# decisiongraph/leann-rs

Hardware: AMD Instinct MI355X
Metric: queries/sec @ recall@10>=0.95 (higher is better)
Workload: dtype f32

## Files before the change

### include/leann_backend.h

```cpp
#ifndef LEANN_BACKEND_H
#define LEANN_BACKEND_H
#include <stddef.h>
#include <stdint.h>

#ifdef __cplusplus
extern "C" {
#endif

typedef struct leann_backend leann_backend;

enum { LEANN_BACKEND_HNSW = 0, LEANN_BACKEND_DISKANN = 1 };

enum {
    LEANN_OK = 0,
    LEANN_ERR_INVALID = 1,
    LEANN_ERR_NOT_FOUND = 2,
    LEANN_ERR_FORMAT = 3,
    LEANN_ERR_DEVICE = 4,
    LEANN_ERR_UNSUPPORTED = 5,
    LEANN_ERR_IO = 6,
    LEANN_ERR_OVERFLOW = 7
};

const char *leann_last_error(void);
const char *leann_version(void);

int leann_backend_open(const char *index_path_stem, int backend, size_t dims,
                       const char *device_spec, leann_backend **out);

int leann_backend_search(const leann_backend *h, const float *query, size_t top_k,
                         size_t complexity, uint64_t *keys, float *dists, size_t *n_out);

int leann_backend_search_batch(const leann_backend *h, const float *queries, size_t nq,
                               size_t top_k, size_t complexity, uint64_t *keys, float *dists,
                               uint32_t *counts);

int leann_backend_search_filtered(const leann_backend *h, const float *query, size_t top_k,
                                  size_t complexity, const uint8_t *allow, uint64_t *keys,
                                  float *dists, size_t *n_out);
int leann_backend_search_filtered_batch(const leann_backend *h, const float *queries, size_t nq,
                                        size_t top_k, size_t complexity, const uint8_t *allow,
                                        size_t allow_stride, uint64_t *keys, float *dists,
                                        uint32_t *counts);

int leann_backend_search_filtered_exact_batch(const leann_backend *h, const float *queries, size_t nq,
                                              size_t top_k, const uint8_t *allow, size_t allow_stride,
                                              uint64_t *keys, float *dists, uint32_t *counts);

typedef struct leann_filter leann_filter;
int leann_backend_filter_create(const leann_backend *h, const uint8_t *allow, leann_filter **out);
size_t leann_backend_filter_count(const leann_filter *f);
void leann_backend_filter_free(leann_filter *f);
int leann_backend_search_filter_batch(const leann_backend *h, const float *queries, size_t nq, size_t top_k,
                                      size_t complexity, const leann_filter *filter, int mode,
                                      uint64_t *keys, float *dists, uint32_t *counts);

int leann_backend_set_coalescing(leann_backend *h, uint32_t wait_us, uint32_t max_batch);
int leann_backend_coalescing_stats(const leann_backend *h, uint64_t *n_launches, uint64_t *n_queries);

size_t leann_backend_len(const leann_backend *h);
size_t leann_backend_dims(const leann_backend *h);
void leann_backend_close(leann_backend *h);

int leann_backend_build(int backend, const float *vectors, size_t n, size_t dims,
                        size_t graph_degree, size_t complexity, const char *index_path_stem);
int leann_backend_add(int backend, const float *vectors, size_t n, size_t dims, size_t start_id,
                      const char *index_path_stem);

int leann_backend_remove(leann_backend *h, const uint64_t *keys, size_t n, size_t *n_removed);
int leann_backend_consolidate(leann_backend *h);
size_t leann_backend_live_len(const leann_backend *h);
int leann_backend_removed_bitmap(const leann_backend *h, uint8_t *out , size_t *n_pending);
int leann_backend_remove_from_index(int backend, const uint64_t *keys, size_t n, size_t dims, const char *index_path_stem);
int leann_tombstones_write(const char *path, const uint8_t *bitmap, uint64_t n, uint64_t n_pending);
int leann_tombstones_read(const char *path, uint64_t n_expected, uint8_t *bitmap_out, uint64_t *n_removed, uint64_t *n_pending);

typedef struct {
    uint64_t n_queries;
    uint64_t n_dist_evals;
    uint64_t n_hops_base;
    uint64_t n_hops_upper;
    uint64_t n_table_overflow;
    uint64_t algorithmic_bytes;
} leann_search_stats;
int leann_backend_stats(const leann_backend *h, leann_search_stats *out, int reset);


int leann_backend_build_device(int backend, const float *d_vectors, size_t n, size_t dims,
                               size_t ld, size_t graph_degree, size_t complexity, int device,
                               uint64_t key_offset, int take_copy, leann_backend **out);
int leann_backend_from_arrays(int backend, const float *vectors, size_t n, size_t dims,
                              uint32_t M, uint32_t M0, uint32_t max_level, uint32_t entry,
                              const uint8_t *levels, const uint32_t *upper_off,
                              const uint32_t *adj0, const uint32_t *adjU, size_t n_upper_lists,
                              int device, uint64_t key_offset, leann_backend **out);
int leann_backend_graph_info(const leann_backend *h, uint64_t *info );
int leann_backend_graph_export(const leann_backend *h, uint8_t *levels, uint32_t *upper_off,
                               uint32_t *adj0, uint32_t *adjU, float *vectors );
int leann_backend_save(const leann_backend *h, const char *index_path_stem);

int leann_backend_search_batch_device(const leann_backend *h, const float *d_queries, size_t nq,
                                      size_t top_k, size_t complexity, uint64_t *d_keys,
                                      float *d_dists, uint32_t *d_counts, uint32_t *d_stats,
                                      void *stream);
int leann_backend_search_filtered_batch_device(const leann_backend *h, const float *d_queries,
                                               size_t nq, size_t top_k, size_t complexity,
                                               const uint8_t *d_allow, size_t allow_stride,
                                               uint64_t *d_keys, float *d_dists, uint32_t *d_counts,
                                               uint32_t *d_stats, void *stream);
int leann_backend_search_filtered_exact_batch_device(const leann_backend *h, const float *d_queries,
                                                     size_t nq, size_t top_k, const uint8_t *d_allow,
                                                     size_t allow_stride, uint64_t *d_keys, float *d_dists,
                                                     uint32_t *d_counts, void *stream);
const float *leann_backend_device_rows(const leann_backend *h);

int leann_synth_rows_device(uint64_t seed, uint32_t dims, uint32_t ld, uint32_t r,
                            uint32_t n_clusters, float sigma, uint32_t stream_id, uint64_t i0,
                            uint64_t n, float *d_out, void *stream);

int leann_scan_topk_device(const float *d_rows, size_t n, size_t dims, size_t ld,
                           const float *d_queries, size_t nq, size_t top_k,
                           const uint8_t *d_allow_mask, uint64_t key_offset, uint64_t *d_keys,
                           float *d_scores, uint32_t *d_counts, void *stream);

typedef struct leann_recompute leann_recompute;
int leann_recompute_create(const uint16_t *d_features, size_t n, size_t h, const uint16_t *d_weights,
                           size_t dims, int device, uint64_t key_offset, leann_recompute **out);
int leann_recompute_create_pooled(const uint16_t *d_features, const uint8_t *d_mask, size_t n,
                                  size_t tokens_per_passage, size_t h, const uint16_t *d_weights,
                                  size_t dims, int device, uint64_t key_offset, leann_recompute **out);
int leann_recompute_search_batch_device(const leann_recompute *r, const float *d_queries, size_t nq,
                                        size_t top_k, const uint8_t *d_allow_mask, uint64_t *d_keys,
                                        float *d_scores, uint32_t *d_counts, void *stream);
int leann_recompute_create_host(const uint16_t *features, size_t n, size_t h, const uint16_t *weights,
                                size_t dims, int device, uint64_t key_offset, leann_recompute **out);
int leann_recompute_search_batch(const leann_recompute *r, const float *queries, size_t nq, size_t top_k,
                                 const uint8_t *allow_mask, uint64_t *keys, float *scores, uint32_t *counts);
int leann_recompute_create_sharded(const leann_recompute *const *parts, size_t n_parts, leann_recompute **out);
int leann_recompute_encode_device(const leann_recompute *r, uint64_t row0, uint64_t rows, float *d_out,
                                  void *stream);
size_t leann_recompute_len(const leann_recompute *r);
int leann_recompute_last_timing(const leann_recompute *r, float *ms3);
void leann_recompute_close(leann_recompute *r);
int leann_recompute_build_index(const leann_recompute *r, int backend, size_t graph_degree, size_t complexity,
                                leann_backend **out);
int leann_backend_feature_rows_export(const leann_backend *h, uint32_t *feat_h, uint32_t *row_bytes, void *out);
int leann_synth_features_device(uint64_t seed, uint32_t h, uint32_t r_int, uint32_t n_clusters, float sigma,
                                uint32_t stream_id, uint64_t i0, uint64_t n, uint16_t *d_out, void *stream);
int leann_synth_weights_device(uint64_t seed, uint32_t h, uint32_t dims, uint16_t *d_out, void *stream);

int leann_merge_topk_device(const uint64_t *d_keys, const float *d_dists, const uint32_t *d_counts,
                            size_t n_shards, size_t nq, size_t k_in, size_t k_out, int descending,
                            uint64_t *d_out_keys, float *d_out_dists, uint32_t *d_out_counts,
                            void *stream);

int leann_hybrid_rerank_device(const uint64_t *d_keys, const float *d_dists, const uint32_t *d_counts, size_t nq, size_t fetch_k,
                               const uint32_t *d_bm25_pos, const float *d_bm25_score, const uint32_t *d_bm25_count,
                               size_t bm25_stride, size_t n_docs, float alpha, int compat_polarity, size_t top_k,
                               uint64_t *d_out_keys, float *d_out_scores, uint32_t *d_out_counts, void *stream);

typedef struct leann_bm25 leann_bm25;
int leann_bm25_create(size_t n_docs, size_t n_terms, const uint64_t *post_off, const uint32_t *post_doc, const uint32_t *post_tf,
                      const uint32_t *doc_len, float avg_doc_len, int device, leann_bm25 **out);
size_t leann_bm25_len(const leann_bm25 *b);
size_t leann_bm25_slots(const leann_bm25 *b);
void leann_bm25_close(leann_bm25 *b);
int leann_bm25_check_queries(size_t n_terms, size_t nq, const uint32_t *q_off, const uint32_t *q_term, const float *q_idf);
int leann_bm25_search_batch(const leann_bm25 *b, size_t nq, const uint32_t *q_off, const uint32_t *q_term, const float *q_idf,
                            size_t top_k, uint32_t *pos, float *scores, uint32_t *counts, uint32_t *n_positive, float *min_max);
int leann_bm25_search_batch_device(const leann_bm25 *b, size_t nq, const uint32_t *q_off, const uint32_t *q_term, const float *q_idf,
                                   size_t top_k, uint32_t *d_pos, float *d_scores, uint32_t *d_counts, uint32_t *d_n_positive,
                                   float *d_min_max, void *stream);
int leann_bm25_hybrid_rerank_device(const leann_bm25 *b, size_t nq, const uint32_t *q_off, const uint32_t *q_term, const float *q_idf,
                                    const uint64_t *d_keys, const float *d_dists, const uint32_t *d_counts, size_t fetch_k,
                                    float alpha, int compat_polarity, size_t top_k,
                                    uint64_t *d_out_keys, float *d_out_scores, uint32_t *d_out_counts, void *stream);

typedef struct leann_sharded leann_sharded;
int leann_sharded_open(const char *index_path_stem, int backend, size_t dims, const char *device_spec, leann_sharded **out);
size_t leann_backend_shard_count(const leann_backend *h);
int leann_backend_shard(const leann_backend *h, size_t g, leann_backend **out);
int leann_sharded_build_device(int backend, const float *const *d_vectors, const size_t *rows, size_t n_shards, size_t dims,
                               size_t ld, size_t graph_degree, size_t complexity, const int *devices, leann_sharded **out);
int leann_sharded_from_handles(leann_backend *const *shards, size_t n_shards, int take_ownership, leann_sharded **out);
int leann_sharded_as_backend(leann_sharded *s, leann_backend **out);
int leann_rccl_get_unique_id(void *id128);
int leann_sharded_attach(leann_backend *local_shard, const void *unique_id128, int world, int rank, size_t total_rows,
                         leann_sharded **out);
int leann_sharded_search_batch_device(const leann_sharded *s, const float *d_queries, size_t nq, size_t top_k, size_t complexity,
                                      uint64_t *d_keys, float *d_dists, uint32_t *d_counts, uint32_t *d_stats, void *stream);
int leann_sharded_search_batch_device_async(const leann_sharded *s, const float *d_queries, size_t nq, size_t top_k,
                                            size_t complexity, uint64_t *d_keys, float *d_dists, uint32_t *d_counts,
                                            uint32_t *d_stats, void *stream, uint64_t *ticket);
int leann_sharded_wait(const leann_sharded *s, uint64_t ticket, void *stream);
size_t leann_sharded_len(const leann_sharded *s);
size_t leann_sharded_shards(const leann_sharded *s);
void leann_sharded_close(leann_sharded *s);

void leann_debug_reload_env(void);

int leann_device_count(int *n);
int leann_device_malloc(int device, size_t bytes, void **out);
int leann_device_free(void *p);
int leann_device_upload(void *d_dst, const void *h_src, size_t bytes);
int leann_device_download(void *h_dst, const void *d_src, size_t bytes);
int leann_device_sync(int device);

#ifdef __cplusplus
}
#endif
#endif
```

### leann-rs_amd/_native.py

```python
import ctypes as C
import os

_HERE = os.path.dirname(os.path.abspath(__file__))
LIB_PATH = os.environ.get("LEANN_LIB") or os.path.join(_HERE, "csrc", "libleann_hip.so")

u64p = C.POINTER(C.c_uint64)
u32p = C.POINTER(C.c_uint32)
u8p = C.POINTER(C.c_uint8)
f32p = C.POINTER(C.c_float)
vp = C.c_void_p


class LeannError(RuntimeError):
    def __init__(self, code, msg):
        super().__init__(msg)
        self.code = code


class SearchStats(C.Structure):
    _fields_ = [("n_queries", C.c_uint64), ("n_dist_evals", C.c_uint64), ("n_hops_base", C.c_uint64),
                ("n_hops_upper", C.c_uint64), ("n_table_overflow", C.c_uint64),
                ("algorithmic_bytes", C.c_uint64)]


SIGNATURES = {
    "leann_last_error": (C.c_char_p, []),
    "leann_version": (C.c_char_p, []),
    "leann_debug_reload_env": (None, []),
    "leann_backend_shard_count": (C.c_size_t, [vp]),
    "leann_backend_shard": (C.c_int, [vp, C.c_size_t, C.POINTER(vp)]),
    "leann_hybrid_rerank_device": (C.c_int, [vp, vp, vp, C.c_size_t, C.c_size_t, vp, vp, vp, C.c_size_t, C.c_size_t, C.c_float, C.c_int,
                                            C.c_size_t, vp, vp, vp, vp]),
    "leann_bm25_create": (C.c_int, [C.c_size_t, C.c_size_t, u64p, u32p, u32p, u32p, C.c_float, C.c_int, C.POINTER(vp)]),
    "leann_bm25_len": (C.c_size_t, [vp]),
    "leann_bm25_slots": (C.c_size_t, [vp]),
    "leann_bm25_close": (None, [vp]),
    "leann_bm25_check_queries": (C.c_int, [C.c_size_t, C.c_size_t, u32p, u32p, f32p]),
    "leann_bm25_search_batch": (C.c_int, [vp, C.c_size_t, u32p, u32p, f32p, C.c_size_t, u32p, f32p, u32p, u32p, f32p]),
    "leann_bm25_search_batch_device": (C.c_int, [vp, C.c_size_t, u32p, u32p, f32p, C.c_size_t, vp, vp, vp, vp, vp, vp]),
    "leann_bm25_hybrid_rerank_device": (C.c_int, [vp, C.c_size_t, u32p, u32p, f32p, vp, vp, vp, C.c_size_t, C.c_float, C.c_int,
                                                 C.c_size_t, vp, vp, vp, vp]),
    "leann_backend_open": (C.c_int, [C.c_char_p, C.c_int, C.c_size_t, C.c_char_p, C.POINTER(vp)]),
    "leann_backend_search": (C.c_int, [vp, f32p, C.c_size_t, C.c_size_t, u64p, f32p, C.POINTER(C.c_size_t)]),
    "leann_backend_search_batch": (C.c_int, [vp, f32p, C.c_size_t, C.c_size_t, C.c_size_t, u64p, f32p, u32p]),
    "leann_backend_search_filtered": (C.c_int, [vp, f32p, C.c_size_t, C.c_size_t, u8p, u64p, f32p, C.POINTER(C.c_size_t)]),
    "leann_backend_search_filtered_batch": (C.c_int, [vp, f32p, C.c_size_t, C.c_size_t, C.c_size_t, u8p, C.c_size_t,
                                                     u64p, f32p, u32p]),
    "leann_backend_set_coalescing": (C.c_int, [vp, C.c_uint32, C.c_uint32]),
    "leann_backend_coalescing_stats": (C.c_int, [vp, u64p, u64p]),
    "leann_backend_len": (C.c_size_t, [vp]),
    "leann_backend_dims": (C.c_size_t, [vp]),
    "leann_backend_close": (None, [vp]),
    "leann_backend_build": (C.c_int, [C.c_int, f32p, C.c_size_t, C.c_size_t, C.c_size_t, C.c_size_t, C.c_char_p]),
    "leann_backend_add": (C.c_int, [C.c_int, f32p, C.c_size_t, C.c_size_t, C.c_size_t, C.c_char_p]),
    "leann_backend_remove": (C.c_int, [vp, u64p, C.c_size_t, C.POINTER(C.c_size_t)]),
    "leann_backend_consolidate": (C.c_int, [vp]),
    "leann_backend_live_len": (C.c_size_t, [vp]),
    "leann_backend_removed_bitmap": (C.c_int, [vp, u8p, C.POINTER(C.c_size_t)]),
    "leann_backend_remove_from_index": (C.c_int, [C.c_int, u64p, C.c_size_t, C.c_size_t, C.c_char_p]),
    "leann_tombstones_write": (C.c_int, [C.c_char_p, u8p, C.c_uint64, C.c_uint64]),
    "leann_tombstones_read": (C.c_int, [C.c_char_p, C.c_uint64, u8p, u64p, u64p]),
    "leann_backend_stats": (C.c_int, [vp, C.POINTER(SearchStats), C.c_int]),
    "leann_backend_build_device": (C.c_int, [C.c_int, vp, C.c_size_t, C.c_size_t, C.c_size_t, C.c_size_t,
                                            C.c_size_t, C.c_int, C.c_uint64, C.c_int, C.POINTER(vp)]),
    "leann_backend_from_arrays": (C.c_int, [C.c_int, f32p, C.c_size_t, C.c_size_t, C.c_uint32, C.c_uint32,
                                           C.c_uint32, C.c_uint32, u8p, u32p, u32p, u32p, C.c_size_t,
                                           C.c_int, C.c_uint64, C.POINTER(vp)]),
    "leann_backend_graph_info": (C.c_int, [vp, u64p]),
    "leann_backend_graph_export": (C.c_int, [vp, u8p, u32p, u32p, u32p, f32p]),
    "leann_backend_save": (C.c_int, [vp, C.c_char_p]),
    "leann_backend_search_batch_device": (C.c_int, [vp, vp, C.c_size_t, C.c_size_t, C.c_size_t, vp, vp, vp,
                                                   vp, vp]),
    "leann_backend_search_filtered_exact_batch": (C.c_int, [vp, f32p, C.c_size_t, C.c_size_t, u8p, C.c_size_t, u64p, f32p, u32p]),
    "leann_backend_filter_create": (C.c_int, [vp, u8p, C.POINTER(vp)]),
    "leann_backend_filter_count": (C.c_size_t, [vp]),
    "leann_backend_filter_free": (None, [vp]),
    "leann_backend_search_filter_batch": (C.c_int, [vp, f32p, C.c_size_t, C.c_size_t, C.c_size_t, vp, C.c_int, u64p, f32p, u32p]),
    "leann_backend_search_filtered_exact_batch_device": (C.c_int, [vp, vp, C.c_size_t, C.c_size_t, vp, C.c_size_t, vp, vp, vp, vp]),
    "leann_backend_search_filtered_batch_device": (C.c_int, [vp, vp, C.c_size_t, C.c_size_t, C.c_size_t, vp, C.c_size_t,
                                                            vp, vp, vp, vp, vp]),
    "leann_backend_device_rows": (vp, [vp]),
    "leann_synth_rows_device": (C.c_int, [C.c_uint64, C.c_uint32, C.c_uint32, C.c_uint32, C.c_uint32,
                                         C.c_float, C.c_uint32, C.c_uint64, C.c_uint64, vp, vp]),
    "leann_scan_topk_device": (C.c_int, [vp, C.c_size_t, C.c_size_t, C.c_size_t, vp, C.c_size_t, C.c_size_t,
                                        vp, C.c_uint64, vp, vp, vp, vp]),
    "leann_recompute_create": (C.c_int, [vp, C.c_size_t, C.c_size_t, vp, C.c_size_t, C.c_int, C.c_uint64, C.POINTER(vp)]),
    "leann_recompute_create_pooled": (C.c_int, [vp, vp, C.c_size_t, C.c_size_t, C.c_size_t, vp, C.c_size_t, C.c_int, C.c_uint64,
                                               C.POINTER(vp)]),
    "leann_recompute_create_sharded": (C.c_int, [C.POINTER(vp), C.c_size_t, C.POINTER(vp)]),
    "leann_recompute_create_host": (C.c_int, [C.POINTER(C.c_uint16), C.c_size_t, C.c_size_t, C.POINTER(C.c_uint16), C.c_size_t, C.c_int,
                                             C.c_uint64, C.POINTER(vp)]),
    "leann_recompute_search_batch": (C.c_int, [vp, f32p, C.c_size_t, C.c_size_t, u8p, u64p, f32p, u32p]),
    "leann_recompute_search_batch_device": (C.c_int, [vp, vp, C.c_size_t, C.c_size_t, vp, vp, vp, vp, vp]),
    "leann_recompute_encode_device": (C.c_int, [vp, C.c_uint64, C.c_uint64, vp, vp]),
    "leann_recompute_len": (C.c_size_t, [vp]),
    "leann_recompute_last_timing": (C.c_int, [vp, f32p]),
    "leann_recompute_close": (None, [vp]),
    "leann_recompute_build_index": (C.c_int, [vp, C.c_int, C.c_size_t, C.c_size_t, C.POINTER(vp)]),
    "leann_backend_feature_rows_export": (C.c_int, [vp, u32p, u32p, vp]),
    "leann_synth_features_device": (C.c_int, [C.c_uint64, C.c_uint32, C.c_uint32, C.c_uint32, C.c_float, C.c_uint32, C.c_uint64,
                                             C.c_uint64, vp, vp]),
    "leann_synth_weights_device": (C.c_int, [C.c_uint64, C.c_uint32, C.c_uint32, vp, vp]),
    "leann_merge_topk_device": (C.c_int, [vp, vp, vp, C.c_size_t, C.c_size_t, C.c_size_t, C.c_size_t,
                                         C.c_int, vp, vp, vp, vp]),
    "leann_sharded_open": (C.c_int, [C.c_char_p, C.c_int, C.c_size_t, C.c_char_p, C.POINTER(vp)]),
    "leann_sharded_build_device": (C.c_int, [C.c_int, C.POINTER(vp), C.POINTER(C.c_size_t), C.c_size_t, C.c_size_t, C.c_size_t, C.c_size_t,
                                            C.c_size_t, C.POINTER(C.c_int), C.POINTER(vp)]),
    "leann_sharded_from_handles": (C.c_int, [C.POINTER(vp), C.c_size_t, C.c_int, C.POINTER(vp)]),
    "leann_sharded_as_backend": (C.c_int, [vp, C.POINTER(vp)]),
    "leann_rccl_get_unique_id": (C.c_int, [vp]),
    "leann_sharded_attach": (C.c_int, [vp, vp, C.c_int, C.c_int, C.c_size_t, C.POINTER(vp)]),
    "leann_sharded_search_batch_device": (C.c_int, [vp, vp, C.c_size_t, C.c_size_t, C.c_size_t, vp, vp, vp, vp, vp]),
    "leann_sharded_search_batch_device_async": (C.c_int, [vp, vp, C.c_size_t, C.c_size_t, C.c_size_t, vp, vp, vp, vp, vp, u64p]),
    "leann_sharded_wait": (C.c_int, [vp, C.c_uint64, vp]),
    "leann_sharded_len": (C.c_size_t, [vp]),
    "leann_sharded_shards": (C.c_size_t, [vp]),
    "leann_sharded_close": (None, [vp]),
    "leann_device_count": (C.c_int, [C.POINTER(C.c_int)]),
    "leann_device_malloc": (C.c_int, [C.c_int, C.c_size_t, C.POINTER(vp)]),
    "leann_device_free": (C.c_int, [vp]),
    "leann_device_upload": (C.c_int, [vp, vp, C.c_size_t]),
    "leann_device_download": (C.c_int, [vp, vp, C.c_size_t]),
    "leann_device_sync": (C.c_int, [C.c_int]),
}

_lib = None


def lib():
    global _lib
    if _lib is None:
        if not os.path.exists(LIB_PATH):
            raise ImportError(
                f"{LIB_PATH} is missing: build it with `make` (hipcc --offload-arch=gfx950). "
                "leann-rs_amd has no CPU fallback.")
        L = C.CDLL(LIB_PATH)
        for name, (res, args) in SIGNATURES.items():
            f = getattr(L, name)
            f.restype = res
            f.argtypes = args
        _lib = L
    return _lib


def check(rc):
    if rc != 0:
        raise LeannError(rc, lib().leann_last_error().decode("utf-8", "replace"))


def device_count():
    n = C.c_int(0)
    lib().leann_device_count(C.byref(n))
    return n.value
```

### leann-rs_amd/backend.py

```python
import ctypes as C
import enum
import os

import numpy as np

from . import _native as N
from ._native import LeannError, f32p, u32p, u64p, u8p


class BackendType(enum.IntEnum):
    Hnsw = 0
    DiskAnn = 1

    @classmethod
    def from_name(cls, name):
        if name == "hnsw":
            return cls.Hnsw
        if name == "diskann":
            return cls.DiskAnn
        raise LeannError(1, f"Unknown backend: {name}")

    def load_searcher(self, index_path, dimensions, device=0):
        return BackendSearcher.load(self, index_path, dimensions, device)


def _p(a, t):
    return a.ctypes.data_as(t) if a is not None else None


class BackendSearcher:

    def __init__(self, handle, backend_type):
        self._h = handle
        self.backend_type = BackendType(backend_type)

    @classmethod
    def load(cls, backend_type, index_path, dimensions, device=0):
        h = C.c_void_p()
        N.check(N.lib().leann_backend_open(os.fsencode(str(index_path)), int(backend_type), dimensions,
                                           str(device).encode(), C.byref(h)))
        return cls(h, backend_type)

    @classmethod
    def from_arrays(cls, backend_type, vectors, M, M0, max_level, entry, levels, upper_off, adj0, adjU,
                    device=0, key_offset=0):
        vectors = np.ascontiguousarray(vectors, np.float32)
        levels = np.ascontiguousarray(levels, np.uint8)
        upper_off = np.ascontiguousarray(upper_off, np.uint32)
        adj0 = np.ascontiguousarray(adj0, np.uint32)
        adjU = np.ascontiguousarray(adjU, np.uint32)
        nul = adjU.size // M if adjU.size else 0
        h = C.c_void_p()
        n, d = vectors.shape
        N.check(N.lib().leann_backend_from_arrays(
            int(backend_type), _p(vectors, f32p), n, d, M, M0, max_level, entry, _p(levels, u8p),
            _p(upper_off, u32p), _p(adj0, u32p), _p(adjU, u32p) if nul else None, nul, device,
            key_offset, C.byref(h)))
        return cls(h, backend_type)

    @classmethod
    def build_device(cls, backend_type, d_vectors_ptr, n, dims, ld, graph_degree, complexity, device=0,
                     key_offset=0, take_copy=False):
        h = C.c_void_p()
        N.check(N.lib().leann_backend_build_device(int(backend_type), d_vectors_ptr, n, dims, ld,
                                                   graph_degree, complexity, device, key_offset,
                                                   1 if take_copy else 0, C.byref(h)))
        return cls(h, backend_type)

    def search(self, query, top_k, complexity):
        q = np.ascontiguousarray(query, np.float32).reshape(-1)
        if q.shape[0] != self.dims():
            raise LeannError(1, f"query has {q.shape[0]} dimensions, index has {self.dims()}")
        keys = np.zeros(max(top_k, 1), np.uint64)
        dists = np.zeros(max(top_k, 1), np.float32)
        n = C.c_size_t(0)
        N.check(N.lib().leann_backend_search(self._h, _p(q, f32p), top_k, complexity, _p(keys, u64p),
                                             _p(dists, f32p), C.byref(n)))
        return keys[: n.value].copy(), dists[: n.value].copy()

    def search_batch(self, queries, top_k, complexity):
        Q = np.ascontiguousarray(queries, np.float32)
        if Q.ndim != 2 or Q.shape[1] != self.dims():
            raise LeannError(1, f"queries must be [nq x {self.dims()}]")
        nq = Q.shape[0]
        keys = np.full((nq, top_k), np.iinfo(np.uint64).max, np.uint64)
        dists = np.full((nq, top_k), np.inf, np.float32)
        counts = np.zeros(nq, np.uint32)
        N.check(N.lib().leann_backend_search_batch(self._h, _p(Q, f32p), nq, top_k, complexity,
                                                   _p(keys, u64p), _p(dists, f32p), _p(counts, u32p)))
        return keys, dists, counts

    def search_filtered(self, query, top_k, complexity, allow):
        q = np.ascontiguousarray(query, np.float32).reshape(-1)
        if q.shape[0] != self.dims():
            raise LeannError(1, f"query has {q.shape[0]} dimensions, index has {self.dims()}")
        allow = np.ascontiguousarray(allow, np.uint8).reshape(-1)
        if allow.shape[0] < (self.len() + 7) // 8:
            raise LeannError(1, f"allow-bitmap has {allow.shape[0]} bytes, index needs {(self.len() + 7) // 8}")
        keys = np.zeros(max(top_k, 1), np.uint64)
        dists = np.zeros(max(top_k, 1), np.float32)
        n = C.c_size_t(0)
        N.check(N.lib().leann_backend_search_filtered(self._h, _p(q, f32p), top_k, complexity, _p(allow, u8p),
                                                      _p(keys, u64p), _p(dists, f32p), C.byref(n)))
        return keys[: n.value].copy(), dists[: n.value].copy()

    def search_filtered_batch(self, queries, top_k, complexity, allow):
        Q = np.ascontiguousarray(queries, np.float32)
        if Q.ndim != 2 or Q.shape[1] != self.dims():
            raise LeannError(1, f"queries must be [nq x {self.dims()}]")
        allow = np.ascontiguousarray(allow, np.uint8)
        stride = 0 if allow.ndim == 1 else allow.shape[1]
        if allow.shape[-1] < (self.len() + 7) // 8 or (allow.ndim == 2 and allow.shape[0] != Q.shape[0]):
            raise LeannError(1, "allow-bitmap shape does not match the index / the batch")
        nq = Q.shape[0]
        keys = np.full((nq, top_k), np.iinfo(np.uint64).max, np.uint64)
        dists = np.full((nq, top_k), np.inf, np.float32)
        counts = np.zeros(nq, np.uint32)
        N.check(N.lib().leann_backend_search_filtered_batch(self._h, _p(Q, f32p), nq, top_k, complexity, _p(allow, u8p),
                                                            stride, _p(keys, u64p), _p(dists, f32p), _p(counts, u32p)))
        return keys, dists, counts

    def search_filtered_exact_batch(self, queries, top_k, allow):
        Q = np.ascontiguousarray(queries, np.float32)
        if Q.ndim != 2 or Q.shape[1] != self.dims():
            raise LeannError(1, f"queries must be [nq x {self.dims()}]")
        allow = np.ascontiguousarray(allow, np.uint8)
        stride = 0 if allow.ndim == 1 else allow.shape[1]
        if allow.shape[-1] < (self.len() + 7) // 8 or (allow.ndim == 2 and allow.shape[0] != Q.shape[0]):
            raise LeannError(1, "allow-bitmap shape does not match the index / the batch")
        nq = Q.shape[0]
        keys = np.full((nq, top_k), np.iinfo(np.uint64).max, np.uint64)
        dists = np.full((nq, top_k), np.inf, np.float32)
        counts = np.zeros(nq, np.uint32)
        N.check(N.lib().leann_backend_search_filtered_exact_batch(self._h, _p(Q, f32p), nq, top_k, _p(allow, u8p), stride,
                                                                  _p(keys, u64p), _p(dists, f32p), _p(counts, u32p)))
        return keys, dists, counts

    def search_filtered_exact_batch_device(self, d_queries, nq, top_k, d_allow, allow_stride, d_keys, d_dists, d_counts,
                                           stream=None):
        N.check(N.lib().leann_backend_search_filtered_exact_batch_device(self._h, d_queries, nq, top_k, d_allow, allow_stride,
                                                                         d_keys, d_dists, d_counts, stream))

    def register_filter(self, allow):
        allow = np.ascontiguousarray(allow, np.uint8)
        if allow.ndim != 1 or allow.shape[0] < (self.len() + 7) // 8:
            raise LeannError(1, "allow-bitmap shape does not match the index")
        h = C.c_void_p()
        N.check(N.lib().leann_backend_filter_create(self._h, _p(allow, u8p), C.byref(h)))
        return Filter(h)

    def search_filter_batch(self, queries, top_k, complexity, flt, mode="auto"):
        Q = np.ascontiguousarray(queries, np.float32)
        if Q.ndim != 2 or Q.shape[1] != self.dims():
            raise LeannError(1, f"queries must be [nq x {self.dims()}]")
        nq = Q.shape[0]
        keys = np.full((nq, top_k), np.iinfo(np.uint64).max, np.uint64)
        dists = np.full((nq, top_k), np.inf, np.float32)
        counts = np.zeros(nq, np.uint32)
        N.check(N.lib().leann_backend_search_filter_batch(self._h, _p(Q, f32p), nq, top_k, complexity, flt._h,
                                                          {"walk": 0, "exact": 1, "auto": 2}[mode], _p(keys, u64p), _p(dists, f32p),
                                                          _p(counts, u32p)))
        return keys, dists, counts

    def search_batch_device(self, d_queries, nq, top_k, complexity, d_keys, d_dists, d_counts,
                            d_stats=None, stream=None):
        N.check(N.lib().leann_backend_search_batch_device(self._h, d_queries, nq, top_k, complexity,
                                                          d_keys, d_dists, d_counts, d_stats, stream))

    def search_filtered_batch_device(self, d_queries, nq, top_k, complexity, d_allow, allow_stride, d_keys, d_dists,
                                     d_counts, d_stats=None, stream=None):
        N.check(N.lib().leann_backend_search_filtered_batch_device(self._h, d_queries, nq, top_k, complexity, d_allow,
                                                                   allow_stride, d_keys, d_dists, d_counts, d_stats, stream))

    def set_coalescing(self, wait_us=200, max_batch=4096):
        N.check(N.lib().leann_backend_set_coalescing(self._h, wait_us, max_batch))

    def coalescing_stats(self):
        a, b = C.c_uint64(0), C.c_uint64(0)
        N.check(N.lib().leann_backend_coalescing_stats(self._h, C.byref(a), C.byref(b)))
        return {"launches": a.value, "queries": b.value}

    def len(self):
        return int(N.lib().leann_backend_len(self._h))

    __len__ = len

    def is_empty(self):
        return self.len() == 0

    def dims(self):
        return int(N.lib().leann_backend_dims(self._h))

    def remove(self, keys):
        k = np.ascontiguousarray(keys, np.uint64).reshape(-1)
        n = C.c_size_t(0)
        N.check(N.lib().leann_backend_remove(self._h, _p(k, u64p), k.shape[0], C.byref(n)))
        return int(n.value)

    def consolidate(self):
        N.check(N.lib().leann_backend_consolidate(self._h))

    def live_len(self):
        return int(N.lib().leann_backend_live_len(self._h))

    def removed_bitmap(self):
        bm = np.zeros(max((self.len() + 7) // 8, 1), np.uint8)
        pend = C.c_size_t(0)
        N.check(N.lib().leann_backend_removed_bitmap(self._h, _p(bm, u8p), C.byref(pend)))
        return bm[: (self.len() + 7) // 8], int(pend.value)

    def stats(self, reset=False):
        s = N.SearchStats()
        N.check(N.lib().leann_backend_stats(self._h, C.byref(s), 1 if reset else 0))
        return {k: int(getattr(s, k)) for k, _ in N.SearchStats._fields_}

    def graph_info(self):
        info = np.zeros(8, np.uint64)
        N.check(N.lib().leann_backend_graph_info(self._h, _p(info, u64p)))
        names = ("n", "dims", "ld", "M", "M0", "max_level", "entry", "n_upper_lists")
        return {k: int(v) for k, v in zip(names, info)}

    def graph_export(self, with_vectors=False):
        gi = self.graph_info()
        n = gi["n"]
        levels = np.zeros(n, np.uint8)
        upper_off = np.zeros(n, np.uint32)
        adj0 = np.zeros((n, gi["M0"]), np.uint32)
        adjU = np.zeros((max(gi["n_upper_lists"], 1), gi["M"]), np.uint32)
        X = np.zeros((n, gi["dims"]), np.float32) if with_vectors else None
        N.check(N.lib().leann_backend_graph_export(self._h, _p(levels, u8p), _p(upper_off, u32p),
                                                   _p(adj0, u32p), _p(adjU, u32p), _p(X, f32p)))
        return dict(gi, levels=levels, upper_off=upper_off, adj0=adj0, adjU=adjU[: gi["n_upper_lists"]],
                    vectors=X)

    def n_shards(self):
        return int(N.lib().leann_backend_shard_count(self._h))

    def shard(self, g):
        h = C.c_void_p()
        N.check(N.lib().leann_backend_shard(self._h, g, C.byref(h)))
        s = BackendSearcher(h, self.backend_type)
        s._borrowed = True
        return s

    def device_rows_ptr(self):
        return N.lib().leann_backend_device_rows(self._h)

    def save(self, index_path):
        N.check(N.lib().leann_backend_save(self._h, os.fsencode(str(index_path))))

    def close(self):
        if self._h:
            if not getattr(self, "_borrowed", False):
                N.lib().leann_backend_close(self._h)
            self._h = None

    def __del__(self):
        try:
            self.close()
        except Exception:
            pass


class HnswSearcher(BackendSearcher):

    @classmethod
    def load(cls, index_path, dimensions, device=0):
        return BackendSearcher.load.__func__(cls, BackendType.Hnsw, index_path, dimensions, device)


class DiskAnnSearcher(BackendSearcher):

    @classmethod
    def load(cls, index_path, dimensions, device=0):
        return BackendSearcher.load.__func__(cls, BackendType.DiskAnn, index_path, dimensions, device)


class BackendBuilder:

    def __init__(self, backend_type):
        self.backend_type = BackendType(backend_type)

    def build(self, embeddings, ids, index_path, dimensions, graph_degree, complexity):
        X = np.ascontiguousarray(embeddings, np.float32)
        if X.ndim != 2 or X.shape[1] != dimensions:
            raise LeannError(1, f"embeddings must be [n x {dimensions}]")
        N.check(N.lib().leann_backend_build(int(self.backend_type), _p(X, f32p), X.shape[0], dimensions,
                                            graph_degree, complexity, os.fsencode(str(index_path))))

    def add_to_index(self, embeddings, index_path, dimensions, start_id):
        X = np.ascontiguousarray(embeddings, np.float32)
        N.check(N.lib().leann_backend_add(int(self.backend_type), _p(X, f32p), X.shape[0], dimensions,
                                          start_id, os.fsencode(str(index_path))))

    def remove_from_index(self, keys, index_path, dimensions):
        k = np.ascontiguousarray(keys, np.uint64).reshape(-1)
        N.check(N.lib().leann_backend_remove_from_index(int(self.backend_type), _p(k, u64p), k.shape[0], dimensions,
                                                        os.fsencode(str(index_path))))



class Filter:

    def __init__(self, handle):
        self._h = handle

    def count(self):
        return int(N.lib().leann_backend_filter_count(self._h))

    def close(self):
        if self._h:
            N.lib().leann_backend_filter_free(self._h)
            self._h = None

    def __del__(self):
        try:
            self.close()
        except Exception:
            pass


class ShardedIndex:

    def __init__(self, handle, keep=()):
        self._h = handle
        self._keep = keep

    @classmethod
    def open(cls, backend_type, index_path, dimensions, device_spec):
        h = C.c_void_p()
        N.check(N.lib().leann_sharded_open(os.fsencode(str(index_path)), int(backend_type), dimensions, str(device_spec).encode(), C.byref(h)))
        return cls(h)

    @classmethod
    def build_device(cls, backend_type, d_ptrs, rows, dims, ld, graph_degree, complexity, devices, keep=()):
        G = len(d_ptrs)
        ptrs = (C.c_void_p * G)(*[C.c_void_p(p) for p in d_ptrs])
        rws = (C.c_size_t * G)(*rows)
        devs = (C.c_int * G)(*devices)
        h = C.c_void_p()
        N.check(N.lib().leann_sharded_build_device(int(backend_type), ptrs, rws, G, dims, ld, graph_degree, complexity, devs, C.byref(h)))
        return cls(h, keep)

    @classmethod
    def from_searchers(cls, searchers, take_ownership=False):
        G = len(searchers)
        hs = (C.c_void_p * G)(*[s._h for s in searchers])
        h = C.c_void_p()
        N.check(N.lib().leann_sharded_from_handles(hs, G, 1 if take_ownership else 0, C.byref(h)))
        if take_ownership:
            for s in searchers:
                s._h = None
        return cls(h, tuple(searchers))

    @staticmethod
    def rccl_unique_id():
        buf = C.create_string_buffer(128)
        N.check(N.lib().leann_rccl_get_unique_id(buf))
        return buf.raw

    @classmethod
    def attach(cls, searcher, unique_id, world, rank, total_rows=0):
        h = C.c_void_p()
        N.check(N.lib().leann_sharded_attach(searcher._h, C.c_char_p(bytes(unique_id)), world, rank, total_rows, C.byref(h)))
        return cls(h, (searcher,))

    def search_batch_device(self, d_queries, nq, top_k, complexity, d_keys, d_dists, d_counts, d_stats=None, stream=None):
        N.check(N.lib().leann_sharded_search_batch_device(self._h, d_queries, nq, top_k, complexity, d_keys, d_dists, d_counts, d_stats, stream))

    def search_batch_device_async(self, d_queries, nq, top_k, complexity, d_keys, d_dists, d_counts, d_stats=None, stream=None):
        t = C.c_uint64(0)
        N.check(N.lib().leann_sharded_search_batch_device_async(self._h, d_queries, nq, top_k, complexity, d_keys, d_dists, d_counts, d_stats,
                                                                stream, C.byref(t)))
        return t.value

    def wait(self, ticket, stream=None):
        N.check(N.lib().leann_sharded_wait(self._h, ticket, stream))

    def as_backend(self, backend_type=BackendType.Hnsw):
        h = C.c_void_p()
        N.check(N.lib().leann_sharded_as_backend(self._h, C.byref(h)))
        keep, self._h = self._keep, None
        s = BackendSearcher(h, backend_type)
        s._keep = keep
        return s

    def len(self):
        return int(N.lib().leann_sharded_len(self._h))

    def n_shards(self):
        return int(N.lib().leann_sharded_shards(self._h))

    def close(self):
        if self._h:
            N.lib().leann_sharded_close(self._h)
            self._h = None

    def __del__(self):
        try:
            self.close()
        except Exception:
            pass
```

### leann-rs_amd/csrc/api.hip

```cpp
#include "common.cuh"
#include "search.cuh"
#include "../../include/leann_backend.h"
#include "internal.h"

#include <algorithm>
#include <cstdarg>
#include <cstdio>
#include <cstring>
#include <strings.h>
#include <map>
#include <mutex>
#include <string>
#include <vector>
#include <sys/stat.h>
#include <chrono>
#include <condition_variable>
#include <thread>

static thread_local char g_err[2048] = "";
extern "C" void leann_set_error(const char *fmt, ...) {
    va_list ap;
    va_start(ap, fmt);
    vsnprintf(g_err, sizeof(g_err), fmt, ap);
    va_end(ap);
}
extern "C" const char *leann_last_error(void) { return g_err; }
void leann_log(int level, const char *fmt, ...) {
    static const int threshold = [] {
        const char *e = getenv("LEANN_LOG");
        if (!e) return (int)LEANN_LOG_WARN;
        if (!strcasecmp(e, "error")) return (int)LEANN_LOG_ERROR;
        if (!strcasecmp(e, "info")) return (int)LEANN_LOG_INFO;
        if (!strcasecmp(e, "debug") || !strcasecmp(e, "trace")) return (int)LEANN_LOG_DEBUG;
        return (int)LEANN_LOG_WARN;
    }();
    if (level > threshold) return;
    static const char *names[] = {"ERROR", "WARN", "INFO", "DEBUG"};
    char buf[1024];
    va_list ap;
    va_start(ap, fmt);
    vsnprintf(buf, sizeof(buf), fmt, ap);
    va_end(ap);
    fprintf(stderr, "%s leann_hip: %s\n", names[level < 0 ? 0 : (level > 3 ? 3 : level)], buf);
}
extern "C" const char *leann_version(void) { return "leann-rs_amd 0.1 (gfx950)"; }

static LeannKnobs *read_knobs_from_env() {
    LeannKnobs *k = new LeannKnobs();
    auto num = [](const char *name, int lo, int hi) { const char *e = getenv(name); if (!e || !*e) return 0; int v = atoi(e); return v >= lo && v <= hi ? v : 0; };
    auto flag = [](const char *name) { const char *e = getenv(name); return e && *e && strcmp(e, "0") != 0; };
    k->hash_bits = num("LEANN_DEBUG_HASH_BITS", 6, 15);
    k->nw = num("LEANN_DEBUG_NW", 1, 64);
    k->gpool_bits = num("LEANN_DEBUG_GPOOL_BITS", 6, 31);
    k->gpool2_bits = num("LEANN_DEBUG_GPOOL2_BITS", 6, 31);
    k->no_feat256 = flag("LEANN_DEBUG_NO_FEAT256");
    k->no_zero_copy = flag("LEANN_DEBUG_NO_ZERO_COPY");
    k->no_emit = flag("LEANN_DEBUG_NO_EMIT");
    k->fused_v1 = flag("LEANN_DEBUG_FUSED_V1");
    k->no_list = flag("LEANN_RECOMPUTE_NO_LIST");
    k->no_tiled = flag("LEANN_RECOMPUTE_NO_TILED");
    k->hnsw_reference_ef = flag("LEANN_HNSW_REFERENCE_EF");
    k->force_remote = flag("LEANN_DEBUG_FORCE_REMOTE");
    if (const char *e = getenv("LEANN_COALESCE")) k->coalesce_off = !strcmp(e, "off") || !strcmp(e, "0");
    if (const char *e = getenv("LEANN_STAMP_BUF")) k->stamp_buf = strtoull(e, nullptr, 0);
    return k;
}
static std::atomic<const LeannKnobs *> g_knobs{nullptr};
const LeannKnobs &leann_knobs() {
    const LeannKnobs *k = g_knobs.load(std::memory_order_acquire);
    if (!k) {
        LeannKnobs *fresh = read_knobs_from_env();
        const LeannKnobs *expected = nullptr;
        if (g_knobs.compare_exchange_strong(expected, fresh, std::memory_order_acq_rel)) k = fresh;
        else { delete fresh; k = expected; }
    }
    return *k;
}
extern "C" void leann_debug_reload_env(void) { g_knobs.store(read_knobs_from_env(), std::memory_order_release); }

extern "C" int leann_device_count(int *n) {
    int c = 0;
    hipError_t e = hipGetDeviceCount(&c);
    if (e != hipSuccess) { c = 0; (void)hipGetLastError(); }
    *n = c;
    return LEANN_OK;
}
extern "C" int leann_device_malloc(int device, size_t bytes, void **out) {
    HIP_CHECK_RET(hipSetDevice(device));
    HIP_CHECK_RET(hipMalloc(out, bytes ? bytes : 16));
    return LEANN_OK;
}
extern "C" int leann_device_free(void *p) {
    if (p) HIP_CHECK_RET(hipFree(p));
    return LEANN_OK;
}
extern "C" int leann_device_upload(void *d, const void *h, size_t bytes) {
    HIP_CHECK_RET(hipMemcpy(d, h, bytes, hipMemcpyHostToDevice));
    return LEANN_OK;
}
extern "C" int leann_device_download(void *h, const void *d, size_t bytes) {
    HIP_CHECK_RET(hipMemcpy(h, d, bytes, hipMemcpyDeviceToHost));
    return LEANN_OK;
}
extern "C" int leann_device_sync(int device) {
    HIP_CHECK_RET(hipSetDevice(device));
    HIP_CHECK_RET(hipDeviceSynchronize());
    return LEANN_OK;
}

extern "C" int leann_backend_set_coalescing(leann_backend *h, uint32_t wait_us, uint32_t max_batch);
static void ws_free(Workspace *w) {
    if (!w) return;
    (void)hipFree(w->d_q);
    (void)hipFree(w->d_keys);
    (void)hipFree(w->d_dists);
    (void)hipFree(w->d_counts);
    (void)hipFree(w->d_stats);
    (void)hipFree(w->d_allow);
    if (w->pin) (void)hipHostFree(w->pin);
    if (w->stream) (void)hipStreamDestroy(w->stream);
    delete w;
}
static uint32_t debug_bits(int knob, uint32_t lo, uint32_t hi, uint32_t dflt) {
    return knob >= (int)lo && knob <= (int)hi ? (uint32_t)knob : dflt;
}
static int ensure_gpool(leann_backend *h) {
    std::lock_guard<std::mutex> lk(h->mu);
    if (h->gpool) return LEANN_OK;
    unsigned long long *p = nullptr, *p2 = nullptr;
    uint32_t *lock = nullptr, *lock2 = nullptr;
    const uint32_t bits = debug_bits(leann_knobs().gpool_bits, 6, GPOOL_BITS, GPOOL_BITS), tables = GPOOL_TABLES;
    const size_t slots = (size_t)tables << bits;
    uint32_t bits2 = 0, tables2 = 0;
    const uint64_t need = h->g.n + 128;
    if (need > (1ull << bits) - (1ull << (bits - 2))) {
        bits2 = bits + 1;
        while (bits2 < 31 && (1ull << bits2) - (1ull << (bits2 - 2)) < need) bits2++;
        bits2 = debug_bits(leann_knobs().gpool2_bits, 6, 31, bits2);
        const uint64_t per = 8ull << bits2;
        tables2 = (uint32_t)std::min<uint64_t>(64, std::max<uint64_t>(2, (1ull << 30) / per));
    }
    auto fail = [&](const char *what) {
        (void)hipFree(p); (void)hipFree(p2); (void)hipFree(lock); (void)hipFree(lock2);
        leann_set_error("visited-table pool: %s failed: %s", what, hipGetErrorString(hipGetLastError()));
        return LEANN_ERR_DEVICE;
    };
    if (hipMalloc((void **)&p, slots * 8) != hipSuccess) return fail("hipMalloc");
    if (hipMalloc((void **)&lock, (tables + 4) * 4) != hipSuccess) return fail("hipMalloc");
    if (hipMemset(p, 0, slots * 8) != hipSuccess) return fail("hipMemset");
    if (hipMemset(lock, 0, (tables + 4) * 4) != hipSuccess) return fail("hipMemset");
    if (tables2) {
        if (hipMalloc((void **)&p2, ((size_t)tables2 << bits2) * 8) != hipSuccess) return fail("hipMalloc");
        if (hipMalloc((void **)&lock2, tables2 * 4) != hipSuccess) return fail("hipMalloc");
        if (hipMemset(p2, 0, ((size_t)tables2 << bits2) * 8) != hipSuccess) return fail("hipMemset");
        if (hipMemset(lock2, 0, tables2 * 4) != hipSuccess) return fail("hipMemset");
    }
    if (hipDeviceSynchronize() != hipSuccess) return fail("hipDeviceSynchronize");
    h->gpool_lock = lock;
    h->gpool_ctr = lock + tables;
    h->gpool_bits = bits;
    h->gpool_tables = tables;
    h->gpool2 = p2;
    h->gpool2_lock = lock2;
    h->gpool2_bits = bits2;
    h->gpool2_tables = tables2;
    h->gpool = p;
    return LEANN_OK;
}
static void set_pool_args(const leann_backend *h, SearchArgs &a) {
    a.gpool = h->gpool; a.gpool_lock = h->gpool_lock; a.gpool_ctr = h->gpool_ctr;
    a.gpool_bits = h->gpool_bits; a.gpool_tables = h->gpool_tables;
    a.gpool2 = h->gpool2; a.gpool2_lock = h->gpool2_lock; a.gpool2_bits = h->gpool2_bits; a.gpool2_tables = h->gpool2_tables;
}

void leann_internal_free_graph(leann_backend *h) {
    if (h->owns_rows) (void)hipFree((void *)h->g.X);
    (void)hipFree((void *)h->g.norms);
    (void)hipFree((void *)h->g.adj0);
    (void)hipFree((void *)h->g.adjU);
    (void)hipFree((void *)h->g.upper_off);
    (void)hipFree(h->d_levels);
    (void)hipFree(h->gpool);
    (void)hipFree(h->gpool_lock);
    (void)hipFree(h->gpool2);
    (void)hipFree(h->gpool2_lock);
    (void)hipFree(h->Wf32);
    for (auto &kv : h->proj_scratch) (void)hipFree(kv.second.first);
    leann_internal_free_removed(h);
}

extern "C" void leann_backend_close(leann_backend *h) {
    if (!h) return;
    leann_backend_set_coalescing(h, 0, 0);
    (void)hipSetDevice(h->device);
    (void)hipDeviceSynchronize();
    for (auto *w : h->free_ws) ws_free(w);
    if (h->sharded) leann_sharded_close(h->sharded);
    else leann_internal_free_graph(h);
    delete h;
}
extern "C" size_t leann_backend_len(const leann_backend *h) { return h ? (size_t)h->g.n : 0; }
extern "C" size_t leann_backend_dims(const leann_backend *h) { return h ? (size_t)h->g.d : 0; }
extern "C" const float *leann_backend_device_rows(const leann_backend *h) { return h && !h->sharded ? h->g.X : nullptr; }
#define NOT_ON_SHARDED(h, what)                                                                                                    \
    do {                                                                                                                           \
        if ((h) && (h)->sharded) {                                                                                                 \
            leann_set_error("%s is not available on a sharded handle (use leann_backend_shard(h, g) for one shard's)", what);       \
            return LEANN_ERR_UNSUPPORTED;                                                                                          \
        }                                                                                                                          \
    } while (0)

extern "C" int leann_backend_stats(const leann_backend *hc, leann_search_stats *out, int reset) {
    leann_backend *h = const_cast<leann_backend *>(hc);
    if (!h || !out) { leann_set_error("leann_backend_stats: null argument"); return LEANN_ERR_INVALID; }
    std::lock_guard<std::mutex> lk(h->mu);
    *out = h->stats;
    if (reset) h->stats = leann_search_stats{};
    return LEANN_OK;
}

size_t leann_internal_effective_complexity(const leann_backend *h, size_t complexity) {
    return (h->fixed_ef && h->kind == LEANN_BACKEND_HNSW) ? (size_t)h->fixed_ef : complexity;
}

static uint32_t pick_hash_bits(uint32_t ef) {
    if (const int v = leann_knobs().hash_bits) return (uint32_t)v;
    uint32_t want = ef * 24u, b = 13;
    while ((1u << b) < want && b < 15) b++;
    return b;
}

using SearchKernel = void (*)(GraphView, SearchArgs);
static int launch_one(SearchKernel kernel, int nthreads, size_t lds, const GraphView &g, const SearchArgs &a, hipStream_t st) {
    if (lds > 64 * 1024)
        HIP_CHECK_RET(hipFuncSetAttribute((const void *)kernel, hipFuncAttributeMaxDynamicSharedMemorySize, 160 * 1024));
    hipLaunchKernelGGL(kernel, dim3(a.nq), dim3(nthreads), lds, st, g, a);
    HIP_CHECK_RET(hipGetLastError());
    return LEANN_OK;
}
static int search_lds_checked(const GraphView &g, const SearchArgs &a, size_t *lds, int nw) {
    *lds = search_lds_bytes(a.ef, std::max(g.M0, g.M), a.hash_bits, a.allow ? a.k : 0u, nw > 4 ? 2u : 1u);
    if (*lds > 160 * 1024) {
        leann_set_error("search: complexity %u needs %zu B of LDS per query (> 160 KiB)", a.ef, *lds);
        return LEANN_ERR_INVALID;
    }
    return LEANN_OK;
}

static bool wide_graph(const GraphView &g) { return std::max(g.M0, g.M) > 64; }

template <int T, int R, int NW>
static int launch_search_NW(const GraphView &g, const SearchArgs &a, hipStream_t st) {
    size_t lds;
    if (int rc = search_lds_checked(g, a, &lds, NW)) return rc;
    SearchKernel k = a.allow ? beam_search_filtered_kernel<T, R, NW> : a.q_rows ? beam_search_kernel<T, R, NW, true> : beam_search_kernel<T, R, NW, false>;
    if constexpr (NW != 8)
        if (wide_graph(g))
            k = a.allow ? wide_beam_search_filtered_kernel<T, R, NW> : a.q_rows ? wide_beam_search_kernel<T, R, NW, true> : wide_beam_search_kernel<T, R, NW, false>;
    return launch_one(k, NW * 64, lds, g, a, st);
}

template <int T, int R>
static int launch_search_T(const GraphView &g, const SearchArgs &a, hipStream_t st) {
    int nw = a.nq <= 384 ? 16 : a.nq <= 640 ? 8 : 4;
    if (const int v = leann_knobs().nw) nw = v;
    if (nw >= 8 && wide_graph(g)) nw = 16;
    if (nw >= 16) return launch_search_NW<T, R, 16>(g, a, st);
    if (nw >= 8) return launch_search_NW<T, R, 8>(g, a, st);
    return launch_search_NW<T, R, 4>(g, a, st);
}

template <int T, int R>
static int launch_search_feat(const GraphView &g, const SearchArgs &a, hipStream_t st) {
    size_t lds;
    if (int rc = search_lds_checked(g, a, &lds, a.nq <= 512 ? 16 : 4)) return rc;
    const bool wide = wide_graph(g), filt = a.allow != nullptr, small = a.nq <= 512;
    SearchKernel k;
    if (T == 1 && g.feat_h == 256 && !leann_knobs().no_feat256)
        k = wide ? (small ? (filt ? wide_beam_search_feat256_filtered_kernel<1, 16> : wide_beam_search_feat256_kernel<1, 16>)
                          : (filt ? wide_beam_search_feat256_filtered_kernel<LEANN_FEAT_G, 4> : wide_beam_search_feat256_kernel<LEANN_FEAT_G, 4>))
                 : (small ? (filt ? beam_search_feat256_filtered_kernel<1, 16> : beam_search_feat256_kernel<1, 16>)
                          : (filt ? beam_search_feat256_filtered_kernel<LEANN_FEAT_G, 4> : beam_search_feat256_kernel<LEANN_FEAT_G, 4>));
    else
        k = wide ? (small ? (filt ? wide_beam_search_feat_filtered_kernel<T, R, 16> : wide_beam_search_feat_kernel<T, R, 16>)
                          : (filt ? wide_beam_search_feat_filtered_kernel<T, R, 4> : wide_beam_search_feat_kernel<T, R, 4>))
                 : (small ? (filt ? beam_search_feat_filtered_kernel<T, R, 16> : beam_search_feat_kernel<T, R, 16>)
                          : (filt ? beam_search_feat_filtered_kernel<T, R, 4> : beam_search_feat_kernel<T, R, 4>));
    return launch_one(k, small ? 16 * 64 : 4 * 64, lds, g, a, st);
}

static int project_queries(leann_backend *h, const float *d_queries, size_t nq, hipStream_t st, const float **out) {
    float *G = nullptr;
    {
        std::lock_guard<std::mutex> lk(h->mu);
        auto &sc = h->proj_scratch[st];
        const size_t need = nq * h->g.feat_h;
        if (sc.second < need) {
            (void)hipFree(sc.first);
            sc.first = nullptr;
            sc.second = 0;
            if (hipMalloc((void **)&sc.first, need * 4) != hipSuccess) { leann_set_error("hipMalloc(%zu) failed", need * 4); return LEANN_ERR_DEVICE; }
            sc.second = need;
        }
        G = sc.first;
    }
    int rc = leann_internal_score(h->Wf32, h->g.feat_h, h->g.d, h->g.d, d_queries, nq, h->g.d, G, st);
    *out = G;
    return rc;
}

int leann_internal_launch_search(leann_backend *h, SearchArgs a, hipStream_t st) {
    if (a.nq == 0) return LEANN_OK;
    if (h->g.feat_h) {
        if (a.q_rows) { leann_set_error("recompute-on index: construction searches are not supported"); return LEANN_ERR_UNSUPPORTED; }
        if (a.ef < a.k) a.ef = a.k;
        a.hash_bits = leann_knobs().hash_bits ? pick_hash_bits(a.ef) : (a.ef <= 64 ? 12u : pick_hash_bits(a.ef));
        int rc = ensure_gpool(h);
        if (rc) return rc;
        set_pool_args(h, a);
        const float *G = nullptr;
        rc = project_queries(h, a.queries, a.nq, st, &G);
        if (rc) return rc;
        a.queries = G;
        a.ldq = h->g.feat_h;
        const int T = (int)((h->g.feat_h + 255) / 256);
        switch (T) {
            case 1: return launch_search_feat<1, LEANN_FEAT_R1>(h->g, a, st);
            case 2: return launch_search_feat<2, 6>(h->g, a, st);
            case 3: case 4: return launch_search_feat<4, 4>(h->g, a, st);
            default: leann_set_error("recompute-on index: feature width %u > 1024 not supported", h->g.feat_h); return LEANN_ERR_INVALID;
        }
    }
    if (a.ef < a.k) a.ef = a.k;
    a.hash_bits = (h->g.ld <= 512 && a.ef <= 64 && !a.q_rows && !leann_knobs().hash_bits) ? 12u : pick_hash_bits(a.ef);
    int rc = ensure_gpool(h);
    if (rc) return rc;
    set_pool_args(h, a);
    const GraphView &g = h->g;
    int T = (int)((g.ld + 255) / 256);
    switch (T) {
        case 1: return launch_search_T<1, 4>(g, a, st);
        case 2: return launch_search_T<2, 4>(g, a, st);
        case 3: return launch_search_T<3, 4>(g, a, st);
        case 4: return launch_search_T<4, 3>(g, a, st);
        case 5: case 6: return launch_search_T<6, 2>(g, a, st);
        case 7: case 8: return launch_search_T<8, 2>(g, a, st);
        case 9: case 10: case 11: case 12: return launch_search_T<12, 1>(g, a, st);
        case 13: case 14: case 15: case 16: return launch_search_T<16, 1>(g, a, st);
        default:
            leann_set_error("search: dims %u > 4096 not supported", g.d);
            return LEANN_ERR_INVALID;
    }
}

extern "C" int leann_backend_search_batch_device(const leann_backend *hc, const float *d_queries, size_t nq,
                                                 size_t top_k, size_t complexity, uint64_t *d_keys, float *d_dists,
                                                 uint32_t *d_counts, uint32_t *d_stats, void *stream) {
    return leann_backend_search_filtered_batch_device(hc, d_queries, nq, top_k, complexity, nullptr, 0, d_keys, d_dists,
                                                      d_counts, d_stats, stream);
}

int leann_internal_search_plain(leann_backend *h, const float *d_queries, size_t nq, size_t top_k, size_t complexity, const SearchFilter &f,
                                uint64_t *d_keys, float *d_dists, uint32_t *d_counts, uint32_t *d_stats, hipStream_t st) {
    if (int rc = leann_internal_check_allow_stride(f, h->g.n)) return rc;
    if (nq == 0) return LEANN_OK;
    if (f.exact && h->g.feat_h) {
        leann_set_error("exact filtered search needs stored vectors; this index recomputes them from features (use leann_recompute_search_batch_device with an allow mask)");
        return LEANN_ERR_UNSUPPORTED;
    }
    if (h->g.n == 0) {
        HIP_CHECK_RET(hipMemsetAsync(d_counts, 0, nq * 4, st));
        return LEANN_OK;
    }
    const leann_filter *reg = f.registered;
    const uint8_t *allow = reg ? reg->d_allow : f.d_allow;
    size_t allow_stride = reg ? 0 : f.allow_stride;
    if (!reg)
        if (int rc = leann_internal_live_allow(h, allow, allow_stride, nq, !f.exact, st, &allow, &allow_stride)) return rc;
    if (f.exact) {
        if (!allow) { leann_set_error("exact filtered search: no filter given"); return LEANN_ERR_INVALID; }
        if (d_stats) HIP_CHECK_RET(hipMemsetAsync(d_stats, 0, nq * 16, st));
        if (reg)
            return leann_internal_filtered_exact_list(h->g.X, h->g.d, h->g.ld, d_queries, nq, top_k, reg->d_list, reg->n_allowed, h->key_offset,
                                                      d_keys, d_dists, d_counts, st);
        return leann_internal_filtered_exact(h->g.X, h->g.n, h->g.d, h->g.ld, d_queries, nq, top_k, allow, allow_stride, h->key_offset, d_keys,
                                             d_dists, d_counts, st);
    }
    SearchArgs a{};
    a.queries = d_queries;
    a.ldq = h->g.d;
    a.nq = (uint32_t)nq;
    a.k = (uint32_t)top_k;
    a.ef = (uint32_t)std::max(leann_internal_effective_complexity(h, complexity), top_k);
    a.target_level = 0;
    a.key_offset = h->key_offset;
    a.out_keys = d_keys;
    a.out_dists = d_dists;
    a.out_counts = d_counts;
    a.out_stats = d_stats;
    a.allow = allow;
    a.allow_stride = allow_stride;
#ifdef LEANN_STAMPS
    if (const unsigned long long e = leann_knobs().stamp_buf) {
        a.out_nexp = reinterpret_cast<uint32_t *>(e);
        a.exp_cap = 0xFEED;
    }
#endif
    return leann_internal_launch_search(h, a, st);
}
static int search_device(leann_backend *h, const float *d_queries, size_t nq, size_t top_k, size_t complexity, const SearchFilter &f,
                         uint64_t *d_keys, float *d_dists, uint32_t *d_counts, uint32_t *d_stats, hipStream_t st) {
    HIP_CHECK_RET(hipSetDevice(h->device));
    if (h->sharded) return leann_internal_sharded_search(h->sharded, d_queries, nq, top_k, complexity, f, d_keys, d_dists, d_counts, d_stats, st, nullptr);
    return leann_internal_search_plain(h, d_queries, nq, top_k, complexity, f, d_keys, d_dists, d_counts, d_stats, st);
}

extern "C" int leann_backend_search_filtered_batch_device(const leann_backend *hc, const float *d_queries, size_t nq,
                                                          size_t top_k, size_t complexity, const uint8_t *d_allow,
                                                          size_t allow_stride, uint64_t *d_keys, float *d_dists,
                                                          uint32_t *d_counts, uint32_t *d_stats, void *stream) {
    leann_backend *h = const_cast<leann_backend *>(hc);
    if (!h || !d_queries || !d_keys || !d_dists || !d_counts || top_k == 0) {
        leann_set_error("leann_backend_search_batch_device: null/zero argument");
        return LEANN_ERR_INVALID;
    }
    SearchFilter f;
    f.d_allow = d_allow; f.allow_stride = allow_stride;
    return search_device(h, d_queries, nq, top_k, complexity, f, d_keys, d_dists, d_counts, d_stats, (hipStream_t)stream);
}

extern "C" int leann_backend_search_batch(const leann_backend *hc, const float *queries, size_t nq, size_t top_k,
                                          size_t complexity, uint64_t *keys, float *dists, uint32_t *counts) {
    return leann_backend_search_filtered_batch(hc, queries, nq, top_k, complexity, nullptr, 0, keys, dists, counts);
}

enum { FILTER_WALK = 0, FILTER_EXACT = 1, FILTER_AUTO = 2 };
static int search_filtered_batch_host(const leann_backend *hc, const float *queries, size_t nq, size_t top_k, size_t complexity,
                                      const uint8_t *allow, size_t allow_stride, uint64_t *keys, float *dists, uint32_t *counts, int mode,
                                      const leann_filter *flt = nullptr);

extern "C" int leann_backend_filter_create(const leann_backend *hc, const uint8_t *allow, leann_filter **out) {
    if (!hc || !allow || !out) {
        leann_set_error("leann_backend_filter_create: null argument");
        return LEANN_ERR_INVALID;
    }
    *out = nullptr;
    if (hc->sharded) {
        const size_t G = leann_internal_sharded_count(hc->sharded);
        leann_filter *f = new leann_filter();
        f->device = hc->device;
        f->n = hc->g.n;
        for (size_t g = 0; g < G; g++) {
            leann_backend *sh = leann_internal_sharded_shard(hc->sharded, g);
            const uint64_t lo = leann_internal_sharded_lo(hc->sharded, g);
            leann_filter *part = nullptr;
            int rc = (!sh || (lo & 7)) ? (leann_set_error("registered filter: shard %zu does not start at a multiple of 8", g), (int)LEANN_ERR_UNSUPPORTED)
                                       : leann_backend_filter_create(sh, allow + lo / 8, &part);
            if (rc) { leann_backend_filter_free(f); return rc; }
            f->parts.push_back(part);
            f->n_allowed += part->n_allowed;
        }
        (void)hipSetDevice(hc->device);
        f->epoch = hc->removal_epoch;
        *out = f;
        return LEANN_OK;
    }
    if (hc->g.n >= (1ull << 32)) {
        leann_set_error("leann_backend_filter_create: the index has 2^32 rows or more");
        return LEANN_ERR_INVALID;
    }
    HIP_CHECK_RET(hipSetDevice(hc->device));
    leann_filter *f = new leann_filter();
    f->device = hc->device;
    f->n = hc->g.n;
    const size_t nbytes = std::max<size_t>((f->n + 7) / 8, 1);
    if (hipMalloc((void **)&f->d_allow, nbytes) != hipSuccess || hipMemcpy(f->d_allow, allow, (f->n + 7) / 8, hipMemcpyHostToDevice) != hipSuccess) {
        leann_set_error("leann_backend_filter_create: device allocation / copy of %zu bytes failed", nbytes);
        if (f->d_allow) (void)hipFree(f->d_allow);
        delete f;
        return LEANN_ERR_DEVICE;
    }
    f->epoch = hc->removal_epoch;
    int rc = leann_internal_and_live_inplace(hc, f->d_allow);
    if (rc == LEANN_OK && f->n) rc = leann_internal_compact_allow(f->d_allow, f->n, &f->d_list, &f->n_allowed, nullptr);
    if (rc != LEANN_OK) {
        (void)hipFree(f->d_allow);
        delete f;
        return rc;
    }
    *out = f;
    return LEANN_OK;
}
extern "C" size_t leann_backend_filter_count(const leann_filter *f) { return f ? f->n_allowed : 0; }
extern "C" void leann_backend_filter_free(leann_filter *f) {
    if (!f) return;
    if (!f->parts.empty()) {
        for (auto *p : f->parts) leann_backend_filter_free(p);
        delete f;
        return;
    }
    (void)hipSetDevice(f->device);
    (void)hipDeviceSynchronize();
    leann_internal_scratch_release(f->d_list);
    if (f->d_allow) (void)hipFree(f->d_allow);
    delete f;
}
extern "C" int leann_backend_search_filter_batch(const leann_backend *hc, const float *queries, size_t nq, size_t top_k, size_t complexity,
                                                 const leann_filter *filter, int mode, uint64_t *keys, float *dists, uint32_t *counts) {
    if (!filter || !hc || filter->n != hc->g.n || filter->device != hc->device || mode < FILTER_WALK || mode > FILTER_AUTO ||
        filter->parts.empty() != (hc->sharded == nullptr)) {
        leann_set_error("leann_backend_search_filter_batch: null / foreign filter (made for %zu rows, the index has %zu) or bad mode %d",
                        filter ? filter->n : (size_t)0, hc ? (size_t)hc->g.n : (size_t)0, mode);
        return LEANN_ERR_INVALID;
    }
    bool stale = filter->epoch != hc->removal_epoch;
    if (hc->sharded)
        for (size_t g = 0; g < filter->parts.size() && g < leann_internal_sharded_count(hc->sharded); g++)
            stale = stale || filter->parts[g]->epoch != leann_internal_sharded_shard(hc->sharded, g)->removal_epoch;
    if (stale) {
        leann_set_error("leann_backend_search_filter_batch: filter predates a removal; register it again");
        return LEANN_ERR_INVALID;
    }
    return search_filtered_batch_host(hc, queries, nq, top_k, complexity, nullptr, 0, keys, dists, counts, mode, filter);
}

extern "C" int leann_backend_search_filtered_batch(const leann_backend *hc, const float *queries, size_t nq, size_t top_k,
                                                   size_t complexity, const uint8_t *allow, size_t allow_stride,
                                                   uint64_t *keys, float *dists, uint32_t *counts) {
    return search_filtered_batch_host(hc, queries, nq, top_k, complexity, allow, allow_stride, keys, dists, counts, FILTER_WALK);
}
extern "C" int leann_backend_search_filtered_exact_batch(const leann_backend *hc, const float *queries, size_t nq, size_t top_k,
                                                         const uint8_t *allow, size_t allow_stride, uint64_t *keys, float *dists,
                                                         uint32_t *counts) {
    if (!allow) {
        leann_set_error("leann_backend_search_filtered_exact_batch: null allow-bitmap");
        return LEANN_ERR_INVALID;
    }
    return search_filtered_batch_host(hc, queries, nq, top_k, 0, allow, allow_stride, keys, dists, counts, FILTER_EXACT);
}
extern "C" int leann_backend_search_filtered_exact_batch_device(const leann_backend *hc, const float *d_queries, size_t nq, size_t top_k,
                                                                const uint8_t *d_allow, size_t allow_stride, uint64_t *d_keys,
                                                                float *d_dists, uint32_t *d_counts, void *stream) {
    leann_backend *h = const_cast<leann_backend *>(hc);
    if (!h || !d_queries || !d_keys || !d_dists || !d_counts || !d_allow || top_k == 0) {
        leann_set_error("leann_backend_search_filtered_exact_batch_device: null/zero argument");
        return LEANN_ERR_INVALID;
    }
    SearchFilter f;
    f.d_allow = d_allow; f.allow_stride = allow_stride; f.exact = true;
    return search_device(h, d_queries, nq, top_k, 0, f, d_keys, d_dists, d_counts, nullptr, (hipStream_t)stream);
}
static int search_filtered_batch_host_impl(const leann_backend *hc, const float *queries, size_t nq, size_t top_k, size_t complexity,
                                      const uint8_t *allow, size_t allow_stride, uint64_t *keys, float *dists, uint32_t *counts, int mode,
                                      const leann_filter *flt) {
    leann_backend *h = const_cast<leann_backend *>(hc);
    bool exact = mode == FILTER_EXACT;
    const bool stored_vectors = hc && !(hc->sharded ? leann_internal_sharded_shard(hc->sharded, 0)->g.feat_h : hc->g.feat_h);
    if (mode == FILTER_AUTO && flt && hc && stored_vectors && top_k <= 1024) {
        const double frac = nq <= 64 ? 0.05 : 0.015;
        exact = flt->n_allowed <= std::max<size_t>((size_t)(frac * (double)hc->g.n), nq <= 64 ? 65536 : 0);
    }
    if (!h || !queries || !keys || !dists || !counts) {
        leann_set_error("leann_backend_search_batch: null argument");
        return LEANN_ERR_INVALID;
    }
    if (nq == 0 || top_k == 0 || h->g.n == 0) {
        for (size_t i = 0; i < nq; i++) counts[i] = 0;
        return LEANN_OK;
    }
    HIP_CHECK_RET(hipSetDevice(h->device));
    Workspace *w = nullptr;
    {
        std::lock_guard<std::mutex> lk(h->mu);
        if (!h->free_ws.empty()) { w = h->free_ws.back(); h->free_ws.pop_back(); }
    }
    if (!w) w = new Workspace();
    int rc = LEANN_OK;
    auto fail = [&](int code) { std::lock_guard<std::mutex> lk(h->mu); h->free_ws.push_back(w); return code; };
    if (!w->stream) {
        if (hipStreamCreateWithFlags(&w->stream, hipStreamNonBlocking) != hipSuccess) {
            leann_set_error("hipStreamCreate failed");
            return fail(LEANN_ERR_DEVICE);
        }
    }
    const size_t d = h->g.d, qf = nq * d, no = nq * top_k;
    const size_t ns = 1;
    auto grow = [&](void **p, size_t &cap, size_t need, size_t elt) -> int {
        if (need <= cap) return 0;
        (void)hipFree(*p);
        *p = nullptr;
        cap = 0;
        if (hipMalloc(p, need * elt) != hipSuccess) { leann_set_error("hipMalloc(%zu) failed", need * elt); return 1; }
        cap = need;
        return 0;
    };
    const size_t o_keys = (qf * 4 + 15) & ~(size_t)15, o_dists = o_keys + no * 8, o_counts = (o_dists + no * 4 + 15) & ~(size_t)15,
                 o_stats = o_counts + ((nq * 4 + 15) & ~(size_t)15), pin_bytes = o_stats + nq * 16;
    bool zero_copy = !h->sharded && !exact && pin_bytes <= ((size_t)256 << 10) && !leann_knobs().no_zero_copy;
    if (zero_copy && w->cap_pin < pin_bytes) {
        if (w->pin) (void)hipHostFree(w->pin);
        w->pin = nullptr;
        w->cap_pin = 0;
        const size_t want = std::max<size_t>(pin_bytes, (size_t)64 << 10);
        if (hipHostMalloc((void **)&w->pin, want, hipHostMallocDefault) == hipSuccess) w->cap_pin = want;
        else { (void)hipGetLastError(); zero_copy = false; }
    }
    const bool zc_in = zero_copy && nq <= 4;
    if (zero_copy && !zc_in && grow((void **)&w->d_q, w->cap_q, qf, 4)) return fail(LEANN_ERR_DEVICE);
    if (!zero_copy && (grow((void **)&w->d_q, w->cap_q, qf, 4) || grow((void **)&w->d_keys, w->cap_keys, no, 8) ||
        grow((void **)&w->d_dists, w->cap_dists, no, 4) || grow((void **)&w->d_counts, w->cap_counts, nq, 4) ||
        grow((void **)&w->d_stats, w->cap_stats, ns * nq * 4, 4)))
        return fail(LEANN_ERR_DEVICE);
    hipStream_t st = w->stream;
    if (allow) {
        const size_t total = allow_stride ? allow_stride * nq : (h->g.n + 7) / 8;
        void *pa = w->d_allow;
        if (grow(&pa, w->cap_allow, total, 1)) { w->d_allow = (uint8_t *)pa; return fail(LEANN_ERR_DEVICE); }
        w->d_allow = (uint8_t *)pa;
        if (hipMemcpyAsync(w->d_allow, allow, total, hipMemcpyHostToDevice, st) != hipSuccess) {
            leann_set_error("H2D copy of the allow-bitmap failed");
            return fail(LEANN_ERR_DEVICE);
        }
    }
    if (zero_copy) memcpy(w->pin, queries, qf * 4);
    if (!zc_in && hipMemcpyAsync(w->d_q, zero_copy ? reinterpret_cast<const float *>(w->pin) : queries, qf * 4, hipMemcpyHostToDevice, st) != hipSuccess) {
        leann_set_error("H2D copy of queries failed");
        return fail(LEANN_ERR_DEVICE);
    }
    SearchFilter f;
    f.exact = exact;
    if (flt) f.registered = flt;
    else if (allow) { f.d_allow = w->d_allow; f.allow_stride = allow_stride; }
    const float *d_q = zc_in ? reinterpret_cast<const float *>(w->pin) : w->d_q;
    uint64_t *d_keys = zero_copy ? reinterpret_cast<uint64_t *>(w->pin + o_keys) : w->d_keys;
    float *d_dists = zero_copy ? reinterpret_cast<float *>(w->pin + o_dists) : w->d_dists;
    uint32_t *d_counts = zero_copy ? reinterpret_cast<uint32_t *>(w->pin + o_counts) : w->d_counts;
    uint32_t *d_stats = zero_copy ? reinterpret_cast<uint32_t *>(w->pin + o_stats) : w->d_stats;
    rc = h->sharded ? leann_internal_sharded_search(h->sharded, d_q, nq, top_k, complexity, f, d_keys, d_dists, d_counts, d_stats, st, nullptr)
                    : leann_internal_search_plain(h, d_q, nq, top_k, complexity, f, d_keys, d_dists, d_counts, d_stats, st);
    if (rc) return fail(rc);
    std::vector<uint32_t> hstats(ns * nq * 4);
    if (zero_copy) {
        if (hipStreamSynchronize(st) != hipSuccess) {
            leann_set_error("search: device error: %s", hipGetErrorString(hipGetLastError()));
            return fail(LEANN_ERR_DEVICE);
        }
        memcpy(keys, w->pin + o_keys, no * 8);
        memcpy(dists, w->pin + o_dists, no * 4);
// ... 30 lines not shown
        return LEANN_ERR_OVERFLOW;
    }
    return LEANN_OK;
}

static int search_filtered_batch_host(const leann_backend *hc, const float *queries, size_t nq, size_t top_k, size_t complexity,
                                      const uint8_t *allow, size_t allow_stride, uint64_t *keys, float *dists, uint32_t *counts, int mode,
                                      const leann_filter *flt) {
    try {
        return search_filtered_batch_host_impl(hc, queries, nq, top_k, complexity, allow, allow_stride, keys, dists, counts, mode, flt);
    } catch (const std::exception &e) {
        leann_set_error("search: %s", e.what());
        return LEANN_ERR_DEVICE;
    }
}

struct PendingQuery {
    const float *q;
    size_t k, ef;
    uint64_t *keys;
    float *dists;
    size_t *n_out;
    int rc = 0;
    bool done = false, answered = false;
    std::string err;
};
struct Coalescer {
    leann_backend *h = nullptr;
    uint32_t wait_us = 200, max_batch = 4096;
    std::mutex mu;
    std::condition_variable cv_submit, cv_done;
    std::vector<PendingQuery *> queue;
    std::thread th;
    bool stop = false;
    uint64_t n_launches = 0, n_queries = 0;
    size_t recent_callers = 0;

    void run() {
        (void)hipSetDevice(h->device);
        std::unique_lock<std::mutex> lk(mu);
        for (;;) {
            cv_submit.wait(lk, [&] { return stop || !queue.empty(); });
            if (stop && queue.empty()) return;
            const size_t fire_at = std::min<size_t>(max_batch, std::max<size_t>(1, recent_callers));
            auto deadline = std::chrono::steady_clock::now() + std::chrono::microseconds(wait_us);
            cv_submit.wait_until(lk, deadline, [&] { return stop || queue.size() >= fire_at; });
            std::vector<PendingQuery *> batch;
            batch.swap(queue);
            lk.unlock();
            std::map<std::pair<size_t, size_t>, std::vector<PendingQuery *>> groups;
            for (auto *p : batch) groups[{p->k, p->ef}].push_back(p);
            const size_t d = h->g.d;
            try {
            for (auto &kv : groups) {
                auto &g = kv.second;
                const size_t nq = g.size(), k = kv.first.first;
                std::vector<float> Q(nq * d);
                for (size_t i = 0; i < nq; i++) memcpy(Q.data() + i * d, g[i]->q, d * 4);
                std::vector<uint64_t> keys(nq * std::max<size_t>(k, 1));
                std::vector<float> dists(nq * std::max<size_t>(k, 1));
                std::vector<uint32_t> counts(nq);
                int rc = leann_backend_search_batch(h, Q.data(), nq, k, kv.first.second, keys.data(), dists.data(), counts.data());
                std::string err = rc ? leann_last_error() : "";
                for (size_t i = 0; i < nq; i++) {
                    if (!rc) {
                        memcpy(g[i]->keys, keys.data() + i * k, counts[i] * 8);
                        memcpy(g[i]->dists, dists.data() + i * k, counts[i] * 4);
                        *g[i]->n_out = counts[i];
                    }
                    g[i]->rc = rc;
                    g[i]->err = err;
                    g[i]->answered = true;
                }
                n_launches++;
                n_queries += nq;
            }
            } catch (const std::exception &e) {
                for (auto *p : batch)
                    if (!p->answered) { p->rc = LEANN_ERR_DEVICE; p->err = std::string("request coalescing: ") + e.what(); *p->n_out = 0; }
            }
            lk.lock();
            recent_callers = batch.size() + queue.size();
            for (auto *p : batch) p->done = true;
            cv_done.notify_all();
        }
    }
};

static std::shared_ptr<Coalescer> make_coalescer(leann_backend *h, uint32_t wait_us, uint32_t max_batch) {
    auto fresh = std::make_shared<Coalescer>();
    fresh->h = h;
    fresh->wait_us = wait_us;
    fresh->max_batch = max_batch ? max_batch : 4096;
    Coalescer *c = fresh.get();
    fresh->th = std::thread([c] { c->run(); });
    return fresh;
}
static void retire_coalescer(std::shared_ptr<Coalescer> old) {
    if (!old) return;
    { std::lock_guard<std::mutex> l2(old->mu); old->stop = true; }
    old->cv_submit.notify_all();
    old->th.join();
}
extern "C" int leann_backend_set_coalescing(leann_backend *h, uint32_t wait_us, uint32_t max_batch) {
    if (!h) { leann_set_error("leann_backend_set_coalescing: null handle"); return LEANN_ERR_INVALID; }
    std::shared_ptr<Coalescer> fresh, old;
    const bool off = wait_us == 0 && max_batch == 0;
    if (!off) fresh = make_coalescer(h, wait_us, max_batch);
    {
        std::lock_guard<std::mutex> lk(h->mu);
        old.swap(h->coalescer);
        h->coalescer = fresh;
        h->coalesce_mode = off ? 2 : 1;
    }
    retire_coalescer(old);
    return LEANN_OK;
}
static std::shared_ptr<Coalescer> auto_coalescer(leann_backend *h) {
    if (leann_knobs().coalesce_off) return nullptr;
    {
        std::lock_guard<std::mutex> lk(h->mu);
        if (h->coalesce_mode != 0) return h->coalescer;
        if (h->coalescer) return h->coalescer;
    }
    std::shared_ptr<Coalescer> fresh = make_coalescer(h, 50, 64), lost;
    {
        std::lock_guard<std::mutex> lk(h->mu);
        if (h->coalesce_mode == 0 && !h->coalescer) { h->coalescer = fresh; return fresh; }
        lost = fresh;
        fresh = h->coalescer;
    }
    retire_coalescer(lost);
    return fresh;
}
extern "C" int leann_backend_coalescing_stats(const leann_backend *hc, uint64_t *n_launches, uint64_t *n_queries) {
    leann_backend *h = const_cast<leann_backend *>(hc);
    std::shared_ptr<Coalescer> c;
    if (h) { std::lock_guard<std::mutex> lk(h->mu); c = h->coalescer; }
    if (!c) { leann_set_error("coalescing is not enabled on this handle"); return LEANN_ERR_INVALID; }
    std::lock_guard<std::mutex> l2(c->mu);
    if (n_launches) *n_launches = c->n_launches;
    if (n_queries) *n_queries = c->n_queries;
    return LEANN_OK;
}

extern "C" int leann_backend_search(const leann_backend *hc, const float *query, size_t top_k, size_t complexity,
                                    uint64_t *keys, float *dists, size_t *n_out) {
    if (!n_out) { leann_set_error("leann_backend_search: n_out is null"); return LEANN_ERR_INVALID; }
    leann_backend *h = const_cast<leann_backend *>(hc);
    std::shared_ptr<Coalescer> c;
    struct InFlight {
        std::atomic<int> *a;
        int before;
        explicit InFlight(std::atomic<int> *p) : a(p), before(p ? p->fetch_add(1) : 0) {}
        ~InFlight() { if (a) a->fetch_sub(1); }
    } inflight(h ? &h->singles_in_flight : nullptr);
    if (h && query && keys && dists && top_k > 0 && h->g.n > 0) {
        int mode;
        { std::lock_guard<std::mutex> lk(h->mu); c = h->coalescer; mode = h->coalesce_mode; }
        if (!c && mode == 0 && inflight.before > 0) c = auto_coalescer(h);
    }
    if (c) {
        PendingQuery p{query, top_k, complexity, keys, dists, n_out};
        std::unique_lock<std::mutex> lk(c->mu);
        if (!c->stop) {
            c->queue.push_back(&p);
            c->cv_submit.notify_one();
            c->cv_done.wait(lk, [&] { return p.done; });
            if (p.rc) leann_set_error("%s", p.err.c_str());
            return p.rc;
        }
    }
    uint32_t cnt = 0;
    int rc = leann_backend_search_batch(h, query, 1, top_k, complexity, keys, dists, &cnt);
    *n_out = cnt;
    return rc;
}

extern "C" int leann_backend_search_filtered(const leann_backend *hc, const float *query, size_t top_k, size_t complexity,
                                             const uint8_t *allow, uint64_t *keys, float *dists, size_t *n_out) {
    if (!n_out) { leann_set_error("leann_backend_search_filtered: n_out is null"); return LEANN_ERR_INVALID; }
    if (!allow) return leann_backend_search(hc, query, top_k, complexity, keys, dists, n_out);
    uint32_t cnt = 0;
    int rc = leann_backend_search_filtered_batch(hc, query, 1, top_k, complexity, allow, 0, keys, dists, &cnt);
    *n_out = cnt;
    return rc;
}

static const char *validate_graph(size_t n, uint32_t M, uint32_t M0, uint32_t max_level, uint32_t entry, const uint8_t *levels,
                                  const uint32_t *upper_off, const uint32_t *adj0, const uint32_t *adjU, size_t n_upper_lists) {
    if (M == 0 || M0 == 0 || M > 128 || M0 > 128) return "graph degree outside [1, 128]";
    if (max_level > 15) return "max_level > 15";
    if (n == 0) return nullptr;
    if (entry >= n) return "entry point is not a row of the index";
    if (!levels && (max_level != 0 || n_upper_lists != 0)) return "upper levels without a level table";
    if (n_upper_lists && !adjU) return "upper lists missing";
    if (levels && levels[entry] < max_level) return "the entry point does not reach max_level";
    for (size_t v = 0; v < n; v++) {
        const uint32_t lv = levels ? levels[v] : 0;
        if (lv > 15) return "node level > 15";
        if (lv && (size_t)upper_off[v] + lv > n_upper_lists) return "upper_off + level runs past the upper lists";
        const uint32_t *l0 = adj0 + v * (size_t)M0;
        for (uint32_t j = 0; j < M0; j++)
            if (l0[j] != LEANN_EMPTY && l0[j] >= n) return "level-0 neighbour id >= n";
        for (uint32_t l = 1; l <= lv; l++) {
            const uint32_t *lu = adjU + ((size_t)upper_off[v] + l - 1) * M;
            for (uint32_t j = 0; j < M; j++) {
                const uint32_t e = lu[j];
                if (e == LEANN_EMPTY) continue;
                if (e >= n) return "upper-level neighbour id >= n";
                if (levels[e] < l) return "upper-level neighbour does not exist on that level";
            }
        }
    }
    return nullptr;
}

int leann_internal_from_host(int backend, size_t n, size_t dims, uint32_t M, uint32_t M0, uint32_t max_level, uint32_t entry,
                             const uint8_t *levels, const uint32_t *upper_off, const uint32_t *adj0, const uint32_t *adjU,
                             size_t n_upper_lists, const float *vectors, const unsigned char *feat_rows, uint32_t feat_h, uint32_t row_bytes,
                             const float *Wf32, int device, uint64_t key_offset, leann_backend **out) {
    const bool feat = feat_rows != nullptr;
    if (!out || dims == 0 || dims > 4096 || n >= (1ull << 31) || (n && ((!vectors && !feat) || !adj0 || !upper_off)) ||
        (backend != LEANN_BACKEND_HNSW && backend != LEANN_BACKEND_DISKANN) ||
        (feat && (!Wf32 || feat_h == 0 || (feat_h & 3) || feat_h > 1024 || row_bytes < 2 * feat_h + 4 || (row_bytes & 7)))) {
        leann_set_error("leann_backend_from_arrays: invalid arguments");
        return LEANN_ERR_INVALID;
    }
    if (const char *why = validate_graph(n, M, M0, max_level, entry, levels, upper_off, adj0, adjU, n_upper_lists)) {
        leann_set_error("leann_backend_from_arrays: inconsistent graph arrays: %s", why);
        return LEANN_ERR_FORMAT;
    }
    int ndev = 0;
    leann_device_count(&ndev);
    if (device < 0 || device >= ndev) {
        leann_set_error("HIP device %d not available (%d visible). This library has no CPU fallback.", device, ndev);
        return LEANN_ERR_DEVICE;
    }
    HIP_CHECK_RET(hipSetDevice(device));
    leann_backend *h = new leann_backend();
    h->kind = backend;
    h->device = device;
    h->key_offset = key_offset;
    h->g.n = n;
    h->g.d = (uint32_t)dims;
    h->g.ld = (uint32_t)((dims + 3) & ~(size_t)3);
    h->g.M = M;
    h->g.M0 = M0;
    h->g.max_level = max_level;
    h->g.entry = entry;
    h->n_upper_lists = n_upper_lists;
    if (const char *e = getenv("LEANN_VAMANA_TWO_STAGE")) h->two_stage = strcmp(e, "0") != 0;
    auto fail = [&](const char *what) {
        leann_set_error("leann_backend_from_arrays: %s failed: %s", what, hipGetErrorString(hipGetLastError()));
        leann_backend_close(h);
        return LEANN_ERR_DEVICE;
    };
    const size_t nn = std::max<size_t>(n, 1), nu = std::max<size_t>(n_upper_lists, 1), ld = h->g.ld;
    if (feat) {
        h->g.feat_h = feat_h;
        if (feat_h == 256) {
            h->g.row_bytes = 512;
            if (hipMalloc((void **)&h->g.X, nn * 512) != hipSuccess || hipMalloc((void **)&h->g.norms, nn * 4) != hipSuccess) return fail("hipMalloc(rows)");
            const size_t slab = (size_t)1 << 20;
            std::vector<unsigned char> fr(std::min(slab, nn) * 512);
            std::vector<float> nr(std::min(slab, nn));
            for (size_t s0 = 0; s0 < n; s0 += slab) {
                const size_t m = std::min(slab, n - s0);
                for (size_t i = 0; i < m; i++) {
                    memcpy(fr.data() + i * 512, feat_rows + (s0 + i) * row_bytes, 512);
                    memcpy(&nr[i], feat_rows + (s0 + i) * row_bytes + 512, 4);
                }
                if (hipMemcpy((unsigned char *)h->g.X + s0 * 512, fr.data(), m * 512, hipMemcpyHostToDevice) != hipSuccess ||
                    hipMemcpy((void *)(h->g.norms + s0), nr.data(), m * 4, hipMemcpyHostToDevice) != hipSuccess)
                    return fail("upload of the feature rows");
            }
        } else {
            h->g.row_bytes = row_bytes;
            if (hipMalloc((void **)&h->g.X, nn * row_bytes) != hipSuccess) return fail("hipMalloc(rows)");
            if (n && hipMemcpy((void *)h->g.X, feat_rows, n * (size_t)row_bytes, hipMemcpyHostToDevice) != hipSuccess) return fail("upload of the feature rows");
        }
        if (hipMalloc((void **)&h->Wf32, (size_t)feat_h * dims * 4) != hipSuccess) return fail("hipMalloc(weights)");
        if (hipMemcpy(h->Wf32, Wf32, (size_t)feat_h * dims * 4, hipMemcpyHostToDevice) != hipSuccess) return fail("upload of the weights");
    } else {
        if (hipMalloc((void **)&h->g.X, std::max<size_t>(n * ld, 4) * 4) != hipSuccess) return fail("hipMalloc(rows)");
        if (n) {
            if (ld == dims) { if (hipMemcpy((void *)h->g.X, vectors, n * dims * 4, hipMemcpyHostToDevice) != hipSuccess) return fail("upload of the rows"); }
            else if (hipMemset((void *)h->g.X, 0, n * ld * 4) != hipSuccess ||
                     hipMemcpy2D((void *)h->g.X, ld * 4, vectors, dims * 4, dims * 4, n, hipMemcpyHostToDevice) != hipSuccess) return fail("upload of the rows");
        }
    }
    if (hipMalloc((void **)&h->g.adj0, nn * M0 * 4) != hipSuccess || hipMalloc((void **)&h->g.adjU, nu * M * 4) != hipSuccess ||
        hipMalloc((void **)&h->g.upper_off, nn * 4) != hipSuccess || hipMalloc((void **)&h->d_levels, nn) != hipSuccess)
        return fail("hipMalloc(graph arrays)");
    if (hipMemset((void *)h->g.adjU, 0xFF, nu * M * 4) != hipSuccess) return fail("hipMemset");
    if (n) {
        if (hipMemcpy((void *)h->g.adj0, adj0, n * M0 * 4, hipMemcpyHostToDevice) != hipSuccess ||
            hipMemcpy((void *)h->g.upper_off, upper_off, n * 4, hipMemcpyHostToDevice) != hipSuccess ||
            (levels ? hipMemcpy(h->d_levels, levels, n, hipMemcpyHostToDevice) : hipMemset(h->d_levels, 0, n)) != hipSuccess ||
            (n_upper_lists && hipMemcpy((void *)h->g.adjU, adjU, n_upper_lists * M * 4, hipMemcpyHostToDevice) != hipSuccess))
            return fail("upload of the graph arrays");
    }
    if (hipDeviceSynchronize() != hipSuccess) return fail("hipDeviceSynchronize");
    *out = h;
    return LEANN_OK;
}

extern "C" int leann_backend_from_arrays(int backend, const float *vectors, size_t n, size_t dims, uint32_t M,
                                         uint32_t M0, uint32_t max_level, uint32_t entry, const uint8_t *levels,
                                         const uint32_t *upper_off, const uint32_t *adj0, const uint32_t *adjU,
                                         size_t n_upper_lists, int device, uint64_t key_offset, leann_backend **out) {
    try {
        return leann_internal_from_host(backend, n, dims, M, M0, max_level, entry, levels, upper_off, adj0, adjU, n_upper_lists, vectors,
                                        nullptr, 0, 0, nullptr, device, key_offset, out);
    } catch (const std::exception &e) {
        leann_set_error("leann_backend_from_arrays: %s", e.what());
        return LEANN_ERR_IO;
    }
}

extern "C" size_t leann_backend_shard_count(const leann_backend *h) { return h && h->sharded ? leann_internal_sharded_count(h->sharded) : 0; }
extern "C" int leann_backend_shard(const leann_backend *h, size_t g, leann_backend **out) {
    if (!h || !out) { leann_set_error("leann_backend_shard: null argument"); return LEANN_ERR_INVALID; }
    *out = nullptr;
    if (!h->sharded || g >= leann_internal_sharded_count(h->sharded) || !leann_internal_sharded_shard(h->sharded, g)) {
        leann_set_error("leann_backend_shard: %s", h->sharded ? "no such shard" : "not a sharded handle");
        return LEANN_ERR_INVALID;
    }
    *out = leann_internal_sharded_shard(h->sharded, g);
    return LEANN_OK;
}

extern "C" int leann_backend_graph_info(const leann_backend *h, uint64_t *info) {
    if (!h || !info) { leann_set_error("leann_backend_graph_info: null argument"); return LEANN_ERR_INVALID; }
    info[0] = h->g.n; info[1] = h->g.d; info[2] = h->g.ld; info[3] = h->g.M; info[4] = h->g.M0;
    info[5] = h->g.max_level; info[6] = h->g.entry; info[7] = h->n_upper_lists;
    return LEANN_OK;
}
extern "C" int leann_backend_graph_export(const leann_backend *h, uint8_t *levels, uint32_t *upper_off, uint32_t *adj0,
                                          uint32_t *adjU, float *vectors) {
    if (!h) { leann_set_error("leann_backend_graph_export: null handle"); return LEANN_ERR_INVALID; }
    NOT_ON_SHARDED(h, "graph export");
    HIP_CHECK_RET(hipSetDevice(h->device));
    HIP_CHECK_RET(hipDeviceSynchronize());
    const size_t n = h->g.n;
    if (n == 0) return LEANN_OK;
    if (levels) HIP_CHECK_RET(hipMemcpy(levels, h->d_levels, n, hipMemcpyDeviceToHost));
    if (upper_off) HIP_CHECK_RET(hipMemcpy(upper_off, h->g.upper_off, n * 4, hipMemcpyDeviceToHost));
    if (adj0) HIP_CHECK_RET(hipMemcpy(adj0, h->g.adj0, n * h->g.M0 * 4, hipMemcpyDeviceToHost));
    if (adjU && h->n_upper_lists)
        HIP_CHECK_RET(hipMemcpy(adjU, h->g.adjU, h->n_upper_lists * h->g.M * 4, hipMemcpyDeviceToHost));
    if (vectors && h->g.feat_h) { leann_set_error("graph_export: a recompute-on index holds no vectors"); return LEANN_ERR_UNSUPPORTED; }
    if (vectors)
        HIP_CHECK_RET(hipMemcpy2D(vectors, (size_t)h->g.d * 4, h->g.X, (size_t)h->g.ld * 4, (size_t)h->g.d * 4, n,
                                  hipMemcpyDeviceToHost));
    return LEANN_OK;
}
```

### leann-rs_amd/csrc/build.hip

```cpp
#include "common.cuh"
#include "search.cuh"
#include "internal.h"
#include "prune.cuh"
#include <hipcub/hipcub.hpp>
#include <algorithm>
#include <cstring>
#include <numeric>

#define EXPCAP 256
#define PATHMAX 48

struct ListView {
    uint32_t *adj0; float *adjd0;
    uint32_t *adjU; float *adjdU;
    const uint32_t *upper_off;
    uint32_t M, M0;
    uint32_t *pend; float *pendd;
    uint32_t P;
    uint32_t two_stage;
};
__device__ __forceinline__ void list_ptr(const ListView &lv, uint32_t node, uint32_t level, uint32_t **ids, float **ds,
                                         uint32_t *cap) {
    if (level == 0) {
        *ids = lv.adj0 + (size_t)node * lv.M0;
// ... 291 lines not shown
    uint64_t *candU_keys = nullptr; float *candU_d = nullptr; uint32_t *candU_cnt = nullptr; uint32_t *d_rowsU = nullptr;
    uint64_t *prop_key = nullptr, *prop_key2 = nullptr; uint32_t *prop_src = nullptr, *prop_src2 = nullptr;
    uint32_t *seg_start = nullptr, *nseg = nullptr;
    uint64_t *exp_keys = nullptr; uint32_t *exp_cnt = nullptr;
    void *cub_tmp = nullptr; size_t cub_bytes = 0;
    hipStream_t st = nullptr;
    size_t batch_fraction = 8;
    float alpha_now = 1.2f;
    Builder() = default;
    Builder(const Builder &) = delete;
    ~Builder() {
        if (st) (void)hipStreamSynchronize(st);
        void *ps[] = {cand_keys, cand_d, cand_cnt, candU_keys, candU_d, candU_cnt, d_rowsU, prop_key, prop_key2,
                      prop_src, prop_src2, seg_start, nseg, cub_tmp, d_order, adjd0, adjdU, exp_keys, exp_cnt, pend, pendd};
        for (void *p : ps) (void)hipFree(p);
        if (st) (void)hipStreamDestroy(st);
    }
};
static int env_int(const char *name, int dflt, int lo, int hi) {
    const char *e = getenv(name);
    if (!e || !*e) return dflt;
    const int v = atoi(e);
    return v >= lo && v <= hi ? v : dflt;
}
struct DevTmp {
    void *p = nullptr;
    ~DevTmp() { (void)hipFree(p); }
};

#define BCHECK(expr)                                                                           \
    do {                                                                                       \
        hipError_t _e = (expr);                                                                \
        if (_e != hipSuccess) {                                                                \
            leann_set_error("build: %s failed: %s (%s:%d)", #expr, hipGetErrorString(_e), __FILE__, __LINE__); \
            return LEANN_ERR_DEVICE;                                                           \
        }                                                                                      \
    } while (0)

static int link_level(Builder &b, const uint32_t *d_rows, uint32_t nq, uint32_t level, const uint64_t *ck, const float *cd,
                      const uint32_t *cc, const uint64_t *ek = nullptr, const uint32_t *ec = nullptr) {
    leann_backend *h = b.h;
    const uint32_t efc = h->efc, msel = h->g.M;
    const float alpha = h->kind == LEANN_BACKEND_DISKANN ? b.alpha_now : 0.f;
    const bool wide = std::max(h->g.M0, h->g.M) > 64;
    hipLaunchKernelGGL(wide ? wide_select_kernel : select_kernel, dim3(nq), dim3(256), 0, b.st, h->g.X, h->g.ld, b.lv, d_rows, nq, level,
                       ck, cd, cc, efc, msel, alpha, b.prop_key, b.prop_src, ek, ec, (uint32_t)EXPCAP);
    const uint32_t num = nq * msel;
    size_t tmp = b.cub_bytes;
    BCHECK(hipcub::DeviceRadixSort::SortPairs(b.cub_tmp, tmp, b.prop_key, b.prop_key2, b.prop_src, b.prop_src2, (int)num, 0, 64, b.st));
    BCHECK(hipMemsetAsync(b.nseg, 0, 4, b.st));
    hipLaunchKernelGGL(segment_heads_kernel, dim3((num + 255) / 256), dim3(256), 0, b.st, b.prop_key2, num, b.seg_start, b.nseg);
    uint32_t grid = std::min<uint32_t>(num, 256 * 16);
    hipLaunchKernelGGL(wide ? wide_reverse_merge_kernel : reverse_merge_kernel, dim3(grid), dim3(256), 0, b.st, h->g.X, h->g.ld, b.lv,
                       level, b.prop_key2, b.prop_src2, num, b.seg_start, b.nseg, alpha, 0u);
    BCHECK(hipGetLastError());
    return LEANN_OK;
}

static int builder_alloc_scratch(Builder &b, size_t bmax) {
    leann_backend *h = b.h;
    const size_t efc = h->efc, msel = h->g.M;
    b.bmax = bmax;
    const size_t bu = bmax / 16 + 64;
    BCHECK(hipMalloc((void **)&b.cand_keys, bmax * efc * 8));
    BCHECK(hipMalloc((void **)&b.cand_d, bmax * efc * 4));
    BCHECK(hipMalloc((void **)&b.cand_cnt, bmax * 4));
    BCHECK(hipMalloc((void **)&b.candU_keys, bu * efc * 8 * 16));
    BCHECK(hipMalloc((void **)&b.candU_d, bu * efc * 4 * 16));
    BCHECK(hipMalloc((void **)&b.candU_cnt, bu * 4 * 16));
    BCHECK(hipMalloc((void **)&b.d_rowsU, bu * 4 * 16));
    BCHECK(hipMalloc((void **)&b.prop_key, bmax * msel * 8));
    BCHECK(hipMalloc((void **)&b.prop_key2, bmax * msel * 8));
    BCHECK(hipMalloc((void **)&b.prop_src, bmax * msel * 4));
    BCHECK(hipMalloc((void **)&b.prop_src2, bmax * msel * 4));
    BCHECK(hipMalloc((void **)&b.seg_start, bmax * msel * 4));
    BCHECK(hipMalloc((void **)&b.nseg, 16));
    if (h->kind == LEANN_BACKEND_DISKANN) {
        BCHECK(hipMalloc((void **)&b.exp_keys, bmax * EXPCAP * 8));
        BCHECK(hipMalloc((void **)&b.exp_cnt, bmax * 4));
    }
    size_t tmp = 0;
    BCHECK(hipcub::DeviceRadixSort::SortPairs(nullptr, tmp, b.prop_key, b.prop_key2, b.prop_src, b.prop_src2,
                                              (int)(bmax * msel), 0, 64, b.st));
    b.cub_bytes = tmp;
    BCHECK(hipMalloc(&b.cub_tmp, tmp));
    return LEANN_OK;
}

static int builder_insert_range(Builder &b, const std::vector<uint32_t> &order_host_upper , size_t s0, size_t n,
                                bool refine = false) {
    (void)order_host_upper;
    leann_backend *h = b.h;
    const uint32_t efc = h->efc;
    const bool hnsw = h->kind == LEANN_BACKEND_HNSW || h->nav_levels;
    size_t s = s0;
    const size_t bu_cap = (b.bmax / 16 + 64) * 16;
    while (s < n) {
        const size_t frac = b.batch_fraction;
        size_t B = std::min<size_t>(std::min<size_t>(b.bmax, refine ? b.bmax : std::max<size_t>(1, s / frac)), n - s);
        const uint32_t Lmax = h->g.max_level;
        struct LevelJob { uint32_t level, nq; size_t off; };
        std::vector<LevelJob> jobs;
        size_t offU = 0;
        if (hnsw && Lmax > 0) {
            for (uint32_t l = Lmax; l >= 1; --l) {
                std::vector<uint32_t> rows;
                for (size_t i = s; i < s + B; i++)
                    if (b.levels[b.order[i]] >= l) rows.push_back(b.order[i]);
                if (rows.empty()) continue;
                if (offU + rows.size() > bu_cap) {
                    leann_set_error("build: upper-level scratch exhausted");
                    return LEANN_ERR_DEVICE;
                }
                BCHECK(hipMemcpyAsync(b.d_rowsU + offU, rows.data(), rows.size() * 4, hipMemcpyHostToDevice, b.st));
                BCHECK(hipStreamSynchronize(b.st));
                SearchArgs a{};
                a.q_rows = b.d_rowsU + offU;
                a.nq = (uint32_t)rows.size();
                a.k = efc;
                a.ef = efc;
                a.target_level = l;
                a.out_keys = b.candU_keys + offU * efc;
                a.out_dists = b.candU_d + offU * efc;
                a.out_counts = b.candU_cnt + offU;
                int rc = leann_internal_launch_search(h, a, b.st);
                if (rc) return rc;
                jobs.push_back({l, (uint32_t)rows.size(), offU});
                offU += rows.size();
            }
        }
        {
            SearchArgs a{};
            a.q_rows = b.d_order + s;
            a.nq = (uint32_t)B;
            a.k = efc;
            a.ef = efc;
            a.target_level = 0;
            a.out_keys = b.cand_keys;
            a.out_dists = b.cand_d;
            a.out_counts = b.cand_cnt;
            a.out_expanded = b.exp_keys;
            a.out_nexp = b.exp_cnt;
            a.exp_cap = EXPCAP;
            int rc = leann_internal_launch_search(h, a, b.st);
            if (rc) return rc;
        }
        for (auto &j : jobs) {
            int rc = link_level(b, b.d_rowsU + j.off, j.nq, j.level, b.candU_keys + j.off * efc, b.candU_d + j.off * efc,
                                b.candU_cnt + j.off);
            if (rc) return rc;
        }
        int rc = link_level(b, b.d_order + s, (uint32_t)B, 0, b.cand_keys, b.cand_d, b.cand_cnt, b.exp_keys, b.exp_cnt);
        if (rc) return rc;
        if (hnsw)
            for (size_t i = s; i < s + B; i++)
                if (b.levels[b.order[i]] > h->g.max_level) { h->g.max_level = b.levels[b.order[i]]; h->g.entry = b.order[i]; }
        s += B;
    }
    BCHECK(hipStreamSynchronize(b.st));
    return LEANN_OK;
}

static uint32_t insertion_order(std::vector<uint32_t> &order, size_t lo, size_t n, const uint32_t *pin_first = nullptr) {
    order.resize(std::max<size_t>(n, 1));
    for (size_t i = 0; i < lo; i++) order[i] = (uint32_t)i;
    const uint64_t m = n - lo;
    if (m == 0) return 0;
    size_t w = lo;
    if (pin_first) order[w++] = *pin_first;
    std::vector<uint64_t> keyed(m);
    for (uint64_t j = 0; j < m; j++) keyed[j] = (mix64((lo + j) ^ 0x4F52444552ull) & 0xFFFFFFFF00000000ull) | (uint32_t)(lo + j);
    std::sort(keyed.begin(), keyed.end());
    for (uint64_t j = 0; j < m; j++) {
        const uint32_t pos = (uint32_t)keyed[j];
        if (pin_first && pos == *pin_first) continue;
        order[w++] = pos;
    }
    return order[lo];
}

static int build_on_device(leann_backend *h, size_t n_existing, size_t bmax_hint) {
    Builder b;
    b.h = h;
    b.batch_fraction = (size_t)env_int("LEANN_BUILD_BATCH_FRACTION", 8, 1, 1 << 20);
    const size_t n = h->g.n;
    BCHECK(hipStreamCreateWithFlags(&b.st, hipStreamNonBlocking));
    b.lv.adj0 = const_cast<uint32_t *>(h->g.adj0);
    b.lv.adjU = const_cast<uint32_t *>(h->g.adjU);
    b.lv.upper_off = h->g.upper_off;
    b.lv.M = h->g.M;
    b.lv.M0 = h->g.M0;
    const size_t nu = std::max<size_t>(h->n_upper_lists, 1);
    BCHECK(hipMalloc((void **)&b.adjd0, std::max<size_t>(n, 1) * h->g.M0 * 4));
    BCHECK(hipMalloc((void **)&b.adjdU, nu * h->g.M * 4));
    BCHECK(hipMemset(b.adjd0, 0, std::max<size_t>(n, 1) * h->g.M0 * 4));
    BCHECK(hipMemset(b.adjdU, 0, nu * h->g.M * 4));
    b.lv.adjd0 = b.adjd0;
    b.lv.adjdU = b.adjdU;
    if (h->kind == LEANN_BACKEND_DISKANN) {
        b.lv.two_stage = (uint32_t)env_int("LEANN_VAMANA_TWO_STAGE", 1, 0, 1);
        h->two_stage = b.lv.two_stage;
        const uint32_t slack = (uint32_t)env_int("LEANN_VAMANA_PENDING", 4, 0, 32);
        b.lv.P = slack;
        if (slack) {
            BCHECK(hipMalloc((void **)&b.pend, std::max<size_t>(n, 1) * slack * 4));
            BCHECK(hipMalloc((void **)&b.pendd, std::max<size_t>(n, 1) * slack * 4));
            BCHECK(hipMemset(b.pend, 0xFF, std::max<size_t>(n, 1) * slack * 4));
            BCHECK(hipMemset(b.pendd, 0, std::max<size_t>(n, 1) * slack * 4));
            b.lv.pend = b.pend;
            b.lv.pendd = b.pendd;
        }
    }
    b.levels.resize(std::max<size_t>(n, 1));
    BCHECK(hipMemcpy(b.levels.data(), h->d_levels, n, hipMemcpyDeviceToHost));
    BCHECK(hipMalloc((void **)&b.d_order, std::max<size_t>(n, 1) * 4));
    int rc = LEANN_OK;
    size_t s0 = n_existing;
    if (n_existing == 0 && n > 0) {
        uint32_t first = 0;
        if (h->kind == LEANN_BACKEND_DISKANN && !h->nav_levels) {
            DevTmp t_mean, t_mk, t_ms, t_mc, t_part;
            const uint32_t S = 1024;
            BCHECK(hipMalloc(&t_mean.p, h->g.ld * 4));
            BCHECK(hipMalloc(&t_mk.p, 8)); BCHECK(hipMalloc(&t_ms.p, 4)); BCHECK(hipMalloc(&t_mc.p, 4));
            BCHECK(hipMalloc(&t_part.p, (size_t)S * h->g.ld * 8));
            float *mean = (float *)t_mean.p; uint64_t *mk = (uint64_t *)t_mk.p; float *ms = (float *)t_ms.p; uint32_t *mc = (uint32_t *)t_mc.p;
            double *part = (double *)t_part.p;
            hipLaunchKernelGGL(col_partial_kernel, dim3((h->g.ld + 63) / 64, S), dim3(64), 0, b.st, h->g.X, n, h->g.d, h->g.ld, S, part);
            hipLaunchKernelGGL(col_mean_kernel, dim3((h->g.ld + 63) / 64), dim3(64), 0, b.st, part, n, h->g.ld, S, mean);
            BCHECK(hipStreamSynchronize(b.st));
            rc = leann_scan_topk_device(h->g.X, n, h->g.d, h->g.ld, mean, 1, 1, nullptr, 0, mk, ms, mc, b.st);
            if (rc) return rc;
            uint64_t key = 0;
            BCHECK(hipMemcpyAsync(&key, mk, 8, hipMemcpyDeviceToHost, b.st));
            BCHECK(hipStreamSynchronize(b.st));
            first = (uint32_t)key;
        }
        const bool leveled = h->kind == LEANN_BACKEND_HNSW || h->nav_levels;
        if (leveled) first = insertion_order(b.order, 0, n);
        else insertion_order(b.order, 0, n, &first);
        h->g.entry = first;
        h->g.max_level = leveled ? b.levels[first] : 0;
        s0 = 1;
    } else {
        insertion_order(b.order, n_existing, n);
        hipLaunchKernelGGL(link_dist_kernel, dim3((unsigned)((n_existing + 3) / 4)), dim3(256), 0, b.st, h->g.X, h->g.ld, b.lv, h->d_levels,
                           (uint32_t)n_existing);
        BCHECK(hipGetLastError());
    }
    BCHECK(hipMemcpyAsync(b.d_order, b.order.data(), n * 4, hipMemcpyHostToDevice, b.st));
    size_t bmax = bmax_hint ? bmax_hint : 16384;
    rc = builder_alloc_scratch(b, bmax);
    const int passes = env_int("LEANN_VAMANA_PASSES", 1, 1, 3);
    b.alpha_now = h->alpha;
    if (passes > 1 && h->kind == LEANN_BACKEND_DISKANN) {
        b.alpha_now = (float)env_int("LEANN_VAMANA_ALPHA1_PCT", (int)(h->alpha * 100.f + 0.5f), 100, 400) / 100.f;
    }
    if (rc == LEANN_OK) rc = builder_insert_range(b, {}, s0, n);
    for (int p = 1; rc == LEANN_OK && p < passes && h->kind == LEANN_BACKEND_DISKANN && n_existing == 0 && n > 1; p++) {
        if (p == passes - 1) b.alpha_now = h->alpha;
        rc = builder_insert_range(b, {}, 0, n, true);
    }
    b.alpha_now = h->alpha;
    if (rc == LEANN_OK && b.lv.P && n) {
        const float alpha = h->alpha;
        hipLaunchKernelGGL(std::max(h->g.M0, h->g.M) > 64 ? wide_reverse_merge_kernel : reverse_merge_kernel, dim3(256 * 16), dim3(256), 0,
                           b.st, h->g.X, h->g.ld, b.lv, 0u, (const uint64_t *)nullptr,
                           (const uint32_t *)nullptr, 0u, (const uint32_t *)nullptr, (const uint32_t *)nullptr, alpha, (uint32_t)n);
        BCHECK(hipGetLastError());
        BCHECK(hipStreamSynchronize(b.st));
    }
    return rc;
}

static int alloc_graph_arrays(leann_backend *h, uint64_t level_seed) {
    const size_t n = h->g.n, nn = std::max<size_t>(n, 1);
    std::vector<uint8_t> levels(nn, 0);
    std::vector<uint32_t> uo(nn, 0);
    uint64_t nu = 0;
    for (size_t i = 0; i < n; i++) {
        levels[i] = (h->kind == LEANN_BACKEND_HNSW || h->nav_levels) ? (uint8_t)node_level(level_seed, i, h->g.M) : 0;
        uo[i] = (uint32_t)nu;
        nu += levels[i];
    }
    h->n_upper_lists = nu;
    uint32_t *adj0 = nullptr, *adjU = nullptr, *duo = nullptr;
    BCHECK(hipMalloc((void **)&adj0, nn * h->g.M0 * 4));
    BCHECK(hipMalloc((void **)&adjU, std::max<uint64_t>(nu, 1) * h->g.M * 4));
    BCHECK(hipMalloc((void **)&duo, nn * 4));
    BCHECK(hipMalloc((void **)&h->d_levels, nn));
    BCHECK(hipMemset(adj0, 0xFF, nn * h->g.M0 * 4));
    BCHECK(hipMemset(adjU, 0xFF, std::max<uint64_t>(nu, 1) * h->g.M * 4));
    BCHECK(hipMemcpy(duo, uo.data(), nn * 4, hipMemcpyHostToDevice));
    BCHECK(hipMemcpy(h->d_levels, levels.data(), nn, hipMemcpyHostToDevice));
    h->g.adj0 = adj0;
    h->g.adjU = adjU;
    h->g.upper_off = duo;
    return LEANN_OK;
}

static constexpr uint64_t LEVEL_SEED = 0x5EED0003ull;

static int build_device_impl(int backend, const float *d_vectors, size_t n, size_t dims, size_t ld, size_t graph_degree, size_t complexity,
                             int device, uint64_t key_offset, int take_copy, leann_backend **out);
static int check_degree(int backend, size_t graph_degree, size_t complexity) {
    const size_t maxdeg = backend == LEANN_BACKEND_HNSW ? 64 : 128;
    if (graph_degree < 2 || graph_degree > maxdeg || complexity < 1) {
        leann_set_error("build: graph_degree must be in [2, %zu] (%s) and complexity >= 1 (got %zu, %zu)", maxdeg,
                        backend == LEANN_BACKEND_HNSW ? "hnsw" : "diskann", graph_degree, complexity);
        return LEANN_ERR_INVALID;
    }
    return LEANN_OK;
}
extern "C" int leann_backend_build_device(int backend, const float *d_vectors, size_t n, size_t dims, size_t ld,
                                          size_t graph_degree, size_t complexity, int device, uint64_t key_offset,
                                          int take_copy, leann_backend **out) {
    try {
        return build_device_impl(backend, d_vectors, n, dims, ld, graph_degree, complexity, device, key_offset, take_copy, out);
    } catch (const std::exception &e) {
        leann_set_error("build: %s", e.what());
        return LEANN_ERR_DEVICE;
    }
}
static int build_device_impl(int backend, const float *d_vectors, size_t n, size_t dims, size_t ld, size_t graph_degree, size_t complexity,
                             int device, uint64_t key_offset, int take_copy, leann_backend **out) {
    if (!out || (n && !d_vectors) || dims == 0 || dims > 4096 || ld < dims || (ld & 3) || n >= (1ull << 31)) {
        leann_set_error("leann_backend_build_device: invalid arguments (n=%zu dims=%zu ld=%zu)", n, dims, ld);
        return LEANN_ERR_INVALID;
    }
    if (backend != LEANN_BACKEND_HNSW && backend != LEANN_BACKEND_DISKANN) {
        leann_set_error("Unknown backend: %d", backend);
        return LEANN_ERR_INVALID;
    }
    if (int rc = check_degree(backend, graph_degree, complexity)) return rc;
    int ndev = 0;
    leann_device_count(&ndev);
    if (device < 0 || device >= ndev) {
        leann_set_error("HIP device %d not available (%d visible). This library has no CPU fallback.", device, ndev);
        return LEANN_ERR_DEVICE;
    }
    BCHECK(hipSetDevice(device));
    leann_backend *h = new leann_backend();
    h->kind = backend;
    h->device = device;
    h->key_offset = key_offset;
    h->efc = (uint32_t)std::max<size_t>(complexity, graph_degree);
    h->alpha = 1.2f;
    h->g.n = n;
    h->g.d = (uint32_t)dims;
    h->g.ld = (uint32_t)ld;
    h->g.M = (uint32_t)graph_degree;
    h->g.M0 = backend == LEANN_BACKEND_HNSW ? (uint32_t)(2 * graph_degree) : (uint32_t)graph_degree;
    h->nav_levels = backend == LEANN_BACKEND_DISKANN && env_int("LEANN_VAMANA_NAV", 0, 0, 1) != 0;
    if (take_copy) {
        float *cp = nullptr;
        if (hipMalloc((void **)&cp, std::max<size_t>(n * ld, 4) * 4) != hipSuccess ||
            (n && hipMemcpy(cp, d_vectors, n * ld * 4, hipMemcpyDeviceToDevice) != hipSuccess)) {
            leann_set_error("build: copying %zu rows failed: %s", n, hipGetErrorString(hipGetLastError()));
            (void)hipFree(cp);
            h->owns_rows = false;
            leann_backend_close(h);
            return LEANN_ERR_DEVICE;
        }
        h->g.X = cp;
        h->owns_rows = true;
    } else {
        h->g.X = d_vectors;
        h->owns_rows = false;
    }
    int rc = alloc_graph_arrays(h, LEVEL_SEED);
    if (rc == LEANN_OK && n) rc = build_on_device(h, 0, 0);
    if (rc) { leann_backend_close(h); return rc; }
    *out = h;
    return LEANN_OK;
}

extern "C" int leann_backend_build(int backend, const float *vectors, size_t n, size_t dims, size_t graph_degree,
                                   size_t complexity, const char *index_path_stem) {
    if (!index_path_stem || (n && !vectors) || dims == 0) {
        leann_set_error("leann_backend_build: invalid arguments");
        return LEANN_ERR_INVALID;
    }
    if (backend != LEANN_BACKEND_HNSW && backend != LEANN_BACKEND_DISKANN) {
        leann_set_error("Unknown backend: %d", backend);
        return LEANN_ERR_INVALID;
    }
    if (int rc = check_degree(backend, graph_degree, complexity)) return rc;
    int ndev = 0;
    leann_device_count(&ndev);
    if (ndev < 1) {
        leann_set_error("no HIP device visible. This library has no CPU fallback.");
        return LEANN_ERR_DEVICE;
    }
    BCHECK(hipSetDevice(0));
    const size_t ld = (dims + 3) & ~(size_t)3;
    float *dX = nullptr;
    BCHECK(hipMalloc((void **)&dX, std::max<size_t>(n * ld, 4) * 4));
    if (n) {
        if (ld == dims) BCHECK(hipMemcpy(dX, vectors, n * dims * 4, hipMemcpyHostToDevice));
        else {
            BCHECK(hipMemset(dX, 0, n * ld * 4));
            BCHECK(hipMemcpy2D(dX, ld * 4, vectors, dims * 4, dims * 4, n, hipMemcpyHostToDevice));
        }
    }
    leann_backend *h = nullptr;
    int rc = leann_backend_build_device(backend, dX, n, dims, ld, graph_degree, complexity, 0, 0, 0, &h);
    if (rc) { (void)hipFree(dX); return rc; }
    h->owns_rows = true;
    rc = leann_backend_save(h, index_path_stem);
    leann_backend_close(h);
    return rc;
}

extern "C" int leann_backend_add(int backend, const float *vectors, size_t n, size_t dims, size_t start_id,
                                 const char *index_path_stem) {
    if (backend == LEANN_BACKEND_DISKANN) {
        leann_set_error("DiskANN backend does not support incremental updates. Use --force to rebuild the entire index.");
        return LEANN_ERR_UNSUPPORTED;
    }
    if (backend != LEANN_BACKEND_HNSW || !index_path_stem || (n && !vectors)) {
        leann_set_error("leann_backend_add: invalid arguments");
        return LEANN_ERR_INVALID;
    }
    leann_backend *old = nullptr;
    int rc = leann_backend_open(index_path_stem, backend, dims, "0", &old);
    if (rc) return rc;
    const size_t n_old = old->g.n;
    std::vector<uint8_t> tomb = old->removed;
    const size_t tomb_n = old->n_removed;
    if (tomb_n) tomb.resize((n_old + n + 7) / 8, 0);
    if (old->g.feat_h) {
        leann_set_error("add_to_index: this index stores no vectors (recompute-on); rebuild it from the encoder inputs (leann_recompute_build_index)");
        leann_backend_close(old);
        return LEANN_ERR_UNSUPPORTED;
    }
    if (start_id != n_old) {
        leann_set_error("add_to_index: start_id %zu does not continue the index (%zu vectors)", start_id, n_old);
        leann_backend_close(old);
        return LEANN_ERR_INVALID;
    }
    const size_t ld = old->g.ld, nt = n_old + n;
    float *dX = nullptr;
    if (hipMalloc((void **)&dX, std::max<size_t>(nt * ld, 4) * 4) != hipSuccess ||
        (n_old && hipMemcpy(dX, old->g.X, n_old * ld * 4, hipMemcpyDeviceToDevice) != hipSuccess) ||
        (n && (hipMemset(dX + n_old * ld, 0, n * ld * 4) != hipSuccess ||
               hipMemcpy2D(dX + n_old * ld, ld * 4, vectors, dims * 4, dims * 4, n, hipMemcpyHostToDevice) != hipSuccess))) {
        leann_set_error("add_to_index: staging %zu rows on the device failed: %s", nt, hipGetErrorString(hipGetLastError()));
        (void)hipFree(dX);
        leann_backend_close(old);
        return LEANN_ERR_DEVICE;
    }
    leann_backend *h = new leann_backend();
    h->kind = backend;
    h->device = old->device;
    h->key_offset = old->key_offset;
    h->efc = old->efc;
    h->alpha = old->alpha;
    h->g = old->g;
    h->g.X = dX;
    h->g.n = nt;
    h->g.adj0 = nullptr; h->g.adjU = nullptr; h->g.upper_off = nullptr;
    h->owns_rows = true;
    rc = alloc_graph_arrays(h, LEVEL_SEED);
    bool same_levels = true;
    if (rc == LEANN_OK && n_old) {
        std::vector<uint8_t> la(n_old), lb(n_old);
        if (hipMemcpy(la.data(), old->d_levels, n_old, hipMemcpyDeviceToHost) != hipSuccess ||
            hipMemcpy(lb.data(), h->d_levels, n_old, hipMemcpyDeviceToHost) != hipSuccess) {
            leann_set_error("add_to_index: reading the level tables failed");
            rc = LEANN_ERR_DEVICE;
        } else {
            same_levels = la == lb;
        }
    }
    if (rc == LEANN_OK && !same_levels) {
        const size_t M = old->g.M, efc = old->efc;
        leann_backend_close(old);
        h->g.X = nullptr;
        h->owns_rows = false;
        leann_backend_close(h);
        rc = leann_backend_build_device(backend, dX, nt, dims, ld, M, efc, 0, 0, 0, &h);
        if (rc) { (void)hipFree(dX); return rc; }
        h->owns_rows = true;
        if (tomb_n) rc = leann_internal_set_removed(h, tomb.data(), tomb_n);
        if (rc == LEANN_OK) rc = leann_backend_save(h, index_path_stem);
        leann_backend_close(h);
        return rc;
    }
    if (rc == LEANN_OK && n_old) {
        if (hipMemcpy(const_cast<uint32_t *>(h->g.adj0), old->g.adj0, n_old * h->g.M0 * 4, hipMemcpyDeviceToDevice) != hipSuccess ||
            (old->n_upper_lists && hipMemcpy(const_cast<uint32_t *>(h->g.adjU), old->g.adjU, old->n_upper_lists * h->g.M * 4,
                                             hipMemcpyDeviceToDevice) != hipSuccess)) {
            leann_set_error("add_to_index: copying the existing graph failed");
            rc = LEANN_ERR_DEVICE;
        }
    }
    const size_t old_lists = old->n_upper_lists;
    leann_backend_close(old);
    if (rc == LEANN_OK && old_lists > h->n_upper_lists) { leann_set_error("add_to_index: inconsistent level table"); rc = LEANN_ERR_INVALID; }
    if (rc == LEANN_OK && n) rc = build_on_device(h, n_old, 0);
    if (rc == LEANN_OK && tomb_n) rc = leann_internal_set_removed(h, tomb.data(), tomb_n);
    if (rc) { leann_backend_close(h); return rc; }
    h->owns_rows = true;
    rc = leann_backend_save(h, index_path_stem);
    leann_backend_close(h);
    return rc;
}
```

### leann-rs_amd/csrc/internal.h

```cpp
#pragma once
#include "search.cuh"
#include "../../include/leann_backend.h"
#include <atomic>
#include <map>
#include <memory>
#include <mutex>
#include <string>
#include <vector>

struct Workspace {
    float *d_q = nullptr;
    uint64_t *d_keys = nullptr;
    float *d_dists = nullptr;
    uint32_t *d_counts = nullptr, *d_stats = nullptr;
    uint8_t *d_allow = nullptr;
    size_t cap_q = 0, cap_keys = 0, cap_dists = 0, cap_counts = 0, cap_stats = 0, cap_allow = 0;
    unsigned char *pin = nullptr;
    size_t cap_pin = 0;
    hipStream_t stream = nullptr;
};

struct LeannKnobs {
    int hash_bits = 0;
    int nw = 0;
    int gpool_bits = 0, gpool2_bits = 0;
    bool no_feat256 = false, no_zero_copy = false, no_emit = false, fused_v1 = false, no_list = false, no_tiled = false;
    bool force_remote = false;
    bool coalesce_off = false;
    bool hnsw_reference_ef = false;
    unsigned long long stamp_buf = 0;
};
const LeannKnobs &leann_knobs();
extern "C" void leann_debug_reload_env(void);

struct Coalescer;
struct leann_sharded;
struct leann_backend {
    leann_sharded *sharded = nullptr;
    int kind = LEANN_BACKEND_HNSW, device = 0;
    GraphView g{};
    uint64_t key_offset = 0;
    bool owns_rows = true;
    uint8_t *d_levels = nullptr;
    uint32_t efc = 64;
    float alpha = 1.2f;
    uint32_t fixed_ef = leann_knobs().hnsw_reference_ef ? 64u : 0u;
    bool nav_levels = false;
    uint64_t n_upper_lists = 0;
    std::mutex mu;
    std::vector<Workspace *> free_ws;
    unsigned long long *gpool = nullptr, *gpool2 = nullptr;
    uint32_t *gpool_lock = nullptr, *gpool_ctr = nullptr, *gpool2_lock = nullptr;
    uint32_t gpool_bits = GPOOL_BITS, gpool_tables = GPOOL_TABLES, gpool2_bits = 0, gpool2_tables = 0;
    leann_search_stats stats{};
    float *Wf32 = nullptr;
    std::map<hipStream_t, std::pair<float *, size_t>> proj_scratch;
    std::shared_ptr<Coalescer> coalescer;
    int coalesce_mode = 0;
    std::atomic<int> singles_in_flight{0};
    std::vector<uint8_t> removed;
    uint8_t *d_live = nullptr;
    size_t n_removed = 0, n_pending = 0;
    uint64_t removal_epoch = 0;
    uint32_t two_stage = 1;
    std::map<hipStream_t, std::pair<uint8_t *, size_t>> live_scratch;
};
int leann_internal_live_allow(leann_backend *h, const uint8_t *d_allow, size_t allow_stride, size_t nq, bool walk, hipStream_t st,
                              const uint8_t **out, size_t *out_stride);
int leann_internal_set_removed(leann_backend *h, const uint8_t *bitmap, size_t n_removed);
void leann_internal_free_removed(leann_backend *h);
std::string leann_internal_tombstone_file(const std::string &index_file);
int leann_internal_tombstones_save(const leann_backend *h, const std::string &index_file);
int leann_internal_tombstones_load(leann_backend *h, const std::string &index_file);

enum { LEANN_LOG_ERROR = 0, LEANN_LOG_WARN = 1, LEANN_LOG_INFO = 2, LEANN_LOG_DEBUG = 3 };
void leann_log(int level, const char *fmt, ...) __attribute__((format(printf, 2, 3)));
int leann_internal_from_host(int backend, size_t n, size_t dims, uint32_t M, uint32_t M0, uint32_t max_level, uint32_t entry,
                             const uint8_t *levels, const uint32_t *upper_off, const uint32_t *adj0, const uint32_t *adjU,
                             size_t n_upper_lists, const float *vectors, const unsigned char *feat_rows, uint32_t feat_h, uint32_t row_bytes,
                             const float *Wf32, int device, uint64_t key_offset, leann_backend **out);
int leann_internal_save_to(const leann_backend *h, const std::string &path);
int leann_internal_parse_device(const char *spec, int *device);
bool leann_internal_spec_is_sharded(const char *spec);
int leann_internal_open_sharded_backend(const char *stem, int backend, size_t dims, const char *spec, leann_backend **out);
size_t leann_internal_sharded_count(const leann_sharded *s);
leann_backend *leann_internal_sharded_shard(const leann_sharded *s, size_t g);
struct leann_filter {
    int device = 0;
    size_t n = 0, n_allowed = 0;
    uint8_t *d_allow = nullptr;
    uint32_t *d_list = nullptr;
    uint64_t epoch = 0;
    std::vector<leann_filter *> parts;
};
struct SearchFilter {
    const uint8_t *d_allow = nullptr;
    size_t allow_stride = 0;
    const leann_filter *registered = nullptr;
    bool exact = false;
};
inline int leann_internal_check_allow_stride(const SearchFilter &f, size_t n) {
    if (f.d_allow && f.allow_stride && f.allow_stride < (n + 7) / 8) {
        leann_set_error("filtered search: allow_stride %zu is smaller than the %zu-byte bitmap", f.allow_stride, (n + 7) / 8);
        return LEANN_ERR_INVALID;
    }
    return LEANN_OK;
}
__attribute__((visibility("hidden"))) int leann_internal_search_plain(leann_backend *h, const float *d_queries, size_t nq, size_t top_k, size_t complexity, const SearchFilter &f,
                                uint64_t *d_keys, float *d_dists, uint32_t *d_counts, uint32_t *d_stats, hipStream_t st);
int leann_internal_sharded_search(leann_sharded *s, const float *d_queries, size_t nq, size_t top_k, size_t complexity, const SearchFilter &f,
                                  uint64_t *d_keys, float *d_dists, uint32_t *d_counts, uint32_t *d_stats, hipStream_t st, uint64_t *ticket);
int leann_internal_sharded_save(const leann_sharded *s, const char *index_path_stem);
uint64_t leann_internal_sharded_lo(const leann_sharded *s, size_t g);
int leann_internal_filtered_exact_list(const float *d_rows, size_t dims, size_t ld, const float *d_queries, size_t nq, size_t top_k,
                                       const uint32_t *d_list, size_t m, uint64_t key_offset, uint64_t *d_keys, float *d_dists,
                                       uint32_t *d_counts, hipStream_t st);
int leann_internal_filtered_exact(const float *d_rows, size_t n, size_t dims, size_t ld, const float *d_queries, size_t nq, size_t top_k,
                                  const uint8_t *d_allow, size_t allow_stride, uint64_t key_offset, uint64_t *d_keys, float *d_dists,
                                  uint32_t *d_counts, hipStream_t st);
int leann_internal_compact_allow(const uint8_t *d_allow, size_t n, uint32_t **d_list, size_t *n_list, hipStream_t st);
int leann_internal_and_live_inplace(const leann_backend *h, uint8_t *d_bitmap);
void leann_internal_scratch_release(void *p);
extern "C" void leann_sharded_close(leann_sharded *s);

int leann_internal_launch_search(leann_backend *h, SearchArgs a, hipStream_t st);
size_t leann_internal_effective_complexity(const leann_backend *h, size_t complexity);

struct CandEmit {
    const float *thr;
    uint32_t *cnt;
    uint64_t *list;
    uint32_t cap;
    const uint8_t *allow;
    uint64_t pos0;
};
int leann_internal_fold_candidates(const CandEmit &em, uint32_t k, uint32_t nq, uint32_t slots, uint64_t *best, uint32_t *d_overflow,
                                   hipStream_t st);
int leann_internal_score(const float *X, size_t rows, size_t dims, size_t ld, const float *d_queries, size_t nq, size_t ldq, float *S,
                         hipStream_t st);
void leann_internal_free_graph(leann_backend *h);
size_t leann_internal_feat_file_row_bytes(const GraphView &g);
int leann_internal_feat_rows_to_host(const leann_backend *h, size_t r0, size_t rows, unsigned char *out);
std::string leann_internal_index_file(const char *stem, int backend);
std::string leann_internal_with_extension(const std::string &stem, const char *ext);
```

### leann-rs_amd/csrc/search.cuh

```cuda
#pragma once
#include "common.cuh"

struct GraphView {
    const float *X;
    const uint32_t *adj0;
    const uint32_t *adjU;
    const uint32_t *upper_off;
    uint64_t n;
    uint32_t d, ld, M, M0, max_level, entry;
    uint32_t feat_h, row_bytes;
    const float *norms;
};

#define GPOOL_TABLES 1024u
#define GPOOL_BITS 16u

struct SearchArgs {
    const float *queries;
    const uint32_t *q_rows;
    uint32_t ldq, nq, k, ef, target_level;
    uint32_t hash_bits;
    uint64_t key_offset;
    uint64_t *out_keys;
    float *out_dists;
    uint32_t *out_counts;
    uint32_t *out_stats;
    uint64_t *out_expanded;
    uint32_t *out_nexp;
    uint32_t exp_cap;
    unsigned long long *gpool;
    uint32_t *gpool_lock;
    uint32_t *gpool_ctr;
    uint32_t gpool_bits, gpool_tables;
    unsigned long long *gpool2;
    uint32_t *gpool2_lock;
    uint32_t gpool2_bits, gpool2_tables;
    const uint8_t *allow;
    uint64_t allow_stride;
};

static_assert(alignof(SearchArgs) == 8 && alignof(GraphView) == 8, "lazy_search_args assumes `a` sits at the 8-byte aligned offset behind `g`");
__device__ __forceinline__ const __attribute__((address_space(4))) SearchArgs *lazy_search_args() {
    typedef const __attribute__((address_space(4))) char *kptr;
    return (const __attribute__((address_space(4))) SearchArgs *)((kptr)__builtin_amdgcn_kernarg_segment_ptr() +
                                                                  ((sizeof(GraphView) + 7) & ~(size_t)7));
}

__device__ __forceinline__ uint32_t uni(uint32_t v) { return (uint32_t)__builtin_amdgcn_readfirstlane((int)v); }

__device__ __forceinline__ uint32_t vis_hash(uint32_t id, uint32_t bits) {
    return (id * 0x9E3779B1u) >> (32 - bits);
}

__device__ __forceinline__ bool vis_insert_lds(uint32_t *tab, uint32_t bits, uint32_t id) {
    const uint32_t mask = (1u << bits) - 1u;
    uint32_t h = vis_hash(id, bits);
    for (;;) {
        uint32_t old = atomicCAS(&tab[h], LEANN_EMPTY, id);
        if (old == LEANN_EMPTY) return true;
        if (old == id) return false;
        h = (h + 1) & mask;
    }
}
__device__ __forceinline__ bool vis_insert_hbm(unsigned long long *tab, uint32_t bits, uint32_t gen, uint32_t id) {
    const uint32_t mask = (1u << bits) - 1u;
    uint32_t h = vis_hash(id, bits);
    const unsigned long long mine = ((unsigned long long)gen << 32) | id;
    for (;;) {
        unsigned long long cur = __hip_atomic_load(&tab[h], __ATOMIC_RELAXED, __HIP_MEMORY_SCOPE_AGENT);
        if ((uint32_t)(cur >> 32) != gen) {
            unsigned long long prev = atomicCAS(&tab[h], cur, mine);
            if (prev == cur) return true;
            continue;
        }
        if ((uint32_t)cur == id) return false;
        h = (h + 1) & mask;
    }
}

template <int T, int R>
__device__ __forceinline__ void wave_dist_rows(const float4 (&q)[T], const float *__restrict__ X, uint32_t ld,
                                               const uint32_t (&ids)[R], int nrows, int lane, float (&out)[R]) {
    float4 v[R][T];
#pragma unroll
    for (int r = 0; r < R; r++) {
        if (r < nrows) {
            const float *row = X + (size_t)ids[r] * ld;
#pragma unroll
            for (int t = 0; t < T; t++) v[r][t] = row_load4(row, ld, t, lane);
        }
    }
#pragma unroll
    for (int r = 0; r < R; r++) {
        if (r < nrows) {
            float4 acc = make_float4(0.f, 0.f, 0.f, 0.f);
#pragma unroll
            for (int t = 0; t < T; t++) fma4(acc, q[t], v[r][t]);
            out[r] = 1.0f - wave_tree_sum(lane4_sum(acc));
        }
    }
}

template <int T, int R>
__device__ __forceinline__ void wave_dist_rows_feat(const float4 (&q)[T], const char *__restrict__ Xb, uint32_t row_bytes,
                                                    uint32_t h, const uint32_t (&ids)[R], int nrows, int lane, float (&out)[R],
                                                    const float *__restrict__ norms = nullptr) {
    uint2 v[R][T];
    float nrm[R];
#pragma unroll
    for (int r = 0; r < R; r++) {
        if (r < nrows) {
            const char *row = Xb + (size_t)ids[r] * row_bytes;
#pragma unroll
            for (int t = 0; t < T; t++) {
                const uint32_t j = 256u * t + 4u * lane;
                v[r][t] = j < h ? *reinterpret_cast<const uint2 *>(row + 2 * (size_t)j) : make_uint2(0u, 0u);
            }
            nrm[r] = norms ? norms[ids[r]] : *reinterpret_cast<const float *>(row + 2 * (size_t)h);
        }
    }
#pragma unroll
    for (int r = 0; r < R; r++) {
        if (r < nrows) {
            float4 acc = make_float4(0.f, 0.f, 0.f, 0.f);
#pragma unroll
            for (int t = 0; t < T; t++) {
                float4 x;
                x.x = __uint_as_float(v[r][t].x << 16);
                x.y = __uint_as_float(v[r][t].x & 0xFFFF0000u);
                x.z = __uint_as_float(v[r][t].y << 16);
                x.w = __uint_as_float(v[r][t].y & 0xFFFF0000u);
                fma4(acc, q[t], x);
            }
            out[r] = 1.0f - wave_tree_sum(lane4_sum(acc)) / nrm[r];
        }
    }
}

typedef uint32_t u32x4_a8 __attribute__((ext_vector_type(4), aligned(8)));
__device__ __forceinline__ float feat8_partial_pair(const float (&q)[8], const u32x4_a8 v) {
    float4 lo, hi;
    lo.x = fmaf(q[0], __uint_as_float(v.x << 16), 0.f);
    lo.y = fmaf(q[1], __uint_as_float(v.x & 0xFFFF0000u), 0.f);
    lo.z = fmaf(q[2], __uint_as_float(v.y << 16), 0.f);
    lo.w = fmaf(q[3], __uint_as_float(v.y & 0xFFFF0000u), 0.f);
    hi.x = fmaf(q[4], __uint_as_float(v.z << 16), 0.f);
    hi.y = fmaf(q[5], __uint_as_float(v.z & 0xFFFF0000u), 0.f);
    hi.z = fmaf(q[6], __uint_as_float(v.w << 16), 0.f);
    hi.w = fmaf(q[7], __uint_as_float(v.w & 0xFFFF0000u), 0.f);
    return lane4_sum(lo) + lane4_sum(hi);
}
template <int G>
__device__ __forceinline__ void group_dist_rows_feat256(const float (&qa)[8], const float (&qb)[8], const char *__restrict__ Xb,
                                                        uint32_t row_bytes, const uint32_t (&id)[G], const bool (&valid)[G], int lane,
                                                        float (&out)[G], const float *__restrict__ norms) {
    const int m = lane & 15;
    u32x4_a8 va[G], vb[G];
    float nrm[G];
#pragma unroll
    for (int g = 0; g < G; g++) {
        va[g] = vb[g] = u32x4_a8{0u, 0u, 0u, 0u};
        nrm[g] = 1.f;
        if (valid[g]) {
            const char *row = Xb + (size_t)id[g] * row_bytes;
            va[g] = *reinterpret_cast<const u32x4_a8 *>(row + 16 * m);
            vb[g] = *reinterpret_cast<const u32x4_a8 *>(row + 256 + 16 * m);
            if (m == 15) nrm[g] = norms ? norms[id[g]] : *reinterpret_cast<const float *>(row + 512);
        }
    }
#pragma unroll
    for (int g = 0; g < G; g++) {
        float sa = feat8_partial_pair(qa, va[g]), sb = feat8_partial_pair(qb, vb[g]);
        sa = dpp_pair_add<0xB1, 0xf>(sa);
        sb = dpp_pair_add<0xB1, 0xf>(sb);
        sa = dpp_pair_add<0x4E, 0xf>(sa);
        sb = dpp_pair_add<0x4E, 0xf>(sb);
        sa = dpp_pair_add<0x114, 0xf>(sa);
        sb = dpp_pair_add<0x114, 0xf>(sb);
        sa = dpp_pair_add<0x118, 0xf>(sa);
        sb = dpp_pair_add<0x118, 0xf>(sb);
        out[g] = 1.0f - (sa + sb) / nrm[g];
    }
}

__device__ __forceinline__ const uint32_t *adj_list(const uint32_t *__restrict__ base, const uint32_t *__restrict__ upper_off, uint32_t deg,
                                                    int lv, uint32_t node) {
    const size_t list = lv == 0 ? (size_t)node : (size_t)upper_off[node] + (uint32_t)(lv - 1);
    return base + list * deg;
}

struct SearchLds {
    uint64_t *s_key;
    uint32_t *s_new;
    uint32_t *misc;
};
__host__ __device__ inline size_t search_lds_bytes(uint32_t ef, uint32_t maxdeg, uint32_t hash_bits, uint32_t kf = 0, uint32_t nbuf = 2) {
    size_t efp = (ef + 1) & ~1u;
    size_t b = 2 * efp * 8 + nbuf * ((size_t)maxdeg + 8) * 8 + nbuf * (size_t)maxdeg * 4 + 16 * 4;
    b = (b + 15) & ~(size_t)15;
    if (kf) b += 2 * (size_t)((kf + 1) & ~1u) * 8 + nbuf * ((size_t)maxdeg + 8) * 8;
    return b + ((size_t)1 << hash_bits) * 4;
}

template <int T, int R, int NW, bool FEAT, bool FILT = false, bool G16 = false, int LW = 1>
__device__ void beam_search_one(const GraphView &g, const SearchArgs &a, uint32_t qi, unsigned char *smem) {
    const int tid = threadIdx.x, lane = tid & 63, wave = tid >> 6;
    const auto *const za = lazy_search_args();
    const uint32_t ef = a.ef;
    static_assert(LW == 1 || LW == 2, "lists of at most 128 ids");
    const uint32_t maxdeg = g.M0 > g.M ? g.M0 : g.M;
    const uint32_t efp = (ef + 1) & ~1u;
    SearchLds s;
    uint64_t *const W0 = reinterpret_cast<uint64_t *>(smem);
    constexpr uint32_t NBUF = NW > 4 ? 2u : 1u;
    const uint32_t kstride = maxdeg + 8;
    s.s_key = W0 + 2 * efp;
    s.s_new = reinterpret_cast<uint32_t *>(s.s_key + NBUF * kstride);
    s.misc = s.s_new + NBUF * maxdeg;
    size_t off = 2 * (size_t)efp * 8 + NBUF * ((size_t)maxdeg + 8) * 8 + NBUF * (size_t)maxdeg * 4 + 64;
    off = (off + 15) & ~(size_t)15;
    const uint32_t kf = FILT ? a.k : 0u, kfp = (kf + 1) & ~1u;
    uint64_t *const R0 = reinterpret_cast<uint64_t *>(smem + off);
    uint64_t *const s_keyR = R0 + 2 * kfp;
    const uint8_t *const allow = FILT ? a.allow + (size_t)qi * a.allow_stride : nullptr;
    uint32_t rsize = 0;
    int rcur = 0;
    if (FILT) off += 2 * (size_t)kfp * 8 + NBUF * ((size_t)maxdeg + 8) * 8;
    uint32_t *table = reinterpret_cast<uint32_t *>(smem + off);
    const uint32_t hbits = a.hash_bits, hsize = 1u << hbits;
    uint32_t vis_limit = hsize - (hsize >> 2);
    uint32_t hbm = 0;
    unsigned long long *gtab = nullptr;
    uint32_t gslot = 0, gen = 0, gbits = 0;

    float4 q[T];
    float qa[8], qb[8];
    {
        const float *qv;
        uint32_t dq = FEAT ? g.feat_h : g.d;
        if (!FEAT && a.q_rows) qv = g.X + (size_t)a.q_rows[qi] * g.ld;
        else qv = a.queries + (size_t)qi * a.ldq;
#pragma unroll
        for (int t = 0; t < T; t++)
            if (!G16) q[t] = vec_load4_guard(qv, dq, t, lane);
        if (G16) {
#pragma unroll
            for (int i = 0; i < 8; i++) {
                qa[i] = qv[8 * (lane & 15) + i];
                qb[i] = qv[128 + 8 * (lane & 15) + i];
            }
        }
    }

    const uint32_t *const adj0_p = g.adj0, *const adjU_p = g.adjU, *const upoff_p = g.upper_off;
    uint32_t n_evals = 1, hops0 = 0, hopsU = 0;
    uint32_t n_vis = 0;
    uint64_t best;
    {
        uint32_t ids[1] = {g.entry};
        float dd[1];
        if (G16) {
            const bool valid[1] = {lane < 16};
            group_dist_rows_feat256<1>(qa, qb, reinterpret_cast<const char *>(g.X), g.row_bytes, ids, valid, lane, dd, g.norms);
            dd[0] = __int_as_float(__builtin_amdgcn_readlane(__float_as_int(dd[0]), 15));
        } else if (FEAT) wave_dist_rows_feat<T, 1>(q, reinterpret_cast<const char *>(g.X), g.row_bytes, g.feat_h, ids, 1, lane, dd, g.norms);
        else wave_dist_rows<T, 1>(q, g.X, g.ld, ids, 1, lane, dd);
        best = make_key(dd[0], g.entry);
    }

#ifdef LEANN_STAMPS
    uint64_t stamp[8] = {0, 0, 0, 0, 0, 0, 0, 0};
#endif
    uint32_t wsize = 0, level_hops = 0;
    int cur = 0;
    bool aborted = false;
    for (int lv = (int)g.max_level; lv >= (int)a.target_level; --lv) {
        const uint32_t ef_l = (lv == (int)a.target_level) ? ef : 1u;
        const uint32_t deg = lv == 0 ? g.M0 : g.M;
        if (!hbm)
            for (uint32_t i = tid; i < hsize; i += NW * 64) table[i] = LEANN_EMPTY;
        __syncthreads();
        if (tid == 0) {
            W0[0] = best;
            if (hbm) {
                gen = atomicAdd(&za->gpool_ctr[1], 1u) + 1u;
                s.misc[5] = gen;
                vis_insert_hbm(gtab, gbits, gen, key_id(best));
            } else {
                table[vis_hash(key_id(best), hbits)] = key_id(best);
            }
            s.misc[1] = LEANN_EMPTY;
            s.misc[2] = LEANN_EMPTY;
            s.misc[3] = 0;
            if (FILT && lv == (int)a.target_level) {
                const uint32_t e = key_id(best);
                const uint32_t ok = (allow[e >> 3] >> (e & 7)) & 1u;
                if (ok) R0[0] = best;
                s.misc[6] = ok;
            }
        }
        __syncthreads();
        if (hbm) gen = uni(s.misc[5]);
        const bool filt_level = FILT && lv == (int)a.target_level;
        if (filt_level) { rsize = uni(s.misc[6]); rcur = 0; }
        cur = 0;
        wsize = 1;
        n_vis = 1;
        uint32_t sel = 0;
        uint32_t hop = 0;
        constexpr bool EARLY_B = NW > 4;
        if constexpr (!EARLY_B) {
            uint32_t e_pref = LEANN_EMPTY, e_pref1 = LEANN_EMPTY;
            const uint32_t *const adj_base = lv == 0 ? adj0_p : adjU_p;
            if (wave == 0) {
                e_pref = (uint32_t)lane < deg ? adj_list(adj_base, upoff_p, deg, lv, key_id(best))[lane] : LEANN_EMPTY;
                if constexpr (LW == 2) e_pref1 = (uint32_t)lane + 64u < deg ? adj_list(adj_base, upoff_p, deg, lv, key_id(best))[lane + 64] : LEANN_EMPTY;
            }
            while (sel != LEANN_EMPTY) {
                uint64_t *Wc = W0 + cur * efp, *Wn = W0 + (cur ^ 1) * efp;
    #ifdef LEANN_STAMPS
                const uint64_t st0 = __builtin_amdgcn_s_memtime();
    #endif
                if (wave == 0) {
                    const uint32_t node = key_id(Wc[sel]);
                    if (za->out_expanded && lv == (int)a.target_level && lane == 0 && hop < za->exp_cap)
                        za->out_expanded[(size_t)qi * za->exp_cap + hop] = ((Wc[sel] >> 32) << 32) | node;
                    uint32_t n_new = 0;
                    bool ovf = (n_vis + deg > vis_limit);
                    if (!ovf) {
                        const uint32_t e = e_pref;
                        bool isnew = false;
                        if (e != LEANN_EMPTY) isnew = hbm ? vis_insert_hbm(gtab, gbits, gen, e) : vis_insert_lds(table, hbits, e);
                        unsigned long long m = __ballot(isnew);
                        uint32_t pos = __popcll(m & ((1ull << lane) - 1ull));
                        if (isnew) s.s_new[pos] = e;
                        n_new = __popcll(m);
                        if constexpr (LW == 2) {
                            const uint32_t e1 = e_pref1;
                            bool isnew1 = false;
                            if (e1 != LEANN_EMPTY) isnew1 = hbm ? vis_insert_hbm(gtab, gbits, gen, e1) : vis_insert_lds(table, hbits, e1);
                            const unsigned long long m1 = __ballot(isnew1);
                            if (isnew1) s.s_new[n_new + __popcll(m1 & ((1ull << lane) - 1ull))] = e1;
                            n_new += __popcll(m1);
                        }
                    }
                    n_vis += n_new;
                    n_evals += n_new;
                    if (!ovf) { if (lv == 0) hops0++; else hopsU++; }
                    if (lane < 8) s.s_key[n_new + lane] = ~0ull;
                    if (filt_level && lane < 8) s_keyR[n_new + lane] = ~0ull;
                    if (lane == 0) {
                        s.misc[0] = n_new;
                        if (ovf) s.misc[3] = 1;
                    }
                }
    #ifdef LEANN_STAMPS
                const uint64_t stB = __builtin_amdgcn_s_memtime();
    #endif
                __syncthreads();
    #ifdef LEANN_STAMPS
                const uint64_t stB1 = __builtin_amdgcn_s_memtime();
    #endif
                const uint32_t table_full = uni(s.misc[3]);
                if (table_full) {
                    const uint32_t next = hbm + 1;
                    if (next > 2 || (next == 2 && !za->gpool2)) { aborted = true; break; }
                    __syncthreads();
                    if (tid == 0) {
                        uint32_t *locks = next == 1 ? za->gpool_lock : za->gpool2_lock;
                        const uint32_t ntab = next == 1 ? za->gpool_tables : za->gpool2_tables;
                        uint32_t t = atomicAdd(&za->gpool_ctr[next == 1 ? 0 : 2], 1u), slot;
                        for (uint32_t i = 0;; i++) {
                            slot = (t + i) % ntab;
                            if (atomicCAS(&locks[slot], 0u, 1u) == 0u) break;
                            if ((i % ntab) == ntab - 1) __builtin_amdgcn_s_sleep(32);
                        }
                        s.misc[4] = slot;
                        if (!hbm) s.misc[5] = atomicAdd(&za->gpool_ctr[1], 1u) + 1u;
                        s.misc[3] = 0;
                    }
                    __syncthreads();
                    const uint32_t nslot = uni(s.misc[4]);
                    const uint32_t nbits = next == 1 ? za->gpool_bits : za->gpool2_bits;
                    unsigned long long *ntab_p = (next == 1 ? za->gpool : za->gpool2) + ((size_t)nslot << nbits);
                    if (!hbm) {
                        gen = uni(s.misc[5]);
                        for (uint32_t i = tid; i < hsize; i += NW * 64) {
                            uint32_t e = table[i];
                            if (e != LEANN_EMPTY) vis_insert_hbm(ntab_p, nbits, gen, e);
                        }
                    } else {
                        for (uint32_t i = tid; i < (1u << gbits); i += NW * 64) {
                            const unsigned long long cur = __hip_atomic_load(&gtab[i], __ATOMIC_RELAXED, __HIP_MEMORY_SCOPE_AGENT);
                            if ((uint32_t)(cur >> 32) == gen) vis_insert_hbm(ntab_p, nbits, gen, (uint32_t)cur);
                        }
                        __syncthreads();
                        if (tid == 0) atomicExch(&za->gpool_lock[gslot], 0u);
                    }
                    gtab = ntab_p;
                    gbits = nbits;
                    gslot = nslot;
                    hbm = next;
                    vis_limit = (1u << gbits) - (1u << (gbits - 2));
                    __syncthreads();
                    continue;
                }
                const uint32_t n_new = uni(s.misc[0]);
                if constexpr (G16) {
                    for (uint32_t jb = 0; jb < n_new; jb += NW * 4 * R) {
                        uint32_t ids[R], jj[R], abyte[R];
                        bool valid[R];
                        float dd[R];
    #pragma unroll
                        for (int r = 0; r < R; r++) {
                            jj[r] = jb + (uint32_t)(r * NW + wave) * 4u + (uint32_t)(lane >> 4);
                            valid[r] = jj[r] < n_new;
                            ids[r] = valid[r] ? s.s_new[jj[r]] : 0u;
                            abyte[r] = (filt_level && valid[r] && (lane & 15) == 15) ? allow[ids[r] >> 3] : 0u;
                        }
                        group_dist_rows_feat256<R>(qa, qb, reinterpret_cast<const char *>(g.X), g.row_bytes, ids, valid, lane, dd, g.norms);
                        if ((lane & 15) == 15) {
    #pragma unroll
                            for (int r = 0; r < R; r++)
                                if (valid[r]) {
                                    const uint64_t key = make_key(dd[r], ids[r]);
                                    s.s_key[jj[r]] = key;
                                    if (filt_level) s_keyR[jj[r]] = ((abyte[r] >> (ids[r] & 7u)) & 1u) ? key : ~0ull;
                                }
                        }
                    }
                } else
                for (uint32_t j0 = wave; j0 < n_new; j0 += NW * R) {
                    uint32_t ids[R];
                    float dd[R];
                    int nrows = 0;
    #pragma unroll
                    for (int r = 0; r < R; r++) {
                        uint32_t j = j0 + r * NW;
                        if (j < n_new) { ids[r] = s.s_new[j]; nrows = r + 1; }
                    }
                    uint32_t abyte = 0, abit = 0;
                    if (filt_level && lane < R && j0 + lane * NW < n_new) {
                        const uint32_t e = s.s_new[j0 + lane * NW];
                        abyte = allow[e >> 3];
                        abit = e & 7u;
                    }
                    if (FEAT) wave_dist_rows_feat<T, R>(q, reinterpret_cast<const char *>(g.X), g.row_bytes, g.feat_h, ids, nrows, lane, dd, g.norms);
                    else wave_dist_rows<T, R>(q, g.X, g.ld, ids, nrows, lane, dd);
                    const unsigned long long amask = FILT ? __ballot((abyte >> abit) & 1u) : 0ull;
                    if (lane == 0) {
    #pragma unroll
                        for (int r = 0; r < R; r++)
                            if (r < nrows) {
                                const uint64_t key = make_key(dd[r], ids[r]);
                                s.s_key[j0 + r * NW] = key;
                                if (filt_level) s_keyR[j0 + r * NW] = ((amask >> r) & 1ull) ? key : ~0ull;
                            }
                    }
                }
    #ifdef LEANN_STAMPS
                const uint64_t stC = __builtin_amdgcn_s_memtime();
    #endif
                __syncthreads();
    #ifdef LEANN_STAMPS
                const uint64_t stB2 = __builtin_amdgcn_s_memtime();
    #endif
                uint32_t *next_slot = &s.misc[1 + (hop & 1)];
                const uint32_t n_pad = (n_new + 7) & ~7u;
                if (wave == 0) {
                    uint32_t u = LEANN_EMPTY;
                    for (uint32_t base = 0; base < wsize && u == LEANN_EMPTY; base += 64) {
                        const uint32_t i = base + lane;
                        const unsigned long long m = __ballot(i < wsize && i != sel && !(Wc[i] & 1ull));
                        if (m) u = base + (uint32_t)__ffsll((long long)m) - 1u;
                    }
                    const uint64_t c_old = u != LEANN_EMPTY ? Wc[u] : ~0ull;
                    const uint64_t kj = (uint32_t)lane < n_new ? s.s_key[lane] : ~0ull;
                    const uint64_t kj1 = LW == 2 && (uint32_t)lane + 64u < n_new ? s.s_key[lane + 64] : ~0ull;
                    const uint64_t km = LW == 2 ? min(kj, kj1) : kj;
                    const uint32_t hi = wave_min_u32((uint32_t)(km >> 32));
                    const uint32_t lo = wave_min_u32((uint32_t)(km >> 32) == hi ? (uint32_t)km : 0xFFFFFFFFu);
                    const uint64_t c_new = n_new ? (((uint64_t)hi << 32) | lo) : ~0ull;
                    uint32_t next = LEANN_EMPTY, cnode = 0;
                    if (c_old != ~0ull || c_new != ~0ull) {
                        uint32_t rank;
                        if ((c_old >> 1) < (c_new >> 1)) {
                            rank = u + (uint32_t)__popcll(__ballot((kj >> 1) < (c_old >> 1)));
                            if constexpr (LW == 2) rank += (uint32_t)__popcll(__ballot((kj1 >> 1) < (c_old >> 1)));
                            cnode = key_id(c_old);
    #ifdef LEANN_STAMPS
                            stamp[7] += 1;
    #endif
                        } else {
                            rank = 0;
                            for (uint32_t base = 0; base < wsize; base += 64) {
                                const uint32_t i = base + lane;
                                rank += (uint32_t)__popcll(__ballot(i < wsize && (Wc[i] >> 1) < (c_new >> 1)));
                            }
                            cnode = key_id(c_new);
                        }
                        if (rank < ef_l) next = rank;
                    }
                    if (lane == 0) *next_slot = next;
                    if (next != LEANN_EMPTY) {
                        e_pref = (uint32_t)lane < deg ? adj_list(adj_base, upoff_p, deg, lv, cnode)[lane] : LEANN_EMPTY;
                        if constexpr (LW == 2) e_pref1 = (uint32_t)lane + 64u < deg ? adj_list(adj_base, upoff_p, deg, lv, cnode)[lane + 64] : LEANN_EMPTY;
                    }
                } else {
                    const ulonglong2 *kp = reinterpret_cast<const ulonglong2 *>(s.s_key);
                    for (uint32_t it = tid - 64; it < wsize + n_new; it += (NW - 1) * 64) {
                        const bool isW = it < wsize;
                        uint64_t k = isW ? Wc[it] : s.s_key[it - wsize];
                        if (isW && it == sel) k |= 1ull;
                        const uint64_t kk = k >> 1;
                        uint32_t cnt = 0;
    #pragma unroll 4
                        for (uint32_t j = 0; j < n_pad; j += 2) {
                            const ulonglong2 v = kp[j >> 1];
                            cnt += ((v.x >> 1) < kk) + ((v.y >> 1) < kk);
                        }
                        uint32_t rank = isW ? it + cnt : cnt;
                        if (!isW) {
                            uint32_t lo = 0, hi = wsize;
                            while (lo < hi) {
                                uint32_t mid = (lo + hi) >> 1;
                                if ((Wc[mid] >> 1) < kk) lo = mid + 1; else hi = mid;
                            }
                            rank += lo;
                        }
                        if (rank < ef_l) Wn[rank] = k;
                    }
                }
                if (filt_level) {
                    uint64_t *Rc = R0 + rcur * kfp, *Rn = R0 + (rcur ^ 1) * kfp;
                    const uint64_t thr = rsize == kf ? Rc[kf - 1] : ~0ull;
                    uint32_t n_in = 0;
                    for (uint32_t j = 0; j < n_new; j += 64) n_in += __popcll(__ballot(j + lane < n_new && s_keyR[j + lane] < thr));
                    if (n_in) {
                        const ulonglong2 *kr = reinterpret_cast<const ulonglong2 *>(s_keyR);
                        for (uint32_t it = tid; it < rsize + n_new; it += NW * 64) {
                            const bool isR = it < rsize;
                            const uint64_t k = isR ? Rc[it] : s_keyR[it - rsize];
                            if (k >= thr && !isR) continue;
                            uint32_t cnt = 0;
    #pragma unroll 4
                            for (uint32_t j = 0; j < n_pad; j += 2) {
                                const ulonglong2 v = kr[j >> 1];
                                cnt += (v.x < k) + (v.y < k);
                            }
                            uint32_t rank = isR ? it + cnt : cnt;
                            if (!isR) {
                                uint32_t lo = 0, hi = rsize;
                                while (lo < hi) {
                                    uint32_t mid = (lo + hi) >> 1;
                                    if (Rc[mid] < k) lo = mid + 1; else hi = mid;
                                }
                                rank += lo;
                            }
                            if (rank < kf) Rn[rank] = k;
                        }
                        rsize = min(rsize + n_in, kf);
                        rcur ^= 1;
                    }
                }
    #ifdef LEANN_STAMPS
                const uint64_t stD = __builtin_amdgcn_s_memtime();
    #endif
                __syncthreads();
    #ifdef LEANN_STAMPS
                {
                    const uint64_t stE = __builtin_amdgcn_s_memtime();
                    stamp[0] += stB - st0; stamp[1] += stB1 - stB; stamp[2] += stC - stB1; stamp[3] += stB2 - stC;
                    stamp[4] += stD - stB2; stamp[5] += stE - stD; stamp[6] += 1;
                }
    #endif
                sel = uni(*next_slot);
                wsize = min(wsize + n_new, ef_l);
                cur ^= 1;
                hop++;
            }
        } else {
            const uint32_t *const adj_base = lv == 0 ? adj0_p : adjU_p;
            uint32_t e_pref = LEANN_EMPTY, e_pref1 = LEANN_EMPTY;
            auto phase_b = [&](uint32_t p, uint64_t ckey, uint32_t hidx) __attribute__((always_inline)) {
                uint64_t *skey = s.s_key + p * kstride;
                uint32_t *snew = s.s_new + p * maxdeg;
                const uint32_t node = key_id(ckey);
                if (za->out_expanded && lv == (int)a.target_level && lane == 0 && hidx < za->exp_cap)
                    za->out_expanded[(size_t)qi * za->exp_cap + hidx] = ((ckey >> 32) << 32) | node;
                uint32_t n_new = 0;
                const bool ovf = (n_vis + deg > vis_limit);
                if (!ovf) {
                    const uint32_t e = e_pref;
                    bool isnew = false;
                    if (e != LEANN_EMPTY) isnew = hbm ? vis_insert_hbm(gtab, gbits, gen, e) : vis_insert_lds(table, hbits, e);
                    const unsigned long long m = __ballot(isnew);
                    const uint32_t pos = __popcll(m & ((1ull << lane) - 1ull));
                    if (isnew) snew[pos] = e;
                    n_new = __popcll(m);
                    if constexpr (LW == 2) {
                        const uint32_t e1 = e_pref1;
                        bool isnew1 = false;
                        if (e1 != LEANN_EMPTY) isnew1 = hbm ? vis_insert_hbm(gtab, gbits, gen, e1) : vis_insert_lds(table, hbits, e1);
                        const unsigned long long m1 = __ballot(isnew1);
                        if (isnew1) snew[n_new + __popcll(m1 & ((1ull << lane) - 1ull))] = e1;
                        n_new += __popcll(m1);
                    }
                }
                n_vis += n_new;
                n_evals += n_new;
                if (!ovf) { if (lv == 0) hops0++; else hopsU++; }
                if (lane < 8) skey[n_new + lane] = ~0ull;
                if (filt_level && lane < 8) (s_keyR + p * kstride)[n_new + lane] = ~0ull;
                if (lane == 0) {
                    s.misc[8 + p] = n_new;
                    if (ovf) s.misc[3] = 1;
                }
            };
            if (wave == 0) {
                e_pref = (uint32_t)lane < deg ? adj_list(adj_base, upoff_p, deg, lv, key_id(best))[lane] : LEANN_EMPTY;
                if constexpr (LW == 2) e_pref1 = (uint32_t)lane + 64u < deg ? adj_list(adj_base, upoff_p, deg, lv, key_id(best))[lane + 64] : LEANN_EMPTY;
                phase_b(0u, best, 0u);
            }
            __syncthreads();
            uint32_t par = 0;
            for (;;) {
                uint64_t *Wc = W0 + cur * efp, *Wn = W0 + (cur ^ 1) * efp;
#ifdef LEANN_STAMPS
                const uint64_t st0 = __builtin_amdgcn_s_memtime();
#endif
                if (uni(s.misc[3])) {
                    const uint32_t next = hbm + 1;
                    if (next > 2 || (next == 2 && !za->gpool2)) { aborted = true; break; }
                    __syncthreads();
                    if (tid == 0) {
                        uint32_t *locks = next == 1 ? za->gpool_lock : za->gpool2_lock;
                        const uint32_t ntab = next == 1 ? za->gpool_tables : za->gpool2_tables;
                        uint32_t t = atomicAdd(&za->gpool_ctr[next == 1 ? 0 : 2], 1u), slot;
                        for (uint32_t i = 0;; i++) {
                            slot = (t + i) % ntab;
                            if (atomicCAS(&locks[slot], 0u, 1u) == 0u) break;
                            if ((i % ntab) == ntab - 1) __builtin_amdgcn_s_sleep(32);
                        }
                        s.misc[4] = slot;
                        if (!hbm) s.misc[5] = atomicAdd(&za->gpool_ctr[1], 1u) + 1u;
                        s.misc[3] = 0;
                    }
                    __syncthreads();
                    const uint32_t nslot = uni(s.misc[4]);
                    const uint32_t nbits = next == 1 ? za->gpool_bits : za->gpool2_bits;
                    unsigned long long *ntab_p = (next == 1 ? za->gpool : za->gpool2) + ((size_t)nslot << nbits);
                    if (!hbm) {
                        gen = uni(s.misc[5]);
                        for (uint32_t i = tid; i < hsize; i += NW * 64) {
                            uint32_t e = table[i];
                            if (e != LEANN_EMPTY) vis_insert_hbm(ntab_p, nbits, gen, e);
                        }
                    } else {
                        for (uint32_t i = tid; i < (1u << gbits); i += NW * 64) {
                            const unsigned long long cur_e = __hip_atomic_load(&gtab[i], __ATOMIC_RELAXED, __HIP_MEMORY_SCOPE_AGENT);
                            if ((uint32_t)(cur_e >> 32) == gen) vis_insert_hbm(ntab_p, nbits, gen, (uint32_t)cur_e);
                        }
                        __syncthreads();
                        if (tid == 0) atomicExch(&za->gpool_lock[gslot], 0u);
                    }
                    gtab = ntab_p;
                    gbits = nbits;
                    gslot = nslot;
                    hbm = next;
                    vis_limit = (1u << gbits) - (1u << (gbits - 2));
                    __syncthreads();
                    if (wave == 0) phase_b(par, Wc[sel], hop);
                    __syncthreads();
                    continue;
                }
                const uint32_t n_new = uni(s.misc[8 + par]);
                uint64_t *const skey = s.s_key + par * kstride;
                const uint32_t *const snew = s.s_new + par * maxdeg;
                uint64_t *const skeyR = s_keyR + par * kstride;
                if constexpr (G16) {
                    for (uint32_t jb = 0; jb < n_new; jb += NW * 4 * R) {
                        uint32_t ids[R], jj[R], abyte[R];
                        bool valid[R];
                        float dd[R];
#pragma unroll
                        for (int r = 0; r < R; r++) {
                            jj[r] = jb + (uint32_t)(r * NW + wave) * 4u + (uint32_t)(lane >> 4);
                            valid[r] = jj[r] < n_new;
                            ids[r] = valid[r] ? snew[jj[r]] : 0u;
                            abyte[r] = (filt_level && valid[r] && (lane & 15) == 15) ? allow[ids[r] >> 3] : 0u;
                        }
#ifndef LEANN_NO_ADJ_TOUCH
                        uint32_t touch = 0;
                        if (lv == 0 && valid[0] && (lane & 14) == 12 && (uint32_t)(lane & 1) * 32u < deg)
                            touch = adj0_p[(size_t)ids[0] * deg + (uint32_t)(lane & 1) * 32u];
#endif
                        group_dist_rows_feat256<R>(qa, qb, reinterpret_cast<const char *>(g.X), g.row_bytes, ids, valid, lane, dd, g.norms);
#ifndef LEANN_NO_ADJ_TOUCH
                        asm volatile("" ::"v"(touch));
#endif
                        if ((lane & 15) == 15) {
#pragma unroll
                            for (int r = 0; r < R; r++)
                                if (valid[r]) {
                                    const uint64_t key = make_key(dd[r], ids[r]);
                                    skey[jj[r]] = key;
                                    if (filt_level) skeyR[jj[r]] = ((abyte[r] >> (ids[r] & 7u)) & 1u) ? key : ~0ull;
                                }
                        }
                    }
                } else
                for (uint32_t j0 = wave; j0 < n_new; j0 += NW * R) {
                    uint32_t ids[R];
                    float dd[R];
                    int nrows = 0;
#pragma unroll
                    for (int r = 0; r < R; r++) {
                        uint32_t j = j0 + r * NW;
                        if (j < n_new) { ids[r] = snew[j]; nrows = r + 1; }
                    }
                    uint32_t abyte = 0, abit = 0;
                    if (filt_level && lane < R && j0 + lane * NW < n_new) {
                        const uint32_t e = snew[j0 + lane * NW];
                        abyte = allow[e >> 3];
                        abit = e & 7u;
                    }
#ifndef LEANN_NO_ADJ_TOUCH
                    uint32_t touch = 0;
                    if (lv == 0 && (uint32_t)(lane >> 1) < (uint32_t)nrows && (uint32_t)(lane & 1) * 32u < deg)
                        touch = adj0_p[(size_t)snew[j0 + (uint32_t)(lane >> 1) * NW] * deg + (uint32_t)(lane & 1) * 32u];
#endif
                    if (FEAT) wave_dist_rows_feat<T, R>(q, reinterpret_cast<const char *>(g.X), g.row_bytes, g.feat_h, ids, nrows, lane, dd, g.norms);
                    else wave_dist_rows<T, R>(q, g.X, g.ld, ids, nrows, lane, dd);
#ifndef LEANN_NO_ADJ_TOUCH
                    asm volatile("" ::"v"(touch));
#endif
                    const unsigned long long amask = FILT ? __ballot((abyte >> abit) & 1u) : 0ull;
                    if (lane == 0) {
#pragma unroll
                        for (int r = 0; r < R; r++)
                            if (r < nrows) {
                                const uint64_t key = make_key(dd[r], ids[r]);
                                skey[j0 + r * NW] = key;
                                if (filt_level) skeyR[j0 + r * NW] = ((amask >> r) & 1ull) ? key : ~0ull;
                            }
                    }
                }
#ifdef LEANN_STAMPS
                const uint64_t stC = __builtin_amdgcn_s_memtime();
#endif
                __syncthreads();
#ifdef LEANN_STAMPS
                const uint64_t stB2 = __builtin_amdgcn_s_memtime();
#endif
                uint32_t *next_slot = &s.misc[1 + (hop & 1)];
                const uint32_t n_pad = (n_new + 7) & ~7u;
                if (wave == 0) {
                    uint32_t u = LEANN_EMPTY;
                    for (uint32_t base = 0; base < wsize && u == LEANN_EMPTY; base += 64) {
                        const uint32_t i = base + lane;
                        const unsigned long long m = __ballot(i < wsize && i != sel && !(Wc[i] & 1ull));
                        if (m) u = base + (uint32_t)__ffsll((long long)m) - 1u;
                    }
                    const uint64_t c_old = u != LEANN_EMPTY ? Wc[u] : ~0ull;
                    const uint64_t kj = (uint32_t)lane < n_new ? skey[lane] : ~0ull;
                    const uint64_t kj1 = LW == 2 && (uint32_t)lane + 64u < n_new ? skey[lane + 64] : ~0ull;
                    const uint64_t km = LW == 2 ? min(kj, kj1) : kj;
                    const uint32_t hi = wave_min_u32((uint32_t)(km >> 32));
                    const uint32_t lo = wave_min_u32((uint32_t)(km >> 32) == hi ? (uint32_t)km : 0xFFFFFFFFu);
                    const uint64_t c_new = n_new ? (((uint64_t)hi << 32) | lo) : ~0ull;
                    uint32_t next = LEANN_EMPTY;
                    uint64_t ckey = 0;
                    if (c_old != ~0ull || c_new != ~0ull) {
                        uint32_t rank;
                        if ((c_old >> 1) < (c_new >> 1)) {
                            rank = u + (uint32_t)__popcll(__ballot((kj >> 1) < (c_old >> 1)));
                            if constexpr (LW == 2) rank += (uint32_t)__popcll(__ballot((kj1 >> 1) < (c_old >> 1)));
                            ckey = c_old;
#ifdef LEANN_STAMPS
                            stamp[7] += 1;
#endif
                        } else {
                            rank = 0;
                            for (uint32_t base = 0; base < wsize; base += 64) {
                                const uint32_t i = base + lane;
                                rank += (uint32_t)__popcll(__ballot(i < wsize && (Wc[i] >> 1) < (c_new >> 1)));
                            }
                            ckey = c_new;
                        }
                        if (rank < ef_l) next = rank;
                    }
                    if (lane == 0) *next_slot = next;
                    if (next != LEANN_EMPTY) {
                        e_pref = (uint32_t)lane < deg ? adj_list(adj_base, upoff_p, deg, lv, key_id(ckey))[lane] : LEANN_EMPTY;
                        if constexpr (LW == 2) e_pref1 = (uint32_t)lane + 64u < deg ? adj_list(adj_base, upoff_p, deg, lv, key_id(ckey))[lane + 64] : LEANN_EMPTY;
                        phase_b(par ^ 1u, ckey, hop + 1);
                    }
                } else {
                    const ulonglong2 *kp = reinterpret_cast<const ulonglong2 *>(skey);
                    for (uint32_t it = tid - 64; it < wsize + n_new; it += (NW - 1) * 64) {
                        const bool isW = it < wsize;
                        uint64_t k = isW ? Wc[it] : skey[it - wsize];
                        if (isW && it == sel) k |= 1ull;
                        const uint64_t kk = k >> 1;
                        uint32_t cnt = 0;
#pragma unroll 4
                        for (uint32_t j = 0; j < n_pad; j += 2) {
                            const ulonglong2 v = kp[j >> 1];
                            cnt += ((v.x >> 1) < kk) + ((v.y >> 1) < kk);
                        }
                        uint32_t rank = isW ? it + cnt : cnt;
                        if (!isW) {
                            uint32_t lo = 0, hi = wsize;
                            while (lo < hi) {
                                uint32_t mid = (lo + hi) >> 1;
                                if ((Wc[mid] >> 1) < kk) lo = mid + 1; else hi = mid;
                            }
                            rank += lo;
                        }
                        if (rank < ef_l) Wn[rank] = k;
                    }
                }
                if (filt_level) {
                    uint64_t *Rc = R0 + rcur * kfp, *Rn = R0 + (rcur ^ 1) * kfp;
                    const uint64_t thr = rsize == kf ? Rc[kf - 1] : ~0ull;
                    uint32_t n_in = 0;
                    for (uint32_t j = 0; j < n_new; j += 64) n_in += __popcll(__ballot(j + lane < n_new && skeyR[j + lane] < thr));
                    if (n_in) {
                        const ulonglong2 *kr = reinterpret_cast<const ulonglong2 *>(skeyR);
                        for (uint32_t it = tid; it < rsize + n_new; it += NW * 64) {
                            const bool isR = it < rsize;
                            const uint64_t k = isR ? Rc[it] : skeyR[it - rsize];
                            if (k >= thr && !isR) continue;
                            uint32_t cnt = 0;
#pragma unroll 4
                            for (uint32_t j = 0; j < n_pad; j += 2) {
                                const ulonglong2 v = kr[j >> 1];
                                cnt += (v.x < k) + (v.y < k);
                            }
                            uint32_t rank = isR ? it + cnt : cnt;
                            if (!isR) {
                                uint32_t lo = 0, hi = rsize;
                                while (lo < hi) {
                                    uint32_t mid = (lo + hi) >> 1;
                                    if (Rc[mid] < k) lo = mid + 1; else hi = mid;
                                }
                                rank += lo;
                            }
                            if (rank < kf) Rn[rank] = k;
                        }
                        rsize = min(rsize + n_in, kf);
                        rcur ^= 1;
                    }
                }
#ifdef LEANN_STAMPS
                const uint64_t stD = __builtin_amdgcn_s_memtime();
#endif
                __syncthreads();
#ifdef LEANN_STAMPS
                {
                    const uint64_t stE = __builtin_amdgcn_s_memtime();
                    stamp[0] += 0; stamp[1] += 0; stamp[2] += stC - st0; stamp[3] += stB2 - stC;
                    stamp[4] += stD - stB2; stamp[5] += stE - stD; stamp[6] += 1;
                }
#endif
                sel = uni(*next_slot);
                wsize = min(wsize + n_new, ef_l);
                cur ^= 1;
                hop++;
                par ^= 1u;
                if (sel == LEANN_EMPTY) break;
            }
        }
        level_hops = hop;
        if (aborted) break;
        best = W0[cur * efp] & ~1ull;
        __syncthreads();
    }

    __syncthreads();
    if (hbm && tid == 0) atomicExch(&(hbm == 1 ? za->gpool_lock : za->gpool2_lock)[gslot], 0u);
    if (aborted) {
        for (uint32_t t = tid; t < za->k; t += NW * 64) {
            za->out_keys[(size_t)qi * za->k + t] = 0xFFFFFFFFFFFFFFFFull;
            za->out_dists[(size_t)qi * za->k + t] = __uint_as_float(0x7F800000u);
        }
        if (tid == 0) {
            za->out_counts[qi] = 0;
            if (za->out_stats) {
                za->out_stats[(size_t)qi * 4 + 0] = n_evals;
                za->out_stats[(size_t)qi * 4 + 1] = hops0;
                za->out_stats[(size_t)qi * 4 + 2] = hopsU;
                za->out_stats[(size_t)qi * 4 + 3] = 3u;
            }
        }
        return;
    }
    const uint32_t nout = FILT ? rsize : min(wsize, za->k);
    uint64_t *Wc = FILT ? R0 + rcur * kfp : W0 + cur * efp;
    for (uint32_t t = tid; t < za->k; t += NW * 64) {
        size_t o = (size_t)qi * za->k + t;
        if (t < nout) {
            uint64_t k = Wc[t];
            za->out_keys[o] = (uint64_t)key_id(k) + za->key_offset;
            za->out_dists[o] = key_dist(k);
        } else {
            za->out_keys[o] = 0xFFFFFFFFFFFFFFFFull;
            za->out_dists[o] = __uint_as_float(0x7F800000u);
        }
    }
#ifdef LEANN_STAMPS
    if (tid == 0 && za->out_expanded == nullptr && za->exp_cap == 0xFEED) {
        unsigned long long *dst = reinterpret_cast<unsigned long long *>(za->out_nexp) + (size_t)qi * 8;
        for (int i = 0; i < 8; i++) dst[i] = stamp[i];
    }
#endif
    if (tid == 0) {
        za->out_counts[qi] = nout;
        if (za->out_nexp && za->exp_cap != 0xFEED) za->out_nexp[qi] = min(level_hops, za->exp_cap);
        if (za->out_stats) {
            za->out_stats[(size_t)qi * 4 + 0] = n_evals;
            za->out_stats[(size_t)qi * 4 + 1] = hops0;
            za->out_stats[(size_t)qi * 4 + 2] = hopsU;
            za->out_stats[(size_t)qi * 4 + 3] = hbm;
        }
    }
    __syncthreads();
}

#ifndef LEANN_T2_OCC
#define LEANN_T2_OCC 6
#endif
#ifndef LEANN_T1_OCC
#define LEANN_T1_OCC 8
#endif
template <int T, int R, int NW, bool BUILD>
__global__ void __launch_bounds__(NW * 64, (NW == 4 && T == 2) ? LEANN_T2_OCC : (NW == 4 && T == 1) ? LEANN_T1_OCC : 1) beam_search_kernel(GraphView g, SearchArgs a) {
    extern __shared__ __attribute__((aligned(16))) unsigned char smem[];
    uint32_t qi = blockIdx.x;
    if (qi >= a.nq) return;
    beam_search_one<T, R, NW, false>(g, a, qi, smem);
}
template <int T, int R, int NW>
__global__ void __launch_bounds__(NW * 64) beam_search_filtered_kernel(GraphView g, SearchArgs a) {
    extern __shared__ __attribute__((aligned(16))) unsigned char smem[];
    uint32_t qi = blockIdx.x;
    if (qi >= a.nq) return;
    beam_search_one<T, R, NW, false, true>(g, a, qi, smem);
}
template <int T, int R, int NW>
__global__ void __launch_bounds__(NW * 64) beam_search_feat_filtered_kernel(GraphView g, SearchArgs a) {
    extern __shared__ __attribute__((aligned(16))) unsigned char smem[];
    uint32_t qi = blockIdx.x;
    if (qi >= a.nq) return;
    beam_search_one<T, R, NW, true, true>(g, a, qi, smem);
}
#ifndef LEANN_FEAT_OCC
#define LEANN_FEAT_OCC 8
#endif
#ifndef LEANN_FEAT_R1
#define LEANN_FEAT_R1 5
#endif
#ifndef LEANN_FEAT_G
#define LEANN_FEAT_G 1
#endif
#ifndef LEANN_FEAT256_OCC
#define LEANN_FEAT256_OCC 7
#endif
template <int G, int NW>
__global__ void __launch_bounds__(NW * 64, NW == 4 ? LEANN_FEAT256_OCC : 1) beam_search_feat256_kernel(GraphView g, SearchArgs a) {
    extern __shared__ __attribute__((aligned(16))) unsigned char smem[];
    uint32_t qi = blockIdx.x;
    if (qi >= a.nq) return;
    beam_search_one<1, G, NW, true, false, true>(g, a, qi, smem);
}
template <int G, int NW>
__global__ void __launch_bounds__(NW * 64) beam_search_feat256_filtered_kernel(GraphView g, SearchArgs a) {
    extern __shared__ __attribute__((aligned(16))) unsigned char smem[];
    uint32_t qi = blockIdx.x;
    if (qi >= a.nq) return;
    beam_search_one<1, G, NW, true, true, true>(g, a, qi, smem);
}
template <int T, int R, int NW>
__global__ void __launch_bounds__(NW * 64, (NW == 4 && T == 1) ? LEANN_FEAT_OCC : 1) beam_search_feat_kernel(GraphView g, SearchArgs a) {
    extern __shared__ __attribute__((aligned(16))) unsigned char smem[];
    uint32_t qi = blockIdx.x;
    if (qi >= a.nq) return;
    beam_search_one<T, R, NW, true>(g, a, qi, smem);
}

template <int T, int R, int NW, bool BUILD>
__global__ void __launch_bounds__(NW * 64) wide_beam_search_kernel(GraphView g, SearchArgs a) {
    extern __shared__ __attribute__((aligned(16))) unsigned char smem[];
    uint32_t qi = blockIdx.x;
    if (qi >= a.nq) return;
    beam_search_one<T, R, NW, false, false, false, 2>(g, a, qi, smem);
}
template <int T, int R, int NW>
__global__ void __launch_bounds__(NW * 64) wide_beam_search_filtered_kernel(GraphView g, SearchArgs a) {
    extern __shared__ __attribute__((aligned(16))) unsigned char smem[];
    uint32_t qi = blockIdx.x;
    if (qi >= a.nq) return;
    beam_search_one<T, R, NW, false, true, false, 2>(g, a, qi, smem);
}
template <int T, int R, int NW>
__global__ void __launch_bounds__(NW * 64) wide_beam_search_feat_kernel(GraphView g, SearchArgs a) {
    extern __shared__ __attribute__((aligned(16))) unsigned char smem[];
    uint32_t qi = blockIdx.x;
    if (qi >= a.nq) return;
    beam_search_one<T, R, NW, true, false, false, 2>(g, a, qi, smem);
}
template <int T, int R, int NW>
__global__ void __launch_bounds__(NW * 64) wide_beam_search_feat_filtered_kernel(GraphView g, SearchArgs a) {
    extern __shared__ __attribute__((aligned(16))) unsigned char smem[];
    uint32_t qi = blockIdx.x;
    if (qi >= a.nq) return;
    beam_search_one<T, R, NW, true, true, false, 2>(g, a, qi, smem);
}
template <int G, int NW>
__global__ void __launch_bounds__(NW * 64) wide_beam_search_feat256_kernel(GraphView g, SearchArgs a) {
    extern __shared__ __attribute__((aligned(16))) unsigned char smem[];
    uint32_t qi = blockIdx.x;
    if (qi >= a.nq) return;
    beam_search_one<1, G, NW, true, false, true, 2>(g, a, qi, smem);
}
template <int G, int NW>
__global__ void __launch_bounds__(NW * 64) wide_beam_search_feat256_filtered_kernel(GraphView g, SearchArgs a) {
    extern __shared__ __attribute__((aligned(16))) unsigned char smem[];
    uint32_t qi = blockIdx.x;
    if (qi >= a.nq) return;
    beam_search_one<1, G, NW, true, true, true, 2>(g, a, qi, smem);
}
```

Measured before the change: 1.117 million.

## Screen candidate rows on high-16-bit planes before reading full f32 rows

Splits each f32 vector into separate high-16 and low-16 bit planes. A new screened beam-search kernel first computes a lower bound on distance from the high halves plus an absolute-value error term, and reads the low plane only when the bound does not rule the candidate out against the current worst beam entry. This targets the memory bandwidth spent on full row reads during graph traversal for 768–1536-dim data. In exchange it stores an extra copy of the dataset, adds a split kernel at build or load time, and changes occupancy. It is auto-enabled only for datasets of at least 1 GiB.

```diff
diff --git a/include/leann_backend.h b/include/leann_backend.h
--- a/include/leann_backend.h
+++ b/include/leann_backend.h
@@ -57,6 +57,9 @@
 
 int leann_backend_set_coalescing(leann_backend *h, uint32_t wait_us, uint32_t max_batch);
 int leann_backend_coalescing_stats(const leann_backend *h, uint64_t *n_launches, uint64_t *n_queries);
+
+int leann_backend_set_row_screen(leann_backend *h, int enable);
+int leann_backend_row_screen_stats(const leann_backend *h, uint64_t out[2]);
 
 size_t leann_backend_len(const leann_backend *h);
 size_t leann_backend_dims(const leann_backend *h);
diff --git a/leann-rs_amd/_native.py b/leann-rs_amd/_native.py
--- a/leann-rs_amd/_native.py
+++ b/leann-rs_amd/_native.py
@@ -48,6 +48,8 @@
                                                      u64p, f32p, u32p]),
     "leann_backend_set_coalescing": (C.c_int, [vp, C.c_uint32, C.c_uint32]),
     "leann_backend_coalescing_stats": (C.c_int, [vp, u64p, u64p]),
+    "leann_backend_set_row_screen": (C.c_int, [vp, C.c_int]),
+    "leann_backend_row_screen_stats": (C.c_int, [vp, u64p]),
     "leann_backend_len": (C.c_size_t, [vp]),
     "leann_backend_dims": (C.c_size_t, [vp]),
     "leann_backend_close": (None, [vp]),
diff --git a/leann-rs_amd/backend.py b/leann-rs_amd/backend.py
--- a/leann-rs_amd/backend.py
+++ b/leann-rs_amd/backend.py
@@ -180,6 +180,14 @@
         N.check(N.lib().leann_backend_coalescing_stats(self._h, C.byref(a), C.byref(b)))
         return {"launches": a.value, "queries": b.value}
 
+    def set_row_screen(self, enable=True):
+        N.check(N.lib().leann_backend_set_row_screen(self._h, 1 if enable else 0))
+
+    def row_screen_stats(self):
+        out = (C.c_uint64 * 2)()
+        N.check(N.lib().leann_backend_row_screen_stats(self._h, out))
+        return {"ruled_out": int(out[0]), "read_in_full": int(out[1])}
+
     def len(self):
         return int(N.lib().leann_backend_len(self._h))
 
diff --git a/leann-rs_amd/csrc/api.hip b/leann-rs_amd/csrc/api.hip
--- a/leann-rs_amd/csrc/api.hip
+++ b/leann-rs_amd/csrc/api.hip
@@ -25,7 +25,7 @@
     va_end(ap);
 }
 extern "C" const char *leann_last_error(void) { return g_err; }
-void leann_log(int level, const char *fmt, ...) {
+bool leann_log_enabled(int level) {
     static const int threshold = [] {
         const char *e = getenv("LEANN_LOG");
         if (!e) return (int)LEANN_LOG_WARN;
@@ -34,7 +34,10 @@
         if (!strcasecmp(e, "debug") || !strcasecmp(e, "trace")) return (int)LEANN_LOG_DEBUG;
         return (int)LEANN_LOG_WARN;
     }();
-    if (level > threshold) return;
+    return level <= threshold;
+}
+void leann_log(int level, const char *fmt, ...) {
+    if (!leann_log_enabled(level)) return;
     static const char *names[] = {"ERROR", "WARN", "INFO", "DEBUG"};
     char buf[1024];
     va_list ap;
@@ -61,6 +64,7 @@
     k->no_tiled = flag("LEANN_RECOMPUTE_NO_TILED");
     k->hnsw_reference_ef = flag("LEANN_HNSW_REFERENCE_EF");
     k->force_remote = flag("LEANN_DEBUG_FORCE_REMOTE");
+    if (const char *e = getenv("LEANN_ROW_SCREEN")) k->row_screen = (!strcmp(e, "0") || !strcasecmp(e, "off")) ? 0 : (!strcmp(e, "1") || !strcasecmp(e, "on")) ? 2 : 1;
     if (const char *e = getenv("LEANN_COALESCE")) k->coalesce_off = !strcmp(e, "off") || !strcmp(e, "0");
     if (const char *e = getenv("LEANN_STAMP_BUF")) k->stamp_buf = strtoull(e, nullptr, 0);
     return k;
@@ -187,6 +191,7 @@
     (void)hipFree(h->Wf32);
     for (auto &kv : h->proj_scratch) (void)hipFree(kv.second.first);
     leann_internal_free_removed(h);
+    leann_internal_free_planes(h);
 }
 
 extern "C" void leann_backend_close(leann_backend *h) {
@@ -260,13 +265,26 @@
     return launch_one(k, NW * 64, lds, g, a, st);
 }
 
+#ifndef LEANN_SCREEN_R3
+#define LEANN_SCREEN_R3 4
+#endif
+#ifndef LEANN_SCREEN_R6
+#define LEANN_SCREEN_R6 2
+#endif
 template <int T, int R>
-static int launch_search_T(const GraphView &g, const SearchArgs &a, hipStream_t st) {
+static int launch_search_T(const GraphView &g, const SearchArgs &a, hipStream_t st, bool screen = false) {
     int nw = a.nq <= 384 ? 16 : a.nq <= 640 ? 8 : 4;
     if (const int v = leann_knobs().nw) nw = v;
     if (nw >= 8 && wide_graph(g)) nw = 16;
     if (nw >= 16) return launch_search_NW<T, R, 16>(g, a, st);
     if (nw >= 8) return launch_search_NW<T, R, 8>(g, a, st);
+    if constexpr (T == 3 || T == 6) {
+        if (screen && !a.allow && !a.q_rows && !wide_graph(g)) {
+            size_t lds;
+            if (int rc = search_lds_checked(g, a, &lds, 4)) return rc;
+            return launch_one(beam_search_screen_kernel<T, T == 3 ? LEANN_SCREEN_R3 : LEANN_SCREEN_R6>, 256, lds, g, a, st);
+        }
+    }
     return launch_search_NW<T, R, 4>(g, a, st);
 }
 
@@ -338,12 +356,14 @@
     set_pool_args(h, a);
     const GraphView &g = h->g;
     int T = (int)((g.ld + 255) / 256);
+    const bool screen = h->row_screen.load(std::memory_order_relaxed) != 0 && leann_internal_planes_ready(h) && leann_internal_screen_shape(g);
+    if (screen) { a.x_hi = h->x_hi; a.x_lo = h->x_lo; a.ldp = h->ldp; a.screen_ctr = h->screen_ctr; }
     switch (T) {
         case 1: return launch_search_T<1, 4>(g, a, st);
         case 2: return launch_search_T<2, 4>(g, a, st);
-        case 3: return launch_search_T<3, 4>(g, a, st);
+        case 3: return launch_search_T<3, 4>(g, a, st, screen);
         case 4: return launch_search_T<4, 3>(g, a, st);
-        case 5: case 6: return launch_search_T<6, 2>(g, a, st);
+        case 5: case 6: return launch_search_T<6, 2>(g, a, st, screen);
         case 7: case 8: return launch_search_T<8, 2>(g, a, st);
         case 9: case 10: case 11: case 12: return launch_search_T<12, 1>(g, a, st);
         case 13: case 14: case 15: case 16: return launch_search_T<16, 1>(g, a, st);
@@ -980,6 +1000,7 @@
             return fail("upload of the graph arrays");
     }
     if (hipDeviceSynchronize() != hipSuccess) return fail("hipDeviceSynchronize");
+    leann_internal_sync_planes(h);
     *out = h;
     return LEANN_OK;
 }
diff --git a/leann-rs_amd/csrc/build.hip b/leann-rs_amd/csrc/build.hip
--- a/leann-rs_amd/csrc/build.hip
+++ b/leann-rs_amd/csrc/build.hip
@@ -617,7 +617,7 @@
 static constexpr uint64_t LEVEL_SEED = 0x5EED0003ull;
 
 static int build_device_impl(int backend, const float *d_vectors, size_t n, size_t dims, size_t ld, size_t graph_degree, size_t complexity,
-                             int device, uint64_t key_offset, int take_copy, leann_backend **out);
+                             int device, uint64_t key_offset, int take_copy, leann_backend **out, bool planes);
 static int check_degree(int backend, size_t graph_degree, size_t complexity) {
     const size_t maxdeg = backend == LEANN_BACKEND_HNSW ? 64 : 128;
     if (graph_degree < 2 || graph_degree > maxdeg || complexity < 1) {
@@ -627,18 +627,22 @@
     }
     return LEANN_OK;
 }
+static int build_device_guarded(int backend, const float *d_vectors, size_t n, size_t dims, size_t ld, size_t graph_degree, size_t complexity,
+                                int device, uint64_t key_offset, int take_copy, leann_backend **out, bool planes) {
+    try {
+        return build_device_impl(backend, d_vectors, n, dims, ld, graph_degree, complexity, device, key_offset, take_copy, out, planes);
+    } catch (const std::exception &e) {
+        leann_set_error("build: %s", e.what());
+        return LEANN_ERR_DEVICE;
+    }
+}
 extern "C" int leann_backend_build_device(int backend, const float *d_vectors, size_t n, size_t dims, size_t ld,
                                           size_t graph_degree, size_t complexity, int device, uint64_t key_offset,
                                           int take_copy, leann_backend **out) {
-    try {
-        return build_device_impl(backend, d_vectors, n, dims, ld, graph_degree, complexity, device, key_offset, take_copy, out);
-    } catch (const std::exception &e) {
-        leann_set_error("build: %s", e.what());
-        return LEANN_ERR_DEVICE;
-    }
+    return build_device_guarded(backend, d_vectors, n, dims, ld, graph_degree, complexity, device, key_offset, take_copy, out, true);
 }
 static int build_device_impl(int backend, const float *d_vectors, size_t n, size_t dims, size_t ld, size_t graph_degree, size_t complexity,
-                             int device, uint64_t key_offset, int take_copy, leann_backend **out) {
+                             int device, uint64_t key_offset, int take_copy, leann_backend **out, bool planes) {
     if (!out || (n && !d_vectors) || dims == 0 || dims > 4096 || ld < dims || (ld & 3) || n >= (1ull << 31)) {
         leann_set_error("leann_backend_build_device: invalid arguments (n=%zu dims=%zu ld=%zu)", n, dims, ld);
         return LEANN_ERR_INVALID;
@@ -686,6 +690,7 @@
     int rc = alloc_graph_arrays(h, LEVEL_SEED);
     if (rc == LEANN_OK && n) rc = build_on_device(h, 0, 0);
     if (rc) { leann_backend_close(h); return rc; }
+    if (planes) leann_internal_sync_planes(h);
     *out = h;
     return LEANN_OK;
 }
@@ -719,7 +724,7 @@
         }
     }
     leann_backend *h = nullptr;
-    int rc = leann_backend_build_device(backend, dX, n, dims, ld, graph_degree, complexity, 0, 0, 0, &h);
+    int rc = build_device_guarded(backend, dX, n, dims, ld, graph_degree, complexity, 0, 0, 0, &h, false);
     if (rc) { (void)hipFree(dX); return rc; }
     h->owns_rows = true;
     rc = leann_backend_save(h, index_path_stem);
@@ -794,7 +799,7 @@
         h->g.X = nullptr;
         h->owns_rows = false;
         leann_backend_close(h);
-        rc = leann_backend_build_device(backend, dX, nt, dims, ld, M, efc, 0, 0, 0, &h);
+        rc = build_device_guarded(backend, dX, nt, dims, ld, M, efc, 0, 0, 0, &h, false);
         if (rc) { (void)hipFree(dX); return rc; }
         h->owns_rows = true;
         if (tomb_n) rc = leann_internal_set_removed(h, tomb.data(), tomb_n);
diff --git a/leann-rs_amd/csrc/internal.h b/leann-rs_amd/csrc/internal.h
--- a/leann-rs_amd/csrc/internal.h
+++ b/leann-rs_amd/csrc/internal.h
@@ -24,6 +24,7 @@
     int hash_bits = 0;
     int nw = 0;
     int gpool_bits = 0, gpool2_bits = 0;
+    int row_screen = 1;
     bool no_feat256 = false, no_zero_copy = false, no_emit = false, fused_v1 = false, no_list = false, no_tiled = false;
     bool force_remote = false;
     bool coalesce_off = false;
@@ -64,7 +65,17 @@
     uint64_t removal_epoch = 0;
     uint32_t two_stage = 1;
     std::map<hipStream_t, std::pair<uint8_t *, size_t>> live_scratch;
+    uint16_t *x_hi = nullptr, *x_lo = nullptr;
+    uint32_t ldp = 0, planes_ld = 0;
+    const float *planes_src = nullptr;
+    uint64_t planes_n = 0;
+    unsigned long long *screen_ctr = nullptr;
+    std::atomic<int> row_screen{leann_knobs().row_screen};
 };
+bool leann_internal_screen_shape(const GraphView &g);
+void leann_internal_sync_planes(leann_backend *h);
+bool leann_internal_planes_ready(const leann_backend *h);
+void leann_internal_free_planes(leann_backend *h);
 int leann_internal_live_allow(leann_backend *h, const uint8_t *d_allow, size_t allow_stride, size_t nq, bool walk, hipStream_t st,
                               const uint8_t **out, size_t *out_stride);
 int leann_internal_set_removed(leann_backend *h, const uint8_t *bitmap, size_t n_removed);
@@ -75,6 +86,7 @@
 
 enum { LEANN_LOG_ERROR = 0, LEANN_LOG_WARN = 1, LEANN_LOG_INFO = 2, LEANN_LOG_DEBUG = 3 };
 void leann_log(int level, const char *fmt, ...) __attribute__((format(printf, 2, 3)));
+bool leann_log_enabled(int level);
 int leann_internal_from_host(int backend, size_t n, size_t dims, uint32_t M, uint32_t M0, uint32_t max_level, uint32_t entry,
                              const uint8_t *levels, const uint32_t *upper_off, const uint32_t *adj0, const uint32_t *adjU,
                              size_t n_upper_lists, const float *vectors, const unsigned char *feat_rows, uint32_t feat_h, uint32_t row_bytes,
diff --git a/leann-rs_amd/csrc/planes.hip b/leann-rs_amd/csrc/planes.hip
--- /dev/null
+++ b/leann-rs_amd/csrc/planes.hip
@@ -0,0 +1,133 @@
+#include "common.cuh"
+#include "internal.h"
+#include "row_screen.h"
+
+__global__ void __launch_bounds__(256) split_planes_kernel(const float *__restrict__ X, uint64_t n, uint32_t ld, uint32_t ldp,
+                                                           uint16_t *__restrict__ hi, uint16_t *__restrict__ lo) {
+    const uint32_t per_row = ldp >> 2;
+    const uint64_t items = n * per_row;
+    for (uint64_t it = (uint64_t)blockIdx.x * blockDim.x + threadIdx.x; it < items; it += (uint64_t)gridDim.x * blockDim.x) {
+        const uint64_t row = it / per_row;
+        const uint32_t j = (uint32_t)(it - row * per_row) << 2;
+        uint4 v = make_uint4(0u, 0u, 0u, 0u);
+        if (j < ld) v = *reinterpret_cast<const uint4 *>(X + row * ld + j);
+        const size_t o = (size_t)row * ldp + rs_plane_pos(j, ldp);
+        *reinterpret_cast<uint2 *>(hi + o) = make_uint2((v.x >> 16) | (v.y & 0xFFFF0000u), (v.z >> 16) | (v.w & 0xFFFF0000u));
+        *reinterpret_cast<uint2 *>(lo + o) = make_uint2((v.x & 0xFFFFu) | (v.y << 16), (v.z & 0xFFFFu) | (v.w << 16));
+    }
+}
+
+bool leann_internal_screen_shape(const GraphView &g) {
+    const uint32_t T = (g.ld + 255) / 256;
+    return g.feat_h == 0 && (T == 3 || T == 5 || T == 6) && std::max(g.M0, g.M) <= 64;
+}
+
+struct DeviceScope {
+    int prev = -1;
+    bool ok;
+    explicit DeviceScope(int device) {
+        if (hipGetDevice(&prev) != hipSuccess) { prev = -1; (void)hipGetLastError(); }
+        ok = prev == device || hipSetDevice(device) == hipSuccess;
+        if (!ok) (void)hipGetLastError();
+    }
+    ~DeviceScope() {
+        int cur = -1;
+        if (prev >= 0 && hipGetDevice(&cur) == hipSuccess && cur != prev) (void)hipSetDevice(prev);
+    }
+};
+
+void leann_internal_free_planes(leann_backend *h) {
+    if (!h->x_hi && !h->x_lo && !h->screen_ctr) return;
+    DeviceScope dev(h->device);
+    if (h->screen_ctr && dev.ok && leann_log_enabled(LEANN_LOG_INFO)) {
+        unsigned long long c[2] = {0, 0};
+        if (hipMemcpy(c, h->screen_ctr, 16, hipMemcpyDeviceToHost) == hipSuccess && c[0] + c[1])
+            leann_log(LEANN_LOG_INFO, "row screen: %llu rows ruled out on their upper halves, %llu read in full (%.1f %% ruled out)", c[0], c[1],
+                      100.0 * (double)c[0] / (double)(c[0] + c[1]));
+        else (void)hipGetLastError();
+    }
+    (void)hipFree(h->x_hi);
+    (void)hipFree(h->x_lo);
+    (void)hipFree(h->screen_ctr);
+    h->x_hi = h->x_lo = nullptr;
+    h->screen_ctr = nullptr;
+    h->planes_src = nullptr;
+    h->planes_n = 0;
+}
+
+bool leann_internal_planes_ready(const leann_backend *h) {
+    return h->x_hi && h->planes_src == h->g.X && h->planes_n == h->g.n && h->planes_ld == h->g.ld;
+}
+
+#define LEANN_SCREEN_AUTO_MIN_BYTES ((size_t)1 << 30)
+
+void leann_internal_sync_planes(leann_backend *h) {
+    const int mode = h->row_screen.load();
+    if (h->sharded || mode == 0 || !h->g.X || h->g.n == 0 || !leann_internal_screen_shape(h->g)) return;
+    if (mode == 1 && (size_t)h->g.n * h->g.ld * 4 < LEANN_SCREEN_AUTO_MIN_BYTES) return;
+    if (leann_internal_planes_ready(h)) return;
+    leann_internal_free_planes(h);
+    DeviceScope dev(h->device);
+    if (!dev.ok) return;
+    const uint32_t ldp = (h->g.ld + 63u) & ~63u;
+    const size_t bytes = (size_t)h->g.n * ldp * 2;
+    if (hipMalloc((void **)&h->x_hi, bytes) != hipSuccess || hipMalloc((void **)&h->x_lo, bytes) != hipSuccess ||
+        hipMalloc((void **)&h->screen_ctr, 16) != hipSuccess || hipMemset(h->screen_ctr, 0, 16) != hipSuccess) {
+        leann_log(LEANN_LOG_WARN, "row screen: no room for the split planes (2 x %zu bytes: %s); searching whole rows", bytes,
+                  hipGetErrorString(hipGetLastError()));
+        leann_internal_free_planes(h);
+        return;
+    }
+    const uint64_t items = h->g.n * (uint64_t)(ldp >> 2);
+    const unsigned grid = (unsigned)std::min<uint64_t>((items + 255) / 256, 1u << 20);
+    hipLaunchKernelGGL(split_planes_kernel, dim3(grid), dim3(256), 0, nullptr, h->g.X, h->g.n, h->g.ld, ldp, h->x_hi, h->x_lo);
+    if (hipGetLastError() != hipSuccess || hipDeviceSynchronize() != hipSuccess) {
+        leann_log(LEANN_LOG_WARN, "row screen: splitting the rows failed (%s); searching whole rows", hipGetErrorString(hipGetLastError()));
+        leann_internal_free_planes(h);
+        return;
+    }
+    h->ldp = ldp;
+    h->planes_src = h->g.X;
+    h->planes_n = h->g.n;
+    h->planes_ld = h->g.ld;
+    leann_log(LEANN_LOG_INFO, "row screen: %llu rows split into two planes of %zu bytes", (unsigned long long)h->g.n, bytes);
+}
+
+static void for_each_plain(leann_backend *h, void (*fn)(leann_backend *, void *), void *ctx) {
+    if (!h->sharded) { fn(h, ctx); return; }
+    for (size_t g = 0; g < leann_internal_sharded_count(h->sharded); g++)
+        if (leann_backend *s = leann_internal_sharded_shard(h->sharded, g)) fn(s, ctx);
+}
+
+extern "C" int leann_backend_set_row_screen(leann_backend *h, int enable) {
+    if (!h) { leann_set_error("leann_backend_set_row_screen: null handle"); return LEANN_ERR_INVALID; }
+    for_each_plain(h, [](leann_backend *s, void *ctx) {
+        std::lock_guard<std::mutex> lk(s->mu);
+        s->row_screen.store(*(int *)ctx ? 2 : 0);
+        if (*(int *)ctx) leann_internal_sync_planes(s);
+    }, &enable);
+    return LEANN_OK;
+}
+
+extern "C" int leann_backend_row_screen_stats(const leann_backend *hc, uint64_t out[2]) {
+    leann_backend *h = const_cast<leann_backend *>(hc);
+    if (!h || !out) { leann_set_error("leann_backend_row_screen_stats: null argument"); return LEANN_ERR_INVALID; }
+    struct Acc { uint64_t v[2]; int rc; } acc{{0, 0}, LEANN_OK};
+    for_each_plain(h, [](leann_backend *s, void *ctx) {
+        Acc *a = (Acc *)ctx;
+        if (!s->screen_ctr || a->rc) return;
+        unsigned long long c[2] = {0, 0};
+        DeviceScope dev(s->device);
+        if (!dev.ok || hipDeviceSynchronize() != hipSuccess ||
+            hipMemcpy(c, s->screen_ctr, 16, hipMemcpyDeviceToHost) != hipSuccess) {
+            leann_set_error("leann_backend_row_screen_stats: reading the counters failed: %s", hipGetErrorString(hipGetLastError()));
+            a->rc = LEANN_ERR_DEVICE;
+            return;
+        }
+        a->v[0] += c[0];
+        a->v[1] += c[1];
+    }, &acc);
+    out[0] = acc.v[0];
+    out[1] = acc.v[1];
+    return acc.rc;
+}
diff --git a/leann-rs_amd/csrc/row_screen.h b/leann-rs_amd/csrc/row_screen.h
--- /dev/null
+++ b/leann-rs_amd/csrc/row_screen.h
@@ -0,0 +1,29 @@
+#pragma once
+#include <math.h>
+#include <stdint.h>
+#include <string.h>
+
+#if defined(__HIPCC__) || defined(__CUDACC__)
+#define LEANN_RS_FN __host__ __device__ __forceinline__
+#else
+#define LEANN_RS_FN static inline
+#endif
+
+#define LEANN_RS_C 0x1.004p-7f
+
+LEANN_RS_FN float rs_bits_to_f32(uint32_t b) { float f; memcpy(&f, &b, 4); return f; }
+LEANN_RS_FN uint32_t rs_f32_to_bits(float f) { uint32_t b; memcpy(&b, &f, 4); return b; }
+LEANN_RS_FN uint16_t rs_hi16(float x) { return (uint16_t)(rs_f32_to_bits(x) >> 16); }
+LEANN_RS_FN uint16_t rs_lo16(float x) { return (uint16_t)(rs_f32_to_bits(x) & 0xFFFFu); }
+LEANN_RS_FN float rs_join(uint16_t hi, uint16_t lo) { return rs_bits_to_f32(((uint32_t)hi << 16) | lo); }
+
+LEANN_RS_FN float rs_lane_bound(float s, float a) { return fmaf(LEANN_RS_C, a, s); }
+LEANN_RS_FN float rs_abs_term(float qabs) { return fmaf(qabs, 0x1p-119f, 0x1p-100f); }
+LEANN_RS_FN float rs_lower_bound(float U, float E) { return 1.0f - (U + E); }
+
+LEANN_RS_FN uint32_t rs_plane_pos(uint32_t j, uint32_t ldp) {
+    const uint32_t blk = j >> 9;
+    if (((blk + 1) << 9) > ldp) return j;
+    const uint32_t w = j & 511u, t = w >> 8, l = (w & 255u) >> 2, e = w & 3u;
+    return (blk << 9) + 8u * l + 4u * t + e;
+}
diff --git a/leann-rs_amd/csrc/search.cuh b/leann-rs_amd/csrc/search.cuh
--- a/leann-rs_amd/csrc/search.cuh
+++ b/leann-rs_amd/csrc/search.cuh
@@ -1,5 +1,6 @@
 #pragma once
 #include "common.cuh"
+#include "row_screen.h"
 
 struct GraphView {
     const float *X;
@@ -37,6 +38,9 @@
     uint32_t gpool2_bits, gpool2_tables;
     const uint8_t *allow;
     uint64_t allow_stride;
+    const uint16_t *x_hi, *x_lo;
+    uint32_t ldp;
+    unsigned long long *screen_ctr;
 };
 
 static_assert(alignof(SearchArgs) == 8 && alignof(GraphView) == 8, "lazy_search_args assumes `a` sits at the 8-byte aligned offset behind `g`");
@@ -99,6 +103,78 @@
             out[r] = 1.0f - wave_tree_sum(lane4_sum(acc));
         }
     }
+}
+
+__device__ __forceinline__ uint2 plane_tail_load(const uint16_t *__restrict__ row, uint32_t ldp, int c, int lane) {
+    const uint32_t j = 256u * c + 4u * lane;
+    return j < ldp ? *reinterpret_cast<const uint2 *>(row + j) : make_uint2(0u, 0u);
+}
+template <int T>
+__device__ __forceinline__ void plane_row_load(const uint16_t *__restrict__ row, uint32_t ldp, int lane, uint2 (&h)[T]) {
+#pragma unroll
+    for (int p = 0; p < T / 2; p++) {
+        if (512u * (uint32_t)(p + 1) <= ldp) {
+            const uint4 v = *reinterpret_cast<const uint4 *>(row + 512 * p + 8 * lane);
+            h[2 * p] = make_uint2(v.x, v.y);
+            h[2 * p + 1] = make_uint2(v.z, v.w);
+        } else {
+            h[2 * p] = plane_tail_load(row, ldp, 2 * p, lane);
+            h[2 * p + 1] = plane_tail_load(row, ldp, 2 * p + 1, lane);
+        }
+    }
+    if (T & 1) h[T - 1] = plane_tail_load(row, ldp, T - 1, lane);
+}
+template <int T, int R>
+__device__ __forceinline__ uint32_t wave_dist_rows_screen(const float4 (&q)[T], const uint16_t *__restrict__ Xhi, const uint16_t *__restrict__ Xlo,
+                                                          uint32_t ldp, const uint32_t (&ids)[R], int nrows, int lane, bool armed, float worst,
+                                                          float E, float (&out)[R]) {
+    uint2 h[R][T], l[R][T];
+#pragma unroll
+    for (int r = 0; r < R; r++)
+        if (r < nrows) plane_row_load<T>(Xhi + (size_t)ids[r] * ldp, ldp, lane, h[r]);
+    uint32_t ruled = 0;
+#pragma unroll
+    for (int r = 0; r < R; r++) {
+        if (r < nrows) {
+            float4 s = make_float4(0.f, 0.f, 0.f, 0.f), a = make_float4(0.f, 0.f, 0.f, 0.f);
+#pragma unroll
+            for (int t = 0; t < T; t++) {
+                float4 x;
+                x.x = __uint_as_float(h[r][t].x << 16);
+                x.y = __uint_as_float(h[r][t].x & 0xFFFF0000u);
+                x.z = __uint_as_float(h[r][t].y << 16);
+                x.w = __uint_as_float(h[r][t].y & 0xFFFF0000u);
+                fma4(s, q[t], x);
+                a.x = fmaf(fabsf(q[t].x), fabsf(x.x), a.x);
+                a.y = fmaf(fabsf(q[t].y), fabsf(x.y), a.y);
+                a.z = fmaf(fabsf(q[t].z), fabsf(x.z), a.z);
+                a.w = fmaf(fabsf(q[t].w), fabsf(x.w), a.w);
+            }
+            const float lb = rs_lower_bound(wave_tree_sum(rs_lane_bound(lane4_sum(s), lane4_sum(a))), E);
+            out[r] = lb;
+            if (armed && lb > worst) ruled |= 1u << r;
+        }
+    }
+#pragma unroll
+    for (int r = 0; r < R; r++)
+        if (r < nrows && !((ruled >> r) & 1u)) plane_row_load<T>(Xlo + (size_t)ids[r] * ldp, ldp, lane, l[r]);
+#pragma unroll
+    for (int r = 0; r < R; r++) {
+        if (r < nrows && !((ruled >> r) & 1u)) {
+            float4 acc = make_float4(0.f, 0.f, 0.f, 0.f);
+#pragma unroll
+            for (int t = 0; t < T; t++) {
+                float4 x;
+                x.x = __uint_as_float((h[r][t].x << 16) | (l[r][t].x & 0xFFFFu));
+                x.y = __uint_as_float((h[r][t].x & 0xFFFF0000u) | (l[r][t].x >> 16));
+                x.z = __uint_as_float((h[r][t].y << 16) | (l[r][t].y & 0xFFFFu));
+                x.w = __uint_as_float((h[r][t].y & 0xFFFF0000u) | (l[r][t].y >> 16));
+                fma4(acc, q[t], x);
+            }
+            out[r] = 1.0f - wave_tree_sum(lane4_sum(acc));
+        }
+    }
+    return ruled;
 }
 
 template <int T, int R>
@@ -202,12 +278,13 @@
     return b + ((size_t)1 << hash_bits) * 4;
 }
 
-template <int T, int R, int NW, bool FEAT, bool FILT = false, bool G16 = false, int LW = 1>
+template <int T, int R, int NW, bool FEAT, bool FILT = false, bool G16 = false, int LW = 1, bool SCREEN = false>
 __device__ void beam_search_one(const GraphView &g, const SearchArgs &a, uint32_t qi, unsigned char *smem) {
     const int tid = threadIdx.x, lane = tid & 63, wave = tid >> 6;
     const auto *const za = lazy_search_args();
     const uint32_t ef = a.ef;
     static_assert(LW == 1 || LW == 2, "lists of at most 128 ids");
+    static_assert(!SCREEN || (NW == 4 && !FEAT && !FILT && !G16 && LW == 1), "the row screen exists in the plain throughput form only");
     const uint32_t maxdeg = g.M0 > g.M ? g.M0 : g.M;
     const uint32_t efp = (ef + 1) & ~1u;
     SearchLds s;
@@ -252,6 +329,15 @@
         }
     }
 
+    float rs_E = 0.f;
+    uint32_t rs_ruled = 0;
+    if constexpr (SCREEN) {
+        float4 qs = make_float4(0.f, 0.f, 0.f, 0.f);
+#pragma unroll
+        for (int t = 0; t < T; t++) { qs.x += fabsf(q[t].x); qs.y += fabsf(q[t].y); qs.z += fabsf(q[t].z); qs.w += fabsf(q[t].w); }
+        rs_E = rs_abs_term(wave_tree_sum(lane4_sum(qs)));
+        if (tid == 0) s.misc[10] = 0;
+    }
     const uint32_t *const adj0_p = g.adj0, *const adjU_p = g.adjU, *const upoff_p = g.upper_off;
     uint32_t n_evals = 1, hops0 = 0, hopsU = 0;
     uint32_t n_vis = 0;
@@ -429,6 +515,26 @@
                                 }
                         }
                     }
+                } else if constexpr (SCREEN) {
+                    const bool armed = wsize == ef_l;
+                    const float worst = orderable_f32(uni((uint32_t)(Wc[wsize - 1] >> 32)));
+                    for (uint32_t j0 = wave; j0 < n_new; j0 += NW * R) {
+                        uint32_t ids[R];
+                        float dd[R];
+                        int nrows = 0;
+    #pragma unroll
+                        for (int r = 0; r < R; r++) {
+                            uint32_t j = j0 + r * NW;
+                            if (j < n_new) { ids[r] = s.s_new[j]; nrows = r + 1; }
+                        }
+                        const uint32_t ruled = wave_dist_rows_screen<T, R>(q, za->x_hi, za->x_lo, za->ldp, ids, nrows, lane, armed, worst, rs_E, dd);
+                        rs_ruled += (uint32_t)__popc(ruled);
+                        if (lane == 0) {
+    #pragma unroll
+                            for (int r = 0; r < R; r++)
+                                if (r < nrows) s.s_key[j0 + r * NW] = make_key(dd[r], ids[r]);
+                        }
+                    }
                 } else
                 for (uint32_t j0 = wave; j0 < n_new; j0 += NW * R) {
                     uint32_t ids[R];
@@ -880,6 +986,15 @@
 
     __syncthreads();
     if (hbm && tid == 0) atomicExch(&(hbm == 1 ? za->gpool_lock : za->gpool2_lock)[gslot], 0u);
+    if constexpr (SCREEN) {
+        if (lane == 0 && rs_ruled) atomicAdd(&s.misc[10], rs_ruled);
+        __syncthreads();
+        if (tid == 0) {
+            const uint32_t ruled = s.misc[10];
+            atomicAdd(&za->screen_ctr[0], (unsigned long long)ruled);
+            atomicAdd(&za->screen_ctr[1], (unsigned long long)(n_evals - 1u - ruled));
+        }
+    }
     if (aborted) {
         for (uint32_t t = tid; t < za->k; t += NW * 64) {
             za->out_keys[(size_t)qi * za->k + t] = 0xFFFFFFFFFFFFFFFFull;
@@ -941,6 +1056,19 @@
     if (qi >= a.nq) return;
     beam_search_one<T, R, NW, false>(g, a, qi, smem);
 }
+#ifndef LEANN_SCREEN_OCC3
+#define LEANN_SCREEN_OCC3 4
+#endif
+#ifndef LEANN_SCREEN_OCC6
+#define LEANN_SCREEN_OCC6 3
+#endif
+template <int T, int R>
+__global__ void __launch_bounds__(256, T == 3 ? LEANN_SCREEN_OCC3 : LEANN_SCREEN_OCC6) beam_search_screen_kernel(GraphView g, SearchArgs a) {
+    extern __shared__ __attribute__((aligned(16))) unsigned char smem[];
+    uint32_t qi = blockIdx.x;
+    if (qi >= a.nq) return;
+    beam_search_one<T, R, 4, false, false, false, 1, true>(g, a, qi, smem);
+}
 template <int T, int R, int NW>
 __global__ void __launch_bounds__(NW * 64) beam_search_filtered_kernel(GraphView g, SearchArgs a) {
     extern __shared__ __attribute__((aligned(16))) unsigned char smem[];
diff --git a/leann-rs_amd/host/row_screen_selftest.cpp b/leann-rs_amd/host/row_screen_selftest.cpp
--- /dev/null
+++ b/leann-rs_amd/host/row_screen_selftest.cpp
@@ -0,0 +1,106 @@
+#include "../csrc/row_screen.h"
+#include <cstdio>
+#include <cstdlib>
+#include <vector>
+
+static uint64_t rng_state = 0x9E3779B97F4A7C15ull;
+static uint64_t rnd() {
+    uint64_t x = (rng_state += 0x9E3779B97F4A7C15ull);
+    x = (x ^ (x >> 30)) * 0xBF58476D1CE4E5B9ull;
+    x = (x ^ (x >> 27)) * 0x94D049BB133111EBull;
+    return x ^ (x >> 31);
+}
+static float uni() { return (float)((rnd() >> 40) + 1) * (1.0f / 16777217.0f); }
+static float gauss() { return sqrtf(-2.0f * logf(uni())) * cosf(6.2831853f * uni()); }
+
+static float tree64(float *v) {
+    for (int w = 32; w >= 1; w >>= 1)
+        for (int i = 0; i < w; i++) v[i] = v[2 * i] + v[2 * i + 1];
+    return v[0];
+}
+static float canon_dist(const float *q, const float *x, int T) {
+    float lane[64];
+    for (int l = 0; l < 64; l++) {
+        float a[4] = {0.f, 0.f, 0.f, 0.f};
+        for (int t = 0; t < T; t++)
+            for (int e = 0; e < 4; e++) a[e] = fmaf(q[256 * t + 4 * l + e], x[256 * t + 4 * l + e], a[e]);
+        lane[l] = (a[0] + a[1]) + (a[2] + a[3]);
+    }
+    return 1.0f - tree64(lane);
+}
+static float screen_lb(const float *q, const float *x, int T) {
+    float lane[64], qs[64];
+    for (int l = 0; l < 64; l++) {
+        float s[4] = {0.f, 0.f, 0.f, 0.f}, a[4] = {0.f, 0.f, 0.f, 0.f}, qa[4] = {0.f, 0.f, 0.f, 0.f};
+        for (int t = 0; t < T; t++)
+            for (int e = 0; e < 4; e++) {
+                const float qe = q[256 * t + 4 * l + e], hi = rs_join(rs_hi16(x[256 * t + 4 * l + e]), 0);
+                s[e] = fmaf(qe, hi, s[e]);
+                a[e] = fmaf(fabsf(qe), fabsf(hi), a[e]);
+                qa[e] += fabsf(qe);
+            }
+        lane[l] = rs_lane_bound((s[0] + s[1]) + (s[2] + s[3]), (a[0] + a[1]) + (a[2] + a[3]));
+        qs[l] = (qa[0] + qa[1]) + (qa[2] + qa[3]);
+    }
+    return rs_lower_bound(tree64(lane), rs_abs_term(tree64(qs)));
+}
+
+static void normalize(std::vector<float> &v, int d, float scale) {
+    double n = 0;
+    for (int i = 0; i < d; i++) n += (double)v[i] * v[i];
+    n = n > 0 ? scale / sqrt(n) : 0;
+    for (int i = 0; i < d; i++) v[i] = (float)(v[i] * n);
+}
+
+int main() {
+    unsigned long long cases = 0, violations = 0, roundtrip_bad = 0, layout_bad = 0;
+    double max_gap = 0, min_gap = 1e30;
+    const int dims[] = {768, 1536, 700, 1, 37, 256, 4096};
+    const float scales[] = {1.0f, 1e-3f, 37.5f, 1e-20f, 1e15f};
+    for (int d : dims) {
+        const int T = (d + 255) / 256;
+        std::vector<float> q(256 * T, 0.f), x(256 * T, 0.f), c(256 * T, 0.f);
+        for (int rep = 0; rep < (d > 2000 ? 40 : 150); rep++) {
+            const float sq = scales[rnd() % 5], sx = scales[rnd() % 5];
+            for (int i = 0; i < d; i++) { q[i] = gauss(); c[i] = gauss(); }
+            normalize(q, d, sq);
+            for (int mode = 0; mode < 6; mode++) {
+                for (int i = 0; i < d; i++) x[i] = mode == 0 ? c[i] : (mode == 5 ? -1.f : 1.f) * q[i] / (sq > 0 ? sq : 1.f) + 1e-3f * c[i];
+                normalize(x, d, sx);
+                if (mode >= 2)
+                    for (int i = 0; i < d; i++) {
+                        uint32_t b = rs_f32_to_bits(x[i]);
+                        const bool same = ((b >> 31) != 0) == (q[i] < 0.f);
+                        b = (b & 0xFFFF0000u) | ((same != (mode == 3)) ? 0xFFFFu : 0u);
+                        x[i] = rs_bits_to_f32(b);
+                    }
+                if (mode == 4)
+                    for (int i = 0; i < d; i += 7) {
+                        const uint32_t sign = (uint32_t)(rnd() & 1) << 31;
+                        const uint32_t pick = (uint32_t)(rnd() % 4);
+                        x[i] = rs_bits_to_f32(sign | (pick == 0 ? 0u : pick == 1 ? 0x0000FFFFu : pick == 2 ? 0x007FFFFFu : 0x00800000u | 0xFFFFu));
+                    }
+                const float dist = canon_dist(q.data(), x.data(), T), lb = screen_lb(q.data(), x.data(), T);
+                cases++;
+                if (!(lb <= dist)) violations++;
+                const double gap = (double)dist - (double)lb;
+                if (gap > max_gap) max_gap = gap;
+                if (gap < min_gap) min_gap = gap;
+                for (int i = 0; i < d; i++)
+                    if (rs_f32_to_bits(rs_join(rs_hi16(x[i]), rs_lo16(x[i]))) != rs_f32_to_bits(x[i])) roundtrip_bad++;
+            }
+        }
+    }
+    for (uint32_t ldp = 64; ldp <= 4096; ldp += 64) {
+        std::vector<int> seen(ldp, 0);
+        for (uint32_t j = 0; j < ldp; j++) {
+            const uint32_t p = rs_plane_pos(j, ldp);
+            if (p >= ldp || seen[p]++) layout_bad++;
+            if ((j & 3u) == 0 && (p & 3u)) layout_bad++;
+            if ((j & 3u) && p != rs_plane_pos(j & ~3u, ldp) + (j & 3u)) layout_bad++;
+        }
+    }
+    printf("{\"cases\": %llu, \"violations\": %llu, \"roundtrip_bad\": %llu, \"layout_bad\": %llu, \"min_gap\": %.9g, \"max_gap\": %.9g}\n", cases,
+           violations, roundtrip_bad, layout_bad, min_gap, max_gap);
+    return violations || roundtrip_bad || layout_bad ? 1 : 0;
+}
```

New measurement: 1.287 million (median of 6 runs). +15.2%, better.
